# annegnx/PnP-Flow

Measured on AMD Instinct MI355X. Metric: restored images/sec, higher is better.
Workload: dtype f32-equivalent (f16 hi+lo split operands, 3 x f16 MFMA per product, f32 accumulate); 1 GPU; CelebA-shaped 256x256 box-inpainting (half-size 40, sigma 0.05) pnp_flow B=32/GPU 100x5 (the configuration BASELINE.json's metric is quoted on; main.py:132-136 at 256^2); image=256x256x3, batch_per_gpu=32, global_batch=32, steps_pnp=100, num_samples=5, weights=synthetic seed 0 (no checkpoint offline), hipgraph=True, unet_batch=160, parallelism=dp1 (contiguous shards of the global batch, no data-path collective)

## Files before the change

pnpflow_amd/csrc/conv_route.h:

```cpp
#pragma once
#include <cstddef>

namespace pf {

constexpr int ROUTE_LDS_MAX = 160 * 1024;

constexpr int PP_MAXCH = 32;
constexpr int PP_PW = 18;
constexpr int pp_w9(int TERMS) { return TERMS == 3 ? 36864 : 18432; }
constexpr int pp_w1(int TERMS) { return TERMS == 3 ? 4096 : 2048; }
constexpr int pp_npix(int MT) { return (8 * MT + 2) * PP_PW; }
constexpr int pp_patch_bytes(int MT) { return pp_npix(MT) * 128; }
constexpr int PP_MT = 1;
constexpr size_t pp_weight_bytes(int n9, int n1, int TERMS) { return (size_t)n9 * pp_w9(TERMS) + (size_t)n1 * pp_w1(TERMS); }
constexpr int pp_teams(int n9, int n1, int TERMS) { return 2 * (pp_weight_bytes(n9, n1, TERMS) + pp_patch_bytes(PP_MT)) <= (size_t)ROUTE_LDS_MAX ? 1 : 2; }
constexpr size_t pp_lds(int n9, int n1, int TEAMS, int TERMS) { return pp_weight_bytes(n9, n1, TERMS) + (size_t)TEAMS * pp_patch_bytes(PP_MT); }
constexpr bool pp_structure(int n9, int n1, bool res) {
    if (res) return n9 == 1 && n1 == 0;
    return (n1 == 0 && n9 >= 1 && n9 <= 3) || (n9 == 1 && (n1 == 2 || n1 == 3));
}

constexpr int SP_PITCH = 20, SP_PW = 18;
constexpr int sp_rows(int MT) { return 8 * MT; }
constexpr int sp_npix(int MT) { return (sp_rows(MT) + 2) * SP_PW; }
constexpr int sp_patch(int MT) { return (sp_rows(MT) + 2) * SP_PITCH * 64; }
constexpr int sp_tap(int NT, int TERMS = 3) { return (TERMS == 3 ? 2 : 1) * NT * 1024; }
constexpr int sp_x(int NT, int TERMS = 3) { return (5 * sp_tap(NT, TERMS) + 4095) / 4096 * 4096; }
constexpr int sp_y(int NT, int TERMS = 3) { return 4 * sp_tap(NT, TERMS); }
constexpr int SP_TAB = PP_MAXCH * 32;
constexpr int sp_lds(int MT, int NT, int TERMS = 3) { return sp_x(NT, TERMS) + sp_y(NT, TERMS) + 2 * sp_patch(MT) + SP_TAB; }

constexpr int DMA_TH = 8, DMA_BN = 128;
constexpr size_t dma_lds() {
    constexpr int PH = DMA_TH + 2, PW = 18, NINST = (PH * PW * 8 + 63) / 64, IPW = (NINST + 3) / 4, BUF = IPW * 4 * 1024;
    return 2 * (size_t)BUF;
}

struct RouteSeg {
    int C = 0, cstride = 0, taps = 0, xform = 0, w_mode = 0;
    bool has_w16 = false;
    bool has_w16_src = false;
    int src_lo = 0, src_hi = 0, src_O = 0, src_kk = 0;
};
struct RouteShape {
    RouteSeg seg[3];
    int nseg = 0, B = 0, H = 0, W = 0, Hs = 0, Ws = 0, Cout = 0, out_cstride = 0, res_cstride = 0, gn_C = 0;
    bool residual = false, addvec = false, coef = false, scale = false, gnb = false;
};
struct RouteEnv {
    int cu_grid = 0;
    int pp = 1;
    int sp = 1;
    int dma = 1;
    int upphase = 1;
};
inline RouteEnv mfma_only(RouteEnv env) { env.pp = env.sp = env.dma = 0; return env; }

enum class ConvFamily { MFMA32, MFMA16, DMA, PP, SP };
struct ConvRoute {
    ConvFamily family = ConvFamily::MFMA32;
    int terms = 0;
    int MT = 0, NT = 0, WM = 0, WN = 0, S = 1, UP = 0, BM = 0, KC = 0;
    int n9 = 0, n1 = 0, teams = 0, nsplit = 0; bool res = false, gnb = false;
    int grid_x = 0, grid_y = 1, xcd_map = 0; size_t lds_bytes = 0;
    int csv_code = 0;
    const char* refused = nullptr;
};

inline int ilog2_exact(int v) { int l = 0; while (l < 30 && (1 << l) < v) ++l; return (1 << l) == v ? l : -1; }

namespace route_detail {

inline bool packed16(const RouteShape& p) {
    for (int i = 0; i < p.nseg; ++i) if (p.seg[i].w_mode != 0 || !p.seg[i].has_w16) return false;
    return true;
}
inline bool chunk_sources(const RouteShape& p, bool nine_taps) {
    for (int i = 0; i < p.nseg; ++i) {
        const RouteSeg& s = p.seg[i];
        if (!s.has_w16_src || s.src_O != p.Cout || (nine_taps && s.src_kk != 9)) return false;
    }
    return true;
}

inline bool pp_ok(const RouteShape& p, int stride, int up, int terms, const RouteEnv& env, int& n9, int& n1) {
    constexpr int TH = 8 * PP_MT;
    if (env.pp == 0 || (terms != 3 && !(terms == 1 && env.pp != 3)) || stride != 1 || up != 0 || p.gnb) return false;
    if (p.Cout != 32 || p.out_cstride != 32 || (p.residual && p.res_cstride != 32)) return false;
    if (p.H % TH || p.W % 16 || p.Hs != p.H || p.Ws != p.W) return false;
    if (ilog2_exact(p.H / TH) < 0 || ilog2_exact(p.W / 16) < 0) return false;
    if (env.cu_grid < 8 || (long long)p.B * (p.H / TH) * (p.W / 16) < 32LL * 2 * env.cu_grid) return false;
    if (p.W > 2048) return false;
    n9 = 0; n1 = 0;
    for (int i = 0; i < p.nseg; ++i) {
        const RouteSeg& s = p.seg[i];
        if (s.w_mode != 0 || !s.has_w16 || s.C % 32) return false;
        if (s.taps == 9) { if (n1 > 0 || s.xform == 0) return false; n9 += s.C / 32; }
        else if (s.taps == 1) { if (s.xform != 0) return false; n1 += s.C / 32; }
        else return false;
    }
    if (!pp_structure(n9, n1, p.residual)) return false;
    if (p.gn_C > 0 && !p.coef) return false;
    if (pp_weight_bytes(n9, n1, terms) + 2 * (size_t)pp_patch_bytes(PP_MT) > (size_t)ROUTE_LDS_MAX) return false;
    return chunk_sources(p, false);
}

inline bool sp_ok(const RouteShape& p, int stride, int up, int terms, const RouteEnv& env) {
    const int mode = env.sp;
    if (mode == 0 || (terms != 3 && !(terms == 1 && mode != 3)) || stride != 1 || up != 0 || p.gnb) return false;
    const int nsplit = p.Cout == 256 ? 2 : 1;
    if (p.Cout != 128 && !(p.Cout == 64 && (mode == 1 || mode == 4)) && !(p.Cout == 256 && mode == 1 && terms == 3)) return false;
    if (p.out_cstride != p.Cout || (p.residual && p.res_cstride != p.Cout)) return false;
    if (!p.addvec) return false;
    const int TH = p.Cout == 64 ? sp_rows(4) : sp_rows(2);
    if (p.H % TH || p.W % 16 || p.Hs != p.H || p.Ws != p.W) return false;
    if ((long long)(TH + 1) * p.W + SP_PW - 1 > 65535) return false;
    if (ilog2_exact(p.H / TH) < 0 || ilog2_exact(p.W / 16) < 0) return false;
    const int grid = env.cu_grid;
    if (grid < 8 || (long long)nsplit * p.B * (p.H / TH) * (p.W / 16) < 4LL * grid || (nsplit == 2 && grid % 16 != 0)) return false;
    int nch = 0;
    for (int i = 0; i < p.nseg; ++i) {
        const RouteSeg& s = p.seg[i];
        if ((double)p.B * p.H * p.W * s.cstride >= 2147483648.0) return false;
        if (s.w_mode != 0 || !s.has_w16 || s.C % 32 || s.taps != 9 || s.xform != 2) return false;
        nch += s.C / 16;
    }
    if (nch < 2 || nch > PP_MAXCH || (nch & 1)) return false;
    if (!(p.gn_C > 0 && p.coef && p.scale)) return false;
    return chunk_sources(p, true);
}

inline bool dma_phase_shape_ok(const RouteShape& p, int terms, const RouteEnv& env) {
    if (env.upphase == 0 || env.dma == 0 || (terms != 3 && terms != 1) || p.nseg != 1 || p.residual || p.gnb) return false;
    if (p.H != 2 * p.Hs || p.W != 2 * p.Ws || p.Hs % DMA_TH != 0 || p.Ws % 16 != 0 || p.Cout % 32 != 0 || (4 * p.Cout) % DMA_BN != 0) return false;
    if (p.seg[0].w_mode != 0 || p.seg[0].C % (terms == 3 ? 32 : 64) != 0) return false;
    if ((size_t)(p.Hs + 2) * (p.Ws + 2) * 128 >= (1ull << 31)) return false;
    if (env.dma >= 2) return true;
    return (long long)p.B * (p.Hs / DMA_TH) * (p.Ws / 16) * (4 * p.Cout / DMA_BN) >= 512;
}

inline bool dma_ok(const RouteShape& p, int stride, int up, int terms, const RouteEnv& env) {
    if (terms != 3 && terms != 1) return false;
    if (terms == 1)
        for (int i = 0; i < p.nseg; ++i)
            if (p.seg[i].w_mode != 0 || !p.seg[i].has_w16_src || (p.seg[i].src_hi - p.seg[i].src_lo) % 64 != 0) return false;
    if (env.dma == 0 || stride != 1 || (up != 0 && up != 1 && up != 2)) return false;
    if (p.gnb) return false;
    if (up == 2) return dma_phase_shape_ok(p, terms, env) && p.seg[0].taps == 4 && p.seg[0].has_w16;
    if (p.Cout % DMA_BN != 0 || p.H % DMA_TH != 0 || p.W % 16 != 0) return false;
    if (up == 1 && (p.H != 2 * p.Hs || p.W != 2 * p.Ws)) return false;
    if (up == 0 && (p.H != p.Hs || p.W != p.Ws)) return false;
    const int kc = terms == 3 ? 32 : 64;
    for (int i = 1; i < p.nseg; ++i) if (p.seg[i].taps == 9 && p.seg[i - 1].taps == 1) return false;
    for (int i = 0; i < p.nseg; ++i) {
        const RouteSeg& s = p.seg[i];
        if (s.w_mode != 0 || !s.has_w16) return false;
        if (s.C % kc != 0 || (s.taps != 9 && s.taps != 1)) return false;
    }
    if ((size_t)(p.Hs + 2) * (p.Ws + 2) * 128 >= (1ull << 31)) return false;
    if (env.dma >= 2) return true;
    const long long wgs = (long long)p.B * (p.H / DMA_TH) * (p.W / 16) * (p.Cout / DMA_BN);
    if (wgs < 512) return false;
    constexpr double min_ratio = 2000.0;
    double macs = 0.0, elts = 0.0; bool all1 = true;
    for (int i = 0; i < p.nseg; ++i) { macs += (double)p.seg[i].taps * p.seg[i].C * p.Cout; elts += p.seg[i].C; all1 &= p.seg[i].taps == 1; }
    if (up) elts *= 0.25;
    if (all1) return p.Cout >= 3 * (int)elts;
    return macs / elts >= min_ratio;
}

struct Tile { int MT, NT, WM, WN; };
constexpr int tile_th(const Tile& t) { return 2 * t.MT * t.WM; }
constexpr int tile_bn(const Tile& t) { return t.WN * t.NT * 32; }
inline long long tile_wgs(const RouteShape& p, const Tile& t) {
    return (long long)p.B * ((p.H + tile_th(t) - 1) / tile_th(t)) * ((p.W + 15) / 16) * ((p.Cout + tile_bn(t) - 1) / tile_bn(t));
}
inline Tile ladder(const RouteShape& p, const Tile* t, int n, long long min_wgs) {
    for (int i = 0; i + 1 < n; ++i) if (tile_wgs(p, t[i]) >= min_wgs) return t[i];
    return t[n - 1];
}
inline void set_tile(ConvRoute& r, const RouteShape& p, const Tile& t, bool xcd_fold) {
    r.MT = t.MT; r.NT = t.NT; r.WM = t.WM; r.WN = t.WN;
    const long long tiles = (long long)p.B * ((p.H + tile_th(t) - 1) / tile_th(t)) * ((p.W + 15) / 16), nblk = (p.Cout + tile_bn(t) - 1) / tile_bn(t);
    r.grid_x = (int)tiles; r.grid_y = (int)nblk; r.xcd_map = 0;
    if (xcd_fold && (tiles * nblk) % 8 == 0) { r.xcd_map = 1; r.grid_x = (int)(tiles * nblk); r.grid_y = 1; }
}
inline size_t mfma_epilogue_floats(const Tile& t) { return 4 * 32 * 36 + (size_t)t.WM * tile_bn(t) * 2; }

inline ConvRoute mfma16(const RouteShape& p, int stride, int up, int terms) {
    ConvRoute r; r.family = ConvFamily::MFMA16; r.terms = terms == 1 ? 1 : 3; r.gnb = p.gnb; r.csv_code = 0;
    if (p.gn_C > 1024 || (p.gn_C > 0 && !p.coef)) { r.refused = "conv_mfma16 parks at most 4 x 256 GroupNorm channels and needs their coefficients"; return r; }
    bool all_1tap = true, all32 = true;
    for (int i = 0; i < p.nseg; ++i) {
        all_1tap &= p.seg[i].taps == 1 && p.seg[i].C % 64 == 0;
        all32 &= p.seg[i].C % 32 == 0;
    }
    if (all_1tap && stride == 1 && !up) { r.S = 1; r.UP = 0; r.KC = 64; }
    else if (stride == 2) { r.S = 2; r.UP = 0; r.KC = 16; }
    else if (up == 2) { r.S = 1; r.UP = 2; r.KC = 16; }
    else { r.S = 1; r.UP = up ? 1 : 0; r.KC = all32 ? 32 : 16; }
    if (p.gnb && !(r.S == 1 && r.UP == 0)) { r.refused = "the GroupNorm-backward epilogue exists at stride 1 without upsampling only"; return r; }
    const long long MIN_WGS = r.KC == 64 ? 1024 : 512;
    static constexpr Tile s1_32 = {2, 1, 4, 1};
    static constexpr Tile s1_64[] = {{4, 1, 2, 2}, {2, 1, 2, 2}, {1, 1, 2, 2}};
    static constexpr Tile s1_128[] = {{4, 1, 1, 4}, {2, 1, 1, 4}, {1, 1, 2, 2}};
    static constexpr Tile s2_32 = {1, 1, 4, 1}, s2_64 = {2, 1, 2, 2}, s2_128 = {1, 1, 2, 2};
    const Tile t = r.S == 1 ? (p.Cout <= 32 ? s1_32 : p.Cout <= 64 ? ladder(p, s1_64, 3, MIN_WGS) : ladder(p, s1_128, 3, MIN_WGS))
                            : (p.Cout <= 32 ? s2_32 : p.Cout <= 64 ? s2_64 : s2_128);
    set_tile(r, p, t, true);
    const int ROW = (r.terms == 3 ? r.KC : r.KC / 2) + 4, HALO = r.KC == 64 ? 0 : 1;
    const int PH = (tile_th(t) - 1) * r.S + 1 + 2 * HALO, PW = 15 * r.S + 1 + 2 * HALO, RS = ((PW * ROW + 63) / 64) * 64;
    const size_t patch = (size_t)PH * RS, epi = mfma_epilogue_floats(t);
    r.lds_bytes = ((patch > epi ? patch : epi) + 2 * (size_t)((p.gn_C + 3) & ~3)) * 4;
    return r;
}

inline ConvRoute mfma32(const RouteShape& p, int stride, int up, int terms) {
    ConvRoute r; r.family = ConvFamily::MFMA32; r.terms = terms; r.csv_code = 0;
    if (p.gnb) { r.refused = "the GroupNorm-backward epilogue exists on conv_mfma16 only"; return r; }
    bool generic = false;
    for (int i = 0; i < p.nseg; ++i) generic |= p.seg[i].w_mode != 0;
    if (generic) {
        for (int i = 0; i < p.nseg; ++i) if (p.seg[i].w_mode == 0) { r.refused = "packed and generic weight operands in one launch"; return r; }
        if (stride != 1 || up) { r.refused = "generic weight operands at stride 1 without upsampling only"; return r; }
    }
    bool all_1tap = true;
    for (int i = 0; i < p.nseg; ++i) all_1tap &= p.seg[i].taps == 1 && (generic ? p.seg[i].C >= 64 : p.seg[i].C % 64 == 0);
    r.BM = generic ? 1 : 0;
    if (all_1tap && stride == 1 && !up) { r.S = 1; r.UP = 0; r.KC = 64; }
    else if (generic) { r.S = 1; r.UP = 0; r.KC = 16; }
    else if (stride == 2) { r.S = 2; r.UP = 0; r.KC = 16; }
    else { r.S = 1; r.UP = up == 2 ? 2 : up ? 1 : 0; r.KC = 16; }
    constexpr long long MIN_WGS = 512;
    static constexpr Tile s1_32 = {2, 1, 4, 1};
    static constexpr Tile s1_64[] = {{2, 2, 4, 1}, {1, 2, 4, 1}, {1, 1, 2, 2}};
    static constexpr Tile s1_128[] = {{2, 2, 2, 2}, {1, 2, 2, 2}, {1, 2, 4, 1}, {1, 1, 2, 2}};
    static constexpr Tile s2_32 = {1, 1, 4, 1}, s2_64 = {1, 2, 4, 1}, s2_128 = {1, 1, 2, 2};
    const Tile t = r.S == 1 ? (p.Cout <= 32 ? s1_32 : p.Cout <= 64 ? ladder(p, s1_64, 3, MIN_WGS) : ladder(p, s1_128, 4, MIN_WGS))
                            : (p.Cout <= 32 ? s2_32 : p.Cout <= 64 ? s2_64 : s2_128);
    set_tile(r, p, t, false);
    const size_t patch = (size_t)((tile_th(t) - 1) * r.S + 3) * (15 * r.S + 3) * (r.KC + 4), epi = mfma_epilogue_floats(t);
    r.lds_bytes = ((patch > epi ? patch : epi) + 2 * (size_t)((p.gn_C + 3) & ~3)) * sizeof(float);
    return r;
}

}

inline bool conv_route_phase_ok(const RouteShape& p, int terms, const RouteEnv& env) { return route_detail::dma_phase_shape_ok(p, terms, env); }

inline ConvRoute conv_route(const RouteShape& p, int stride, int up, int terms, const RouteEnv& env) {
    namespace d = route_detail;
    if (terms != 1 && terms != 3) return d::mfma32(p, stride, up, 0);
    ConvRoute r; r.terms = terms;
    if (d::sp_ok(p, stride, up, terms, env)) {
        r.family = ConvFamily::SP; r.csv_code = 5;
        r.MT = p.Cout == 64 ? 4 : 2; r.NT = p.Cout == 64 ? 2 : 4; r.nsplit = p.Cout == 256 ? 2 : 1; r.res = p.residual;
        for (int i = 0; i < p.nseg; ++i) r.n9 += p.seg[i].C / 16;
        r.grid_x = env.cu_grid; r.lds_bytes = (size_t)sp_lds(r.MT, r.NT, terms);
        return r;
    }
    if (d::pp_ok(p, stride, up, terms, env, r.n9, r.n1)) {
        r.family = ConvFamily::PP; r.csv_code = 2;
        r.MT = PP_MT; r.res = p.residual; r.teams = pp_teams(r.n9, r.n1, terms);
        r.grid_x = env.cu_grid * (r.teams == 1 ? 2 : 1); r.lds_bytes = pp_lds(r.n9, r.n1, r.teams, terms);
        return r;
    }
    r.n9 = r.n1 = 0;
    if (d::dma_ok(p, stride, up, terms, env)) {
        r.family = ConvFamily::DMA; r.csv_code = 1;
        r.MT = 4; r.NT = 1; r.WM = 1; r.WN = 4; r.UP = up; r.KC = terms == 3 ? 32 : 64;
        const long long tiles = up == 2 ? (long long)p.B * (p.Hs / DMA_TH) * (p.Ws / 16) : (long long)p.B * (p.H / DMA_TH) * (p.W / 16);
        const long long nblk = (up == 2 ? 4 * p.Cout : p.Cout) / DMA_BN;
        r.grid_x = (int)tiles; r.grid_y = (int)nblk;
        if ((tiles * nblk) % 8 == 0) { r.xcd_map = 1; r.grid_x = (int)(tiles * nblk); r.grid_y = 1; }
        r.lds_bytes = dma_lds();
        return r;
    }
    return d::packed16(p) ? d::mfma16(p, stride, up, terms) : d::mfma32(p, stride, up, terms);
}

}
```

pnpflow_amd/csrc/conv_sp.hip:

```cpp
#include "pp_common.h"

namespace pf {

constexpr int sp_a9(int MT) { return (sp_npix(MT) * 4 + 255) / 256; }
constexpr int sp_stage_n(int A9, int tap) {
    const int slot = tap < 4 ? tap : tap < 8 ? tap - 1 : 7;
    if (tap == 4 || tap == 8) return 0;
    return A9 / 7 + (slot < A9 % 7 ? 1 : 0);
}
constexpr int sp_stage_0(int A9, int tap) { int n = 0; for (int t = 0; t < tap; ++t) n += sp_stage_n(A9, t); return n; }

__device__ __forceinline__ void glds16_sp(unsigned voff, const char* sbase, unsigned lds_dst) {
    unsigned keep;
    asm volatile("s_mov_b32 %0, m0\n\ts_mov_b32 m0, %3\n\ts_nop 0\n\tglobal_load_lds_dwordx4 %1, %2\n\ts_mov_b32 m0, %0"
                 : "=&s"(keep) : "v"(voff), "s"(sbase), "s"(lds_dst) : "memory");
}

#ifdef PP_PROBE_BUILD
__device__ unsigned long long* g_sp_dbg = nullptr;
#define SP_STAMP(k) do { if (stamp_buf != nullptr && blockIdx.x == 0 && tid == 0 && stamp_n < 64) stamp_buf[stamp_n * 16 + (k)] = __builtin_readcyclecounter(); } while (0)
#else
#define SP_STAMP(k) do { } while (0)
#endif

template <int MT, int NT, bool RES, int TERMS = 3, int NSPLIT = 1>
__global__ __launch_bounds__(256, 1) void conv_sp_kernel(const PPParams p) {
    constexpr int TH = sp_rows(MT), NPIX = sp_npix(MT), A9 = sp_a9(MT), PATCH = sp_patch(MT);
    constexpr int TAPB = sp_tap(NT, TERMS), XB = sp_x(NT, TERMS), COUT = 32 * NT, CTOT = COUT * NSPLIT, OB = CTOT * 4;
    constexpr int NFRAG = (TERMS == 3 ? 2 : 1) * (MT + NT), NMMA = TERMS * MT * NT;
    static_assert(TERMS == 3 || TERMS == 1, "split terms");
    static_assert(NSPLIT == 1 || NSPLIT == 2, "N-halves");
    static_assert(sp_y(NT, TERMS) % 4096 == 0 && 9 * TAPB >= XB, "refill rounds of 4 KiB; slot X's over-fetch stays inside the chunk image");
    constexpr int REQ1 = sp_stage_0(A9, 4), REQ2 = A9 - REQ1 + 3;
    static_assert(sp_stage_0(A9, 9) == A9 && REQ1 + NT + 4 * MT * NT < 64, "staging distribution / vmcnt range");
    extern __shared__ __attribute__((aligned(16))) char smem[];
    const int tid = threadIdx.x;
    const int lane = tid & 63, wq = __builtin_amdgcn_readfirstlane(tid >> 6);
    const int l31 = lane & 31, hi = lane >> 5;
    constexpr unsigned PATCH0 = (unsigned)(XB + sp_y(NT, TERMS)), TAB = PATCH0 + 2u * (unsigned)PATCH;
    const pp_float_cptr scale_c = (pp_float_cptr)(uintptr_t)p.scale;
    const int nch = p.n9;

    const int qi = tid & 3, p0 = tid >> 2;
    unsigned pk[A9], ldsw[A9];
#pragma unroll
    for (int i = 0; i < A9; ++i) {
        const int pp = min(p0 + 64 * i, NPIX - 1);
        const int py = pp / SP_PW, px = pp - py * SP_PW;
        pk[i] = (unsigned)(py * p.W + px) | ((py == 0 ? 1u : 0u) << 20) | ((py == TH + 1 ? 1u : 0u) << 21) | ((px == 0 ? 1u : 0u) << 22) |
                ((px == SP_PW - 1 ? 1u : 0u) << 23);
        ldsw[i] = PATCH0 + (unsigned)((py * SP_PITCH + px) * 64) + (unsigned)((((qi >> 1) ^ ((px >> 2) & 3)) << 4) + (qi & 1) * 8);
    }
    const int pix_safe = p.W + 1;

    const int prow = l31 >> 4, pcol = l31 & 15;
    unsigned a_addr[3][2];
#pragma unroll
    for (int kx = 0; kx < 3; ++kx) {
        const unsigned base = PATCH0 + (unsigned)(((wq * 2 * MT + prow) * SP_PITCH + pcol + kx) * 64);
        const unsigned s = (unsigned)(((pcol + kx) >> 2) & 3);
#pragma unroll
        for (int tm = 0; tm < 2; ++tm) a_addr[kx][tm] = base + ((((unsigned)(hi + 2 * tm)) ^ s) << 4);
    }
    const unsigned b_lane = (unsigned)lane * 16u;
    const unsigned dma_lane = (unsigned)(wq * 1024 + lane * 16);

    const bool bit3 = (lane & 8) != 0;
    const int em = lane & 7;
    const int ch_of_col = 4 * (l31 & 7) + (l31 >> 3);
    const unsigned e_lane = (unsigned)((4 * hi + ((lane >> 3) & 3)) * OB + em * 16);

    const int G = (int)gridDim.x / NSPLIT;
    const int rg0 = (blockIdx.x & 7) * ((int)gridDim.x >> 3) + (blockIdx.x >> 3);
    const int rg = NSPLIT == 2 ? rg0 >> 1 : rg0, half = NSPLIT == 2 ? rg0 & 1 : 0;
    const int hoff = NSPLIT == 2 ? half * COUT : 0;
    const int T = p.B << (p.lx + p.ly);
    const int t_begin = (int)((long)rg * T / G), t_end = (int)((long)(rg + 1) * T / G);
    const int ntl = t_end - t_begin;
    const int rot = ntl > 0 ? (int)(((long)rg * p.rot) % ntl) : 0;
    auto tile_of = [&](int it) __attribute__((always_inline)) -> PPTile {
        const int idx = min(it, ntl - 1);
        const int wrapped = idx + rot >= ntl ? idx + rot - ntl : idx + rot;
        const int tl = t_begin + wrapped;
        PPTile r;
        const int tx = tl & ((1 << p.lx) - 1), ty = (tl >> p.lx) & ((1 << p.ly) - 1);
        r.b = tl >> (p.lx + p.ly); r.oy0 = ty * TH; r.ox0 = tx * 16;
        r.edge = (ty == 0 ? 1 : 0) | (ty == (1 << p.ly) - 1 ? 2 : 0) | (tx == 0 ? 4 : 0) | (tx == (1 << p.lx) - 1 ? 8 : 0);
        return r;
    };

    float4 ra[A9];
    unsigned zero_v;
    asm volatile("v_mov_b32 %0, 0" : "=v"(zero_v));
    struct Coef { float4 csc, csh; float ascale; unsigned inval; };
    Coef cf0, cf1;
    typedef const __attribute__((address_space(1))) char* gptr;
    struct Src { gptr base; unsigned cs4; };
    const unsigned q16 = (unsigned)qi * 16u;
    struct Desc { gptr base; const char* cb; unsigned cs4; int edge; unsigned sofs; };
    struct Ent { uint4 a, b; };
    auto fetch = [&](int c) __attribute__((always_inline)) -> Ent {
        Ent e;
        e.a = *reinterpret_cast<const uint4*>(smem + TAB + (unsigned)c * 32u); e.b = *reinterpret_cast<const uint4*>(smem + TAB + (unsigned)c * 32u + 16u);
        return e;
    };
    auto sptr = [&](unsigned lo, unsigned hi) __attribute__((always_inline)) -> gptr {
        return (gptr)(((unsigned long long)(unsigned)__builtin_amdgcn_readfirstlane((int)hi) << 32) | (unsigned)__builtin_amdgcn_readfirstlane((int)lo));
    };
    auto describe = [&](const PPTile& tl, const Ent& e) __attribute__((always_inline)) -> Desc {
        const int pix = (tl.b * p.H + tl.oy0) * p.W + tl.ox0 - p.W - 1;
        const int cstride = __builtin_amdgcn_readfirstlane((int)e.b.x), coff = __builtin_amdgcn_readfirstlane((int)e.b.y);
        const int gn_c0 = __builtin_amdgcn_readfirstlane((int)e.b.z), seg = __builtin_amdgcn_readfirstlane((int)e.b.w);
        Desc d;
        d.sofs = (unsigned)(8 * tl.b + seg) * 4u;
        d.edge = tl.edge;
        d.cb = reinterpret_cast<const char*>(p.coef + (tl.b * 2 * p.coef_stride + gn_c0));
        d.base = sptr(e.a.x, e.a.y) + (long)(pix * cstride + coff) * 4;
        d.cs4 = (unsigned)cstride * 4u;
        return d;
    };
    auto prep = [&](Coef& N, const Desc& d) __attribute__((always_inline)) -> Src {
        N.ascale = *reinterpret_cast<const float*>(reinterpret_cast<const char*>(p.scale) + d.sofs + zero_v);
        unsigned inval = 0;
#pragma unroll
        for (int i = 0; i < A9; ++i) inval |= (((pk[i] >> 20) & (unsigned)d.edge) != 0u ? 1u : 0u) << i;
        N.inval = inval;
        N.csc = *reinterpret_cast<const float4*>(d.cb + q16); N.csh = *reinterpret_cast<const float4*>(d.cb + (unsigned)(p.coef_stride * 4) + q16);
        Src r; r.base = d.base; r.cs4 = d.cs4;
        return r;
    };
    auto issue_one = [&](const Coef& N, const Src& sr, int i) __attribute__((always_inline)) {
        const unsigned px = ((N.inval >> i) & 1u) ? (unsigned)pix_safe : (pk[i] & 0xffffu);
        const pp_f4v t_ = *reinterpret_cast<const __attribute__((address_space(1))) pp_f4v*>(sr.base + (__umul24(px, sr.cs4) + q16));
        ra[i] = make_float4(t_.x, t_.y, t_.z, t_.w);
    };
    auto transform_one = [&](const Coef& S, int i, unsigned pofs) __attribute__((always_inline)) {
        float4 v = ra[i];
        v.x = silu_pp(v.x * S.csc.x + S.csh.x); v.y = silu_pp(v.y * S.csc.y + S.csh.y);
        v.z = silu_pp(v.z * S.csc.z + S.csh.z); v.w = silu_pp(v.w * S.csc.w + S.csh.w);
        const float f = ((S.inval >> i) & 1u) ? 0.0f : S.ascale;
        v.x *= f; v.y *= f; v.z *= f; v.w *= f;
        f16x4 h = {(_Float16)v.x, (_Float16)v.y, (_Float16)v.z, (_Float16)v.w};
        if constexpr (TERMS == 3) {
            f16x4 l = {(_Float16)(v.x - (float)h[0]), (_Float16)(v.y - (float)h[1]), (_Float16)(v.z - (float)h[2]), (_Float16)(v.w - (float)h[3])};
            const unsigned addr = ldsw[i] + pofs;
            *reinterpret_cast<f16x4*>(smem + addr) = h;
            *reinterpret_cast<f16x4*>(smem + (addr ^ 32u)) = l;
        } else {
            *reinterpret_cast<f16x4*>(smem + ldsw[i] + pofs) = h;
        }
    };

    f32x16 acc[MT][NT];
#pragma unroll
    for (int mt = 0; mt < MT; ++mt)
#pragma unroll
        for (int nt = 0; nt < NT; ++nt)
#pragma unroll
            for (int r = 0; r < 16; ++r) acc[mt][nt][r] = 0.f;
    float run1[4 * NT], run2[4 * NT];
#pragma unroll
    for (int j = 0; j < 4 * NT; ++j) { run1[j] = 0.f; run2[j] = 0.f; }
    int run_b = -1, run_n = 0;

    auto flush_stats = [&]() __attribute__((always_inline)) {
        if (p.stats_out == nullptr || run_b < 0) return;
#pragma unroll
        for (int j = 0; j < 4 * NT; ++j) {
            double a = (double)run1[j], q = (double)run2[j];
            a += __shfl_xor(a, 8); q += __shfl_xor(q, 8);
            a += __shfl_xor(a, 16); q += __shfl_xor(q, 16);
            a += __shfl_xor(a, 32); q += __shfl_xor(q, 32);
            if (lane < 8) {
                double* dst = p.stats_out + ((size_t)run_b * CTOT + hoff + (j >> 2) * 32 + em * 4 + (j & 3)) * 2;
                unsafeAtomicAdd(dst, a); unsafeAtomicAdd(dst + 1, q);
            }
            run1[j] = 0.f; run2[j] = 0.f;
        }
        run_n = 0;
    };

    auto tile_offs = [&](int mt, int nt, int g) __attribute__((always_inline)) -> size_t {
        return (size_t)((mt * 2 + (g >> 1)) * p.W) * OB + (size_t)((g & 1) * 8 * OB + nt * 128) + e_lane;
    };
    int seg_c1 = -1, seg_c2 = -1;
    for (int c = 1; c < nch; ++c)
        if (p.ch[c].seg != p.ch[c - 1].seg) { if (seg_c1 < 0) seg_c1 = c; else seg_c2 = c; }
    const int seg_id[4] = {p.ch[0].seg, p.ch[seg_c1 > 0 ? seg_c1 : 0].seg, p.ch[seg_c2 > 0 ? seg_c2 : 0].seg, p.ch[nch - 1].seg};
    float addv[NT]; float oscale = 0.f;
    auto tile_inputs = [&](const PPTile& tl) __attribute__((always_inline)) {
#pragma unroll
        for (int nt = 0; nt < NT; ++nt) addv[nt] = p.addvec[(size_t)tl.b * p.addvec_bs + hoff + nt * 32 + ch_of_col];
        const float inv_last = scale_c[8 * tl.b + 4 + seg_id[3]];
        oscale = p.out_scale * (1.0f / 256.0f) * inv_last;
        asm volatile("" : "+v"(oscale));
    };
    auto epilogue = [&](const PPTile& tl) __attribute__((always_inline)) {
        if (tl.b != run_b || run_n >= 32) { flush_stats(); run_b = tl.b; }
        ++run_n;
        const size_t pix0 = ((size_t)tl.b * p.H + tl.oy0 + wq * 2 * MT) * p.W + tl.ox0;
        char* obase = reinterpret_cast<char*>(p.out + pix0 * CTOT + hoff);
        const char* rbase = RES ? reinterpret_cast<const char*>(p.residual + pix0 * CTOT + hoff) : nullptr;
        float4 rv[3][4];
        if constexpr (RES) {
#pragma unroll
            for (int g = 0; g < 4; ++g) rv[0][g] = nt_load4(rbase + tile_offs(0, 0, g));
            if (MT * NT > 1) {
#pragma unroll
                for (int g = 0; g < 4; ++g) rv[1][g] = nt_load4(rbase + tile_offs(1 / NT, 1 % NT, g));
            }
        }
#pragma unroll
        for (int mt = 0; mt < MT; ++mt)
#pragma unroll
            for (int nt = 0; nt < NT; ++nt) {
                const int k = mt * NT + nt;
                if constexpr (RES) {
                    if (k + 2 < MT * NT) {
#pragma unroll
                        for (int g = 0; g < 4; ++g) rv[(k + 2) % 3][g] = nt_load4(rbase + tile_offs((k + 2) / NT, (k + 2) % NT, g));
                    }
                }
                float e[16];
#pragma unroll
                for (int r = 0; r < 16; ++r) e[r] = acc[mt][nt][r] * oscale + addv[nt];
#pragma unroll
                for (int g = 0; g < 4; ++g) {
                    oct_transpose(e[4 * g], e[4 * g + 1], e[4 * g + 2], e[4 * g + 3], bit3);
                    float4 v = make_float4(e[4 * g], e[4 * g + 1], e[4 * g + 2], e[4 * g + 3]);
                    if constexpr (RES) {
                        const float rsc = p.res_scale; const float4 r4 = rv[k % 3][g];
                        v.x = fmaf(r4.x, rsc, v.x); v.y = fmaf(r4.y, rsc, v.y); v.z = fmaf(r4.z, rsc, v.z); v.w = fmaf(r4.w, rsc, v.w);
                    }
                    *reinterpret_cast<float4*>(obase + tile_offs(mt, nt, g)) = v;
                    run1[nt * 4 + 0] += v.x; run1[nt * 4 + 1] += v.y; run1[nt * 4 + 2] += v.z; run1[nt * 4 + 3] += v.w;
                    run2[nt * 4 + 0] += v.x * v.x; run2[nt * 4 + 1] += v.y * v.y; run2[nt * 4 + 2] += v.z * v.z; run2[nt * 4 + 3] += v.w * v.w;
                }
            }
#pragma unroll
        for (int mt = 0; mt < MT; ++mt)
#pragma unroll
            for (int nt = 0; nt < NT; ++nt)
#pragma unroll
                for (int r = 0; r < 16; ++r) acc[mt][nt][r] = 0.f;
    };

    f16x8 fa[2][MT][2], fb[2][NT][2];
    auto load_tap = [&](int set, int tap, unsigned pofs) __attribute__((always_inline)) {
        const int ky = tap / 3, kx = tap % 3;
        const unsigned wb = (unsigned)(tap < 5 ? tap * TAPB : XB + (tap - 5) * TAPB) + b_lane;
        if constexpr (TERMS == 3) {
#pragma unroll
            for (int mt = 0; mt < MT; ++mt) fa[set][mt][1] = *reinterpret_cast<const f16x8*>(smem + a_addr[kx][1] + (unsigned)((mt * 2 + ky) * SP_PITCH * 64) + pofs);
        }
#pragma unroll
        for (int nt = 0; nt < NT; ++nt) fb[set][nt][0] = *reinterpret_cast<const f16x8*>(smem + wb + (unsigned)(nt * 1024));
#pragma unroll
        for (int mt = 0; mt < MT; ++mt) fa[set][mt][0] = *reinterpret_cast<const f16x8*>(smem + a_addr[kx][0] + (unsigned)((mt * 2 + ky) * SP_PITCH * 64) + pofs);
        if constexpr (TERMS == 3) {
#pragma unroll
            for (int nt = 0; nt < NT; ++nt) fb[set][nt][1] = *reinterpret_cast<const f16x8*>(smem + wb + (unsigned)(NT * 1024 + nt * 1024));
        }
    };
    auto load_frag = [&](int set, int tap, unsigned pofs, int idx) __attribute__((always_inline)) {
        const int ky = tap / 3, kx = tap % 3;
        const unsigned wb = (unsigned)(tap < 5 ? tap * TAPB : XB + (tap - 5) * TAPB) + b_lane;
        if constexpr (TERMS == 3) {
            if (idx < MT) fa[set][idx][1] = *reinterpret_cast<const f16x8*>(smem + a_addr[kx][1] + (unsigned)((idx * 2 + ky) * SP_PITCH * 64) + pofs);
            else if (idx < MT + NT) fb[set][idx - MT][0] = *reinterpret_cast<const f16x8*>(smem + wb + (unsigned)((idx - MT) * 1024));
            else if (idx < 2 * MT + NT) fa[set][idx - MT - NT][0] = *reinterpret_cast<const f16x8*>(smem + a_addr[kx][0] + (unsigned)(((idx - MT - NT) * 2 + ky) * SP_PITCH * 64) + pofs);
            else fb[set][idx - 2 * MT - NT][1] = *reinterpret_cast<const f16x8*>(smem + wb + (unsigned)(NT * 1024 + (idx - 2 * MT - NT) * 1024));
        } else {
            if (idx < NT) fb[set][idx][0] = *reinterpret_cast<const f16x8*>(smem + wb + (unsigned)(idx * 1024));
            else fa[set][idx - NT][0] = *reinterpret_cast<const f16x8*>(smem + a_addr[kx][0] + (unsigned)(((idx - NT) * 2 + ky) * SP_PITCH * 64) + pofs);
        }
    };
    auto mma_group = [&](int set, int g) __attribute__((always_inline)) {
        const int term = TERMS == 3 ? g / MT : 2, mt = g % MT;
#pragma unroll
        for (int nt = 0; nt < NT; ++nt)
            acc[mt][nt] = __builtin_amdgcn_mfma_f32_32x32x16_f16(fa[set][mt][term == 0 ? 1 : 0], fb[set][nt][term == 1 ? 1 : 0], acc[mt][nt], 0, 0, 0);
    };
    auto mma_tap = [&](int set) __attribute__((always_inline)) {
#pragma unroll
        for (int g = 0; g < TERMS * MT; ++g) mma_group(set, g);
    };
    auto tap_pattern = [&]() __attribute__((always_inline)) {
        if constexpr (TERMS == 3) {
#pragma unroll
        for (int k = 0; k < 3 * MT * NT; ++k) {
            __builtin_amdgcn_sched_group_barrier(0x008, 1, 0);
            if (k < 2 * (MT + NT)) __builtin_amdgcn_sched_group_barrier(0x100, 1, 0);
            if (k < 2 * (MT + NT)) __builtin_amdgcn_sched_group_barrier(0x002, A9 > 7 ? 2 : 1, 0);
            else __builtin_amdgcn_sched_group_barrier(0x002, A9 > 7 ? 5 : 3, 0);
            __builtin_amdgcn_sched_group_barrier(0x400, 1, 0);
            __builtin_amdgcn_sched_group_barrier(0x004, 2, 0);
            if (k >= 3 * MT * NT - 4) __builtin_amdgcn_sched_group_barrier(0x200, 1, 0);
            if (k == 3 * MT * NT - 2) __builtin_amdgcn_sched_group_barrier(0x020, 1, 0);
        }
        } else {
#pragma unroll
        for (int k = 0; k < MT * NT; ++k) {
            __builtin_amdgcn_sched_group_barrier(0x008, 1, 0);
            if (k < NFRAG) __builtin_amdgcn_sched_group_barrier(0x100, 1, 0);
            __builtin_amdgcn_sched_group_barrier(0x002, A9 > 7 ? 10 : 6, 0);
            __builtin_amdgcn_sched_group_barrier(0x400, A9 > 7 ? 2 : 1, 0);
            __builtin_amdgcn_sched_group_barrier(0x004, 4, 0);
            if (k >= MT * NT - 4) __builtin_amdgcn_sched_group_barrier(0x200, 1, 0);
            if (k >= MT * NT - 2) __builtin_amdgcn_sched_group_barrier(0x020, 1, 0);
        }
        }
    };
    auto mma_tap_refill = [&](int set, const __attribute__((address_space(1))) char* src, int t0, int nrounds, int nset, int ntap, unsigned npofs) __attribute__((always_inline)) {
        const unsigned dst0 = (unsigned)(t0 < 5 ? t0 * TAPB : XB + (t0 - 5) * TAPB) + (unsigned)(wq * nrounds * 1024);
        const __attribute__((address_space(1))) char* sb = src + t0 * TAPB + wq * nrounds * 1024;
        unsigned keep;
        asm volatile("s_mov_b32 %0, m0" : "=s"(keep));
#pragma unroll
        for (int g = 0; g < TERMS * MT; ++g) {
            const int term = TERMS == 3 ? g / MT : 2, mt = g % MT;
#pragma unroll
            for (int nt = 0; nt < NT; ++nt) {
                acc[mt][nt] = __builtin_amdgcn_mfma_f32_32x32x16_f16(fa[set][mt][term == 0 ? 1 : 0], fb[set][nt][term == 1 ? 1 : 0], acc[mt][nt], 0, 0, 0);
                __builtin_amdgcn_sched_barrier(0);
                const int j = g * NT + nt;
                if (j < nrounds) {
                    if ((j & 3) == 0) asm volatile("s_mov_b32 m0, %0\n\ts_nop 0" :: "s"(dst0 + (unsigned)(j * 1024)) : "memory");
                    if ((j & 3) == 0) asm volatile("global_load_lds_dwordx4 %0, %1" :: "v"(b_lane), "s"(sb + j * 1024) : "memory");
                    if ((j & 3) == 1) asm volatile("global_load_lds_dwordx4 %0, %1 offset:1024" :: "v"(b_lane), "s"(sb + (j - 1) * 1024) : "memory");
                    if ((j & 3) == 2) asm volatile("global_load_lds_dwordx4 %0, %1 offset:2048" :: "v"(b_lane), "s"(sb + (j - 2) * 1024) : "memory");
                    if ((j & 3) == 3) asm volatile("global_load_lds_dwordx4 %0, %1 offset:3072" :: "v"(b_lane), "s"(sb + (j - 3) * 1024) : "memory");
                }
                if (j < NFRAG) load_frag(nset, ntap, npofs, j);
                __builtin_amdgcn_sched_barrier(0);
            }
        }
        asm volatile("s_mov_b32 m0, %0" :: "s"(keep));
    };

    int stamp_n = 0; (void)stamp_n;
#ifdef PP_PROBE_BUILD
    unsigned long long* const stamp_buf = g_sp_dbg;
#endif
    gptr wimg_next = (gptr)(uintptr_t)(half ? p.wimg_h1[1] : p.ch[1].wimg);
    Desc dn;
    Src sr;
    auto chunk = [&](int it, int c, auto SI_, bool last_chunk) __attribute__((always_inline)) {
        constexpr int SI = decltype(SI_)::value;
        constexpr unsigned PCUR = SI ? PATCH : 0, PNXT = SI ? 0 : PATCH;
        Coef& C = SI == 0 ? cf1 : cf0;
        Coef& N = SI == 0 ? cf0 : cf1;
        const gptr wnext = wimg_next;
        (void)last_chunk;
        SP_STAMP(0);
#pragma unroll
        for (int tap = 0; tap < 4; ++tap) {
            __builtin_amdgcn_sched_barrier(0);
            load_tap((tap + 1 + SI) & 1, tap + 1, PCUR);
#pragma unroll
            for (int i = sp_stage_0(A9, tap); i < sp_stage_0(A9, tap) + sp_stage_n(A9, tap); ++i) { transform_one(C, i, PNXT); issue_one(N, sr, i); }
            mma_tap((tap + SI) & 1);
            tap_pattern();
            __builtin_amdgcn_sched_barrier(0);
            SP_STAMP(1 + tap);
        }
        __builtin_amdgcn_sched_barrier(0);
        if (c == 0) asm volatile("s_waitcnt vmcnt(%0) lgkmcnt(0)" :: "n"(REQ1 + NT + 4 * MT * NT) : "memory");
        else asm volatile("s_waitcnt vmcnt(%0) lgkmcnt(0)" :: "n"(REQ1) : "memory");
#pragma unroll
        for (int i = REQ1; i < A9; ++i) asm volatile("" :: "v"(ra[i].x));
        SP_STAMP(13);
        __builtin_amdgcn_s_barrier();
        __builtin_amdgcn_sched_barrier(0);
        SP_STAMP(5);
        mma_tap_refill((4 + SI) & 1, wnext, 0, XB / 4096, (5 + SI) & 1, 5, PCUR);
        SP_STAMP(6);
#pragma unroll
        for (int tap = 5; tap < 8; ++tap) {
            __builtin_amdgcn_sched_barrier(0);
            int q = c + 3, wrap = 0;
            if (q >= nch) { q -= nch; wrap = 1; }
            if (q >= nch) { q -= nch; wrap = 2; }
            const int c2 = c + 2 >= nch ? c + 2 - nch : c + 2;
            Ent eq, e2;
            if (tap == 6) { eq = fetch(q); e2 = fetch(c2); }
            load_tap((tap + 1 + SI) & 1, tap + 1, PCUR);
#pragma unroll
            for (int i = sp_stage_0(A9, tap); i < sp_stage_0(A9, tap) + sp_stage_n(A9, tap); ++i) { transform_one(C, i, PNXT); issue_one(N, sr, i); }
            if (tap == 6) {
                dn = describe(tile_of(it + wrap), eq);
                wimg_next = sptr(e2.a.z, e2.a.w);
            }
            if (tap == 7) sr = prep(C, dn);
            mma_tap((tap + SI) & 1);
            tap_pattern();
            __builtin_amdgcn_sched_barrier(0);
            SP_STAMP(2 + tap);
        }
        __builtin_amdgcn_sched_barrier(0);
        asm volatile("s_waitcnt vmcnt(%0) lgkmcnt(0)" :: "n"(REQ2) : "memory");
#pragma unroll
        for (int i = 0; i < REQ1; ++i) asm volatile("" :: "v"(ra[i].x));
        SP_STAMP(14);
        __builtin_amdgcn_s_barrier();
        __builtin_amdgcn_sched_barrier(0);
        SP_STAMP(10);
        mma_tap_refill((8 + SI) & 1, wnext, 5, 4 * TAPB / 4096, (9 + SI) & 1, 0, PNXT);
        SP_STAMP(11);
        SP_STAMP(12);
        ++stamp_n;
    };

    if (ntl <= 0) return;
    for (int c = 0; c < nch; ++c) {
        if (tid == 0) {
            const unsigned long long sp_ = (unsigned long long)(uintptr_t)p.ch[c].src, wp_ = (unsigned long long)(uintptr_t)(half ? p.wimg_h1[c] : p.ch[c].wimg);
            *reinterpret_cast<uint4*>(smem + TAB + (unsigned)c * 32u) = make_uint4((unsigned)sp_, (unsigned)(sp_ >> 32), (unsigned)wp_, (unsigned)(wp_ >> 32));
            *reinterpret_cast<uint4*>(smem + TAB + (unsigned)c * 32u + 16u) = make_uint4((unsigned)p.ch[c].cstride, (unsigned)p.ch[c].coff, (unsigned)p.ch[c].gn_c0, (unsigned)p.ch[c].seg);
        }
    }
    __syncthreads();
    {
        const Src s0 = prep(cf0, describe(tile_of(0), fetch(0)));
#pragma unroll
        for (int i = 0; i < A9; ++i) issue_one(cf0, s0, i);
        {
            const char* w0 = reinterpret_cast<const char*>(half ? p.wimg_h1[0] : p.ch[0].wimg);
#pragma unroll
            for (int j = 0; j < (TERMS == 3 ? 9 * TAPB : XB) / 4096; ++j) glds16_sp(dma_lane, w0 + j * 4096, (unsigned)(j * 4096) + (unsigned)(wq * 1024));
            if constexpr (TERMS != 3) {
#pragma unroll
                for (int j = 0; j < 4 * TAPB / 4096; ++j) glds16_sp(dma_lane, w0 + 5 * TAPB + j * 4096, (unsigned)(XB + j * 4096) + (unsigned)(wq * 1024));
            }
        }
#pragma unroll
        for (int i = 0; i < A9; ++i) transform_one(cf0, i, 0);
        const Src s1 = prep(cf1, describe(tile_of(0), fetch(1)));
#pragma unroll
        for (int i = 0; i < A9; ++i) issue_one(cf1, s1, i);
        sr = prep(cf0, describe(tile_of(2 >= nch ? 1 : 0), fetch(2 >= nch ? 2 - nch : 2)));
        asm volatile("s_waitcnt vmcnt(0) lgkmcnt(0)" ::: "memory");
        __builtin_amdgcn_s_barrier();
        __builtin_amdgcn_sched_barrier(0);
        load_tap(0, 0, 0);
    }
    const int seg_lo[4] = {0, seg_c1 > 0 ? seg_c1 : nch, seg_c2 > 0 ? seg_c2 : nch, nch};
#pragma unroll 1
    for (int it = 0; it < ntl; ++it) {
        tile_inputs(tile_of(it));
#pragma unroll 1
        for (int sg = 0; sg < 3; ++sg) {
            const int lo = seg_lo[sg], hi = seg_lo[sg + 1];
            if (lo >= hi) continue;
            if (sg > 0) {
                const PPTile tl = tile_of(it);
                const float ratio = scale_c[8 * tl.b + seg_id[sg]] * scale_c[8 * tl.b + 4 + seg_id[sg - 1]];
                if (ratio != 1.0f) {
#pragma unroll
                    for (int mt = 0; mt < MT; ++mt)
#pragma unroll
                        for (int nt = 0; nt < NT; ++nt)
#pragma unroll
                            for (int r = 0; r < 16; ++r) acc[mt][nt][r] *= ratio;
                }
            }
#pragma unroll 1
            for (int c = lo; c < hi; c += 2) {
                chunk(it, c, ic<0>{}, false);
                chunk(it, c + 1, ic<1>{}, false);
            }
        }
        epilogue(tile_of(it));
    }
    flush_stats();
    asm volatile("s_waitcnt vmcnt(0)" ::: "memory");
}


template <int MT, int NT, int TERMS, int NSPLIT = 1>
static hipError_t launch_sp_t(const PPParams& p0, const ConvRoute& r, hipStream_t s) {
    static unsigned long long attr_set[2] = {0ull, 0ull};
    const void* kern = r.res ? reinterpret_cast<const void*>(conv_sp_kernel<MT, NT, true, TERMS, NSPLIT>) : reinterpret_cast<const void*>(conv_sp_kernel<MT, NT, false, TERMS, NSPLIT>);
    { hipError_t e = set_max_dynamic_lds_once(kern, attr_set[r.res ? 1 : 0], ROUTE_LDS_MAX); if (e != hipSuccess) return e; }
    if (r.grid_x <= 0 || (NSPLIT == 2 && r.grid_x % 16 != 0)) return hipErrorInvalidConfiguration;
    PPParams p = p0;
    p.lx = ilog2_exact(p.W / 16); p.ly = ilog2_exact(p.H / sp_rows(MT));
    p.rot = 5;
    if (r.res) hipLaunchKernelGGL((conv_sp_kernel<MT, NT, true, TERMS, NSPLIT>), dim3(r.grid_x), dim3(256), r.lds_bytes, s, p);
    else hipLaunchKernelGGL((conv_sp_kernel<MT, NT, false, TERMS, NSPLIT>), dim3(r.grid_x), dim3(256), r.lds_bytes, s, p);
    return hipGetLastError();
}

hipError_t launch_conv_sp(const PPParams& p, const ConvRoute& r, hipStream_t s) {
    if (r.family != ConvFamily::SP || r.n9 != p.n9 || p.n1 != 0 || r.res != (p.residual != nullptr)) return hipErrorInvalidValue;
    switch (r.MT * 1000 + r.NT * 100 + r.nsplit * 10 + r.terms) {
        case 2423: return launch_sp_t<2, 4, 3, 2>(p, r, s);
        case 2413: return launch_sp_t<2, 4, 3>(p, r, s);
        case 2411: return launch_sp_t<2, 4, 1>(p, r, s);
        case 4213: return launch_sp_t<4, 2, 3>(p, r, s);
        case 4211: return launch_sp_t<4, 2, 1>(p, r, s);
        default: return hipErrorInvalidValue;
    }
}

}
```

pnpflow_amd/csrc/engine.hip:

```cpp
#include <algorithm>
#include <cmath>
#include <cstdio>
#include <cstring>
#include <cstdlib>
#include <functional>
#include <map>
#include <memory>
#include <string>
#include <vector>

#include "../../include/pnpflow_hip.h"
#include "pf_common.h"
#include "weight_pack.h"
#include "rk45_control.h"
#include "adam_step.h"

using namespace pf;

namespace {

struct HostTensor { std::vector<int64_t> shape; std::vector<float> data; bool loaded = false; };

struct ResDesc {
    std::string prefix;
// ... 73 lines not shown
    int in_ch = 0, out_ch = 0;
    bool up = false, down = false;
};

struct CachedGraph;
struct SolverBufs;
struct OdeBufs;
struct DFlowState;
struct DopriState;
struct PnpGsState;
struct FlowPriorsState;
struct PriorEvalState;

struct pf_engine {
    int device = 0;
    pf_unet_cfg cfg{};
    int arch = 0;
    pf_ncsnpp_cfg ncfg{};
    std::vector<NxMod> nx_mods;
    float solver_time_scale = 1.0f;
    std::string err;
    std::vector<std::pair<std::string, std::vector<int64_t>>> expected;
    std::map<std::string, HostTensor> host;
    bool finalized = false;
    std::vector<LevelDesc> down, up;
    ResDesc mid0, mid2; std::string mid_attn;
    int mid_ch = 0;
    std::vector<std::pair<std::string, int>> res_order;
    std::map<std::string, float*> dev;
    struct W16Src { std::string name; int lo, hi; };
    std::map<const void*, W16Src> w16_src;
    std::vector<void*> weight_allocs;
    int temb_total = 0;
    std::map<std::string, int> temb_off;
    std::map<int, std::unique_ptr<Plan>> plans;
    Plan* last_plan = nullptr;
    Plan* retained_plan = nullptr;
    int retained_B = 0;
    uint64_t plan_clock = 0;
    int64_t bytes = 0;
    int precision = 1;
    SolverBufs* sb = nullptr;
    OdeBufs* ob = nullptr;
    int64_t ode_krylov_iters = 0;
    hipStream_t work_stream = nullptr;
    DFlowState* dflow = nullptr;
    DopriState* dopri = nullptr;
    PnpGsState* pnpgs = nullptr;
    PriorEvalState* prior = nullptr;
    FlowPriorsState* fprior = nullptr;
    std::vector<CachedGraph*> graphs;
    bool profile = false;
    std::vector<std::pair<hipEvent_t, hipEvent_t>> ev_pool;
    std::vector<const Op*> ev_ops;
    size_t ev_used = 0;
    int64_t prof_launches = 0; double prof_ms = 0.0, prof_flops = 0.0;
};

static thread_local std::string g_create_err;

static int poison_mask() { static const int m = getenv("PNPFLOW_HIP_POISON") ? atoi(getenv("PNPFLOW_HIP_POISON")) : 0; return m == 1 ? 7 : m; }
static bool poison_enabled() { return poison_mask() != 0; }
static void poison(void* p, size_t bytes, int group = 1) {
    if ((poison_mask() & group) && p) { hipDeviceSynchronize(); hipMemset(p, 0xFF, bytes); hipDeviceSynchronize(); }
}

struct DeviceGuard {
    int prev = -1; hipError_t err = hipSuccess;
    explicit DeviceGuard(int dev) { if (hipGetDevice(&prev) != hipSuccess) prev = -1; err = hipSetDevice(dev); }
    ~DeviceGuard() { if (prev >= 0) hipSetDevice(prev); }
};
#define USE_DEVICE(e) DeviceGuard _dg((e)->device); HIPCHK(e, _dg.err)

#define LAUNCHCHK(call)                                                        \
    do { hipError_t _r = (call); if (_r != hipSuccess) return _r == hipErrorInvalidValue ? PF_ERR_INVALID : PF_ERR_HIP; } while (0)


#define HIPCHK(e, call)                                                                        \
    do {                                                                                       \
        hipError_t _r = (call);                                                                \
        if (_r != hipSuccess) {                                                                \
            (e)->err = std::string(#call) + ": " + hipGetErrorString(_r);                      \
            return PF_ERR_HIP;                                                                 \
        }                                                                                      \
    } while (0)

#include "solver_rt.inc"

static bool in_attn_res(const pf_unet_cfg& c, int h) {
    for (int i = 0; i < c.num_attn_resolutions; ++i) if (c.attn_resolutions[i] == h) return true;
    return false;
}

static void expect(pf_engine* e, const std::string& n, std::vector<int64_t> s) { e->expected.emplace_back(n, std::move(s)); }
static void expect_lin(pf_engine* e, const std::string& p, int i, int o) { expect(e, p + "weight", {o, i}); expect(e, p + "bias", {o}); }
static void expect_conv(pf_engine* e, const std::string& p, int i, int o, int k) { expect(e, p + "weight", {o, i, k, k}); expect(e, p + "bias", {o}); }
static void expect_gn(pf_engine* e, const std::string& p, int c) { expect(e, p + "weight", {c}); expect(e, p + "bias", {c}); }
static void expect_res(pf_engine* e, const std::string& p, int i, int o, int tch) {
    expect_lin(e, p + "temb_proj.", tch, o); expect_gn(e, p + "norm1.", i); expect_conv(e, p + "conv1.", i, o, 3);
    expect_gn(e, p + "norm2.", o); expect_conv(e, p + "conv2.", o, o, 3);
    if (i != o) expect_conv(e, p + "shortcut.", i, o, 1);
}
static void expect_attn(pf_engine* e, const std::string& p, int c) {
    expect_conv(e, p + "attn_q.", c, c, 1); expect_conv(e, p + "attn_k.", c, c, 1);
    expect_conv(e, p + "attn_v.", c, c, 1); expect_conv(e, p + "proj_out.", c, c, 1);
    expect_gn(e, p + "norm.", c);
}

static int build_arch(pf_engine* e) {
    const pf_unet_cfg& c = e->cfg;
    const int ch = c.ch, nlev = c.num_levels, nres = c.num_res_blocks, tch = 4 * ch;
    char buf[128];
    expect_lin(e, "temb_net.main.0.", ch, tch); expect_lin(e, "temb_net.main.2.", tch, tch);
    expect_conv(e, "begin_conv.", c.input_channels, ch, 3);
    std::vector<int> chans{ch};
    int cur = ch, h = c.input_height;
    for (int lvl = 0; lvl < nlev; ++lvl) {
        LevelDesc L;
        const int o = ch * c.ch_mult[lvl];
        for (int blk = 0; blk < nres; ++blk) {
            ResDesc r;
            snprintf(buf, sizeof buf, "down_modules.%d.%da_%da_block.", lvl, lvl, blk); r.prefix = buf;
            r.cin0 = cur; r.cout = o;
            expect_res(e, r.prefix, cur, o, tch);
            if (in_attn_res(c, h)) {
                r.attn = true;
                snprintf(buf, sizeof buf, "down_modules.%d.%da_%db_attn.", lvl, lvl, blk); r.attn_prefix = buf;
                expect_attn(e, r.attn_prefix, o);
            }
            L.blocks.push_back(r); chans.push_back(o); cur = o;
        }
        if (lvl != nlev - 1) {
            snprintf(buf, sizeof buf, "down_modules.%d.%db_downsample.", lvl, lvl); L.resample = buf; L.res_ch = o;
            expect_conv(e, L.resample, o, o, 3);
            h /= 2; chans.push_back(o);
        }
        e->down.push_back(L);
    }
    e->mid_ch = cur;
    e->mid0.prefix = "mid_modules.0."; e->mid0.cin0 = cur; e->mid0.cout = cur;
    e->mid2.prefix = "mid_modules.2."; e->mid2.cin0 = cur; e->mid2.cout = cur;
    e->mid_attn = "mid_modules.1.";
    expect_res(e, e->mid0.prefix, cur, cur, tch); expect_attn(e, e->mid_attn, cur); expect_res(e, e->mid2.prefix, cur, cur, tch);
    for (int idx = 0; idx < nlev; ++idx) {
        const int lvl = nlev - 1 - idx;
        LevelDesc L;
        const int o = ch * c.ch_mult[lvl];
        for (int blk = 0; blk < nres + 1; ++blk) {
            ResDesc r;
            snprintf(buf, sizeof buf, "up_modules.%d.%da_%da_block.", idx, lvl, blk); r.prefix = buf;
            r.cin0 = cur; r.cin1 = chans.back(); chans.pop_back(); r.cout = o;
            expect_res(e, r.prefix, r.cin0 + r.cin1, o, tch);
            if (in_attn_res(c, h)) {
                r.attn = true;
                snprintf(buf, sizeof buf, "up_modules.%d.%da_%db_attn.", idx, lvl, blk); r.attn_prefix = buf;
                expect_attn(e, r.attn_prefix, o);
            }
            L.blocks.push_back(r); cur = o;
        }
        if (lvl != 0) {
            snprintf(buf, sizeof buf, "up_modules.%d.%db_upsample.up_conv.", idx, lvl); L.resample = buf; L.res_ch = o;
            expect_conv(e, L.resample, o, o, 3);
            h *= 2;
        }
        e->up.push_back(L);
    }
    if (!chans.empty()) { e->err = "internal: skip stack not empty"; return PF_ERR_INVALID; }
    expect_gn(e, "end_conv.0.", cur); expect_conv(e, "end_conv.2.", cur, c.output_channels, 3);
    if (cur != ch) { e->err = "internal: final width != ch"; return PF_ERR_INVALID; }
    for (auto& L : e->down) for (auto& r : L.blocks) e->res_order.emplace_back(r.prefix, r.cout);
    e->res_order.emplace_back(e->mid0.prefix, e->mid0.cout); e->res_order.emplace_back(e->mid2.prefix, e->mid2.cout);
    for (auto& L : e->up) for (auto& r : L.blocks) e->res_order.emplace_back(r.prefix, r.cout);
    int off = 0;
    for (auto& pr : e->res_order) { e->temb_off[pr.first] = off; off += pr.second; }
    e->temb_total = off;
    return PF_OK;
}

static const HostTensor& W(pf_engine* e, const std::string& n) { return e->host.at(n); }

static float* upload_new(pf_engine* e, const std::string& key, const void* src, size_t bytes) {
    float* d = nullptr;
    if (hipMalloc(&d, std::max<size_t>(bytes, 16)) != hipSuccess) return nullptr;
    e->bytes += (int64_t)std::max<size_t>(bytes, 16);
    hipMemcpy(d, src, bytes, hipMemcpyHostToDevice);
    e->weight_allocs.push_back(d);
    e->dev[key] = d;
    return d;
}
static float* upload(pf_engine* e, const std::string& key, const std::vector<float>& v) {
    auto it = e->dev.find(key);
    return it != e->dev.end() ? it->second : upload_new(e, key, v.data(), v.size() * sizeof(float));
}

static wpack::Oihw oihw(pf_engine* e, const std::string& wname) {
    const HostTensor& t = W(e, wname);
    return {t.data.data(), (int)t.shape[0], (int)t.shape[1], (int)(t.shape[2] * t.shape[3])};
}
static std::string range_key(int lo, int hi) { return std::to_string(lo) + ":" + std::to_string(hi); }

template <class Pack>
static float* weight_image(pf_engine* e, const std::string& key, Pack pack, const pf_engine::W16Src* src = nullptr) {
    auto it = e->dev.find(key);
    if (it != e->dev.end()) return it->second;
    const auto img = pack();
    float* d = upload_new(e, key, img.data(), img.size() * sizeof(img[0]));
    if (d && src) e->w16_src[d] = *src;
    return d;
}

static float* packed_conv(pf_engine* e, const std::string& wname, int lo, int hi) {
    return weight_image(e, wname + "#" + range_key(lo, hi), [&] { return wpack::frag32(oihw(e, wname), lo, hi); });
}
static const void* packed_conv16(pf_engine* e, const std::string& wname, int lo, int hi, int terms = 3) {
    const pf_engine::W16Src src{wname, lo, hi};
    return weight_image(e, wname + (terms == 1 ? "#h1_" : "#h") + range_key(lo, hi), [&] { return wpack::slice16(oihw(e, wname), lo, hi, terms); }, terms == 1 ? nullptr : &src);
}

static int conv_terms(const pf_engine* e) { return e->precision == 0 ? 0 : e->precision == 2 ? 1 : 3; }

struct Builder {
    pf_engine* e; Plan* plan; int B; bool ok = true;
    std::multimap<size_t, void*> free_list;
    std::map<void*, size_t> sizes;
    size_t stats_bytes = 0;
    std::vector<std::pair<double**, size_t>> stats_fix;

    float* acquire(size_t nfloats) {
        const size_t bytes = ((nfloats * sizeof(float) + 255) / 256) * 256;
        auto it = free_list.find(bytes);
        if (it != free_list.end()) { void* p = it->second; free_list.erase(it); return (float*)p; }
        void* p = nullptr;
        if (hipMalloc(&p, bytes) != hipSuccess) { ok = false; e->err = "hipMalloc failed (activations)"; return nullptr; }
        poison(p, bytes);
        plan->allocs.push_back(p); sizes[p] = bytes; plan->bytes += (int64_t)bytes; e->bytes += (int64_t)bytes;
        return (float*)p;
    }
    bool keep = getenv("PNPFLOW_HIP_KEEP_ACTIVATIONS") != nullptr;
    void release(float* p) { if (p && !keep) free_list.emplace(sizes[p], p); }
    void recycle(float* p) { if (p) free_list.emplace(sizes[p], p); }
    Tensor make(int C, int H, int W, bool stats) {
        Tensor t; t.C = C; t.H = H; t.W = W; t.p = acquire((size_t)B * H * W * C);
        if (stats) { t.stats = (double*)(uintptr_t)(stats_bytes + 1); stats_bytes += (size_t)B * C * 2 * sizeof(double); }
        return t;
    }
};

static ConvParams base_params(int B, int H, int W, int Hs, int Ws, const Tensor& out) {
    ConvParams p{};
    p.B = B; p.H = H; p.W = W; p.Hs = Hs; p.Ws = Ws; p.Cout = out.C; p.out = out.p; p.out_cstride = out.C;
    p.out_scale = 1.0f; p.res_scale = 1.0f; p.stats_out = out.stats; p.gn_eps = 1e-6f;
    return p;
}

static void add_seg(ConvParams& p, const Tensor& t, int xform, int taps, int gn_off) {
    ConvSeg& s = p.seg[p.nseg++];
    s.src = t.p; s.C = t.C; s.cstride = t.C; s.coff = 0; s.xform = xform; s.taps = taps; s.gn_off = gn_off; s.stats = t.stats;
}
static void packed_seg(pf_engine* e, ConvParams& p, const Tensor& t, int xform, int taps, int gn_off, const std::string& wname, int lo, int hi) {
    add_seg(p, t, xform, taps, gn_off);
    ConvSeg& s = p.seg[p.nseg - 1];
    s.w = packed_conv(e, wname, lo, hi); s.w_mode = 0; s.w16 = packed_conv16(e, wname, lo, hi);
}

static void ensure_coef(Builder& bd) {
    Plan* plan = bd.plan;
    if (plan->coef) return;
    plan->coef = bd.acquire((size_t)bd.B * 2 * Plan::COEF_STRIDE);
    plan->scale = bd.acquire((size_t)bd.B * 8);
    plan->flags = reinterpret_cast<unsigned int*>(bd.acquire(64));
    if (plan->flags) { hipMemset(plan->flags, 0, 64); hipDeviceSynchronize(); }
}

static ConvParams with_coef(Builder& bd, ConvParams p, std::vector<Op>& ops) {
    Plan* plan = bd.plan;
    ensure_coef(bd);
    bool raw_stats = false, packed16 = true;
    for (int i = 0; i < p.nseg; ++i) {
        raw_stats |= p.seg[i].xform == 0 && p.seg[i].stats != nullptr;
        packed16 &= p.seg[i].w_mode == 0 && p.seg[i].w16 != nullptr;
    }
    const bool want_scale = bd.e->precision != 0 && packed16 && (raw_stats || p.gn_C > 0);
    if (p.gn_C == 0 && !want_scale) return p;
    Op op{}; op.kind = OP_GN_COEF;
    GnCoefParams& g = op.gp;
    g.nseg = p.nseg;
    for (int i = 0; i < p.nseg; ++i) { g.st[i] = p.seg[i].stats; g.C[i] = p.seg[i].C; g.xform[i] = p.seg[i].xform; g.gn_off[i] = p.seg[i].gn_off; }
    g.gn_C = p.gn_C; g.gn_cpg = p.gn_cpg; g.HW = p.Hs * p.Ws; g.eps = p.gn_eps; g.gamma = p.gamma; g.beta = p.beta;
    g.coef = plan->coef; g.coef_stride = Plan::COEF_STRIDE; g.scale = want_scale ? plan->scale : nullptr; g.flags = plan->flags; g.id = (int)ops.size();
    static const bool ret_env = !(getenv("PNPFLOW_HIP_GN_RETAIN") && atoi(getenv("PNPFLOW_HIP_GN_RETAIN")) == 0);
    if (plan->retain && ret_env && p.gn_C > 0 && &ops == &plan->ops && !plan->gn_ret.count(p.gamma)) {
        float* mu = bd.acquire((size_t)bd.B * p.gn_C); float* rs = bd.acquire((size_t)bd.B * p.gn_C);
        if (mu && rs) { g.mu_out = mu; g.rs_out = rs; plan->gn_ret[p.gamma] = {mu, rs}; }
    }
    ops.push_back(op);
    p.coef = plan->coef; p.coef_stride = Plan::COEF_STRIDE; p.scale = want_scale ? plan->scale : nullptr;
    return p;
}

static RouteEnv route_env() {
    static const RouteEnv switches = [] {
        auto rd = [](const char* name) { const char* v = getenv(name); return v ? atoi(v) : 1; };
        RouteEnv v; v.pp = rd("PNPFLOW_HIP_PP"); v.sp = rd("PNPFLOW_HIP_SP"); v.dma = rd("PNPFLOW_HIP_DMA"); v.upphase = rd("PNPFLOW_HIP_UPPHASE");
        return v;
    }();
    RouteEnv v = switches; v.cu_grid = persistent_grid();
    return v;
}
static RouteShape routed_shape(pf_engine* e, const ConvParams& p) {
    RouteShape s = route_shape(p);
    for (int i = 0; i < p.nseg; ++i) {
        auto it = e->w16_src.find(p.seg[i].w16);
        if (it == e->w16_src.end()) continue;
        const wpack::Oihw w = oihw(e, it->second.name);
        RouteSeg& q = s.seg[i];
        q.has_w16_src = true; q.src_lo = it->second.lo; q.src_hi = it->second.hi; q.src_O = w.O; q.src_kk = w.kk;
    }
    return s;
}

static bool attach_dma(Builder& bd, ConvParams& p, const ConvRoute& r, std::vector<Op>& ops) {
    pf_engine* e = bd.e;
    if (r.terms == 1)
        for (int i = 0; i < p.nseg; ++i) {
            const pf_engine::W16Src& src = e->w16_src.at(p.seg[i].w16);
            p.seg[i].w16h = packed_conv16(e, src.name, src.lo, src.hi, 1);
            if (!p.seg[i].w16h) return false;
        }
    Op op{}; op.kind = OP_PREP;
    PrepParams& q = op.pp;
    q.nseg = p.nseg; q.B = p.B; q.Hs = p.Hs; q.Ws = p.Ws; q.terms = r.terms;
    q.coef = p.coef; q.coef_stride = p.coef_stride; q.scale = p.scale;
    std::vector<float*> tmp;
    for (int i = 0; i < p.nseg; ++i) {
        ConvSeg& sg = p.seg[i];
        float* a = bd.acquire(conv_dma_a16_bytes(p.B, sg.C, p.Hs, p.Ws, r.terms) / sizeof(float));
        if (!a) return false;
        tmp.push_back(a);
        sg.a16 = a;
        q.src[i] = sg.src; q.dst[i] = a; q.C[i] = sg.C; q.cstride[i] = sg.cstride; q.coff[i] = sg.coff; q.xform[i] = sg.xform; q.gn_off[i] = sg.gn_off;
    }
    ops.push_back(op);
    for (float* a : tmp) bd.recycle(a);
    return true;
}

static bool attach_pp(Builder& bd, const ConvParams& p, const ConvRoute& r, PPParams& q) {
    pf_engine* e = bd.e;
    const bool sp = r.family == ConvFamily::SP;
    const int terms = r.terms;
    q = PPParams{};
    q.cout = p.Cout;
    const int kc = sp ? 16 : 32;
    int n = 0;
    for (int i = 0; i < p.nseg; ++i) {
        const ConvSeg& sg = p.seg[i];
        const pf_engine::W16Src& src = e->w16_src.at(sg.w16);
        const wpack::Oihw w = oihw(e, src.name);
        for (int cc = 0; cc < sg.C / kc; ++cc) {
            PPChunk& k = q.ch[n++];
            k.src = sg.src; k.cstride = sg.cstride; k.coff = sg.coff + cc * kc; k.xform = sg.xform;
            k.gn_c0 = sg.gn_off + cc * kc; k.seg = i;
            const std::string& wn = src.name; const int lo = src.lo + cc * kc;
            const std::string sp_key = wn + (terms == 1 ? "#sph" : "#sp") + std::to_string(p.Cout) + "_" + std::to_string(lo);
            k.wimg = !sp ? weight_image(e, wn + "#pp" + std::to_string(lo), [&] { return wpack::chunk_pp(w, lo); })
                         : weight_image(e, r.nsplit == 2 ? sp_key + "_h0" : sp_key, [&] { return wpack::chunk_sp(w, lo, r.NT, terms, 0); });
            if (!k.wimg) return false;
            if (r.nsplit == 2) {
                q.wimg_h1[n - 1] = weight_image(e, sp_key + "_h1", [&] { return wpack::chunk_sp(w, lo, r.NT, terms, 128); });
                if (!q.wimg_h1[n - 1]) return false;
            }
            (sg.taps == 9 ? q.n9 : q.n1) += 1;
        }
    }
    q.B = p.B; q.H = p.H; q.W = p.W;
    q.out = p.out; q.addvec = p.addvec; q.addvec_bs = p.addvec_bs; q.residual = p.residual; q.res_scale = p.res_scale;
    q.stats_out = p.stats_out; q.out_scale = p.out_scale; q.coef = p.coef; q.coef_stride = p.coef_stride; q.scale = p.scale;
    return true;
}

static ConvFamily push_conv(Builder& bd, const ConvParams& p0, int stride = 1, int up = 0) {
    pf_engine* e = bd.e;
    ConvParams p = with_coef(bd, p0, bd.plan->ops);
    Op op{}; op.kind = OP_CONV;
    op.route = conv_route(routed_shape(e, p), stride, up, conv_terms(e), route_env());
    const ConvFamily f = op.route.family;
    bool built = true;
    if (op.route.refused) { built = false; e->err = std::string("conv launch refused: ") + op.route.refused; }
    else if (f == ConvFamily::PP || f == ConvFamily::SP) built = attach_pp(bd, p, op.route, op.ppp);
    else if (f == ConvFamily::DMA) built = attach_dma(bd, p, op.route, bd.plan->ops);
    if (!built) {
        if (bd.ok) { bd.ok = false; if (!op.route.refused) e->err = "conv launch: a weight image or operand buffer could not be allocated"; }
        return f;
    }
    op.cp = p; op.stride = stride; op.up = up; op.flops = conv_flops(p);
    bd.plan->gemm_flops += op.flops;
    bd.plan->ops.push_back(op);
    return f;
}


static Tensor res_block(Builder& bd, const ResDesc& r, const Tensor& in0, const Tensor* in1, float* temb_vec) {
    pf_engine* e = bd.e; const int B = bd.B, H = in0.H, Wd = in0.W;
    const int cin = in0.C + (in1 ? in1->C : 0);
    Tensor h1 = bd.make(r.cout, H, Wd, true);
    {
        ConvParams p = base_params(B, H, Wd, H, Wd, h1);
        packed_seg(e, p, in0, 2, 9, 0, r.prefix + "conv1.weight", 0, in0.C);
        if (in1) packed_seg(e, p, *in1, 2, 9, in0.C, r.prefix + "conv1.weight", in0.C, cin);
        p.gn_C = cin; p.gn_cpg = cin / 32;
        p.gamma = upload(e, r.prefix + "norm1.weight", W(e, r.prefix + "norm1.weight").data);
        p.beta = upload(e, r.prefix + "norm1.bias", W(e, r.prefix + "norm1.bias").data);
        p.addvec = temb_vec + e->temb_off.at(r.prefix); p.addvec_bs = e->temb_total;
        push_conv(bd, p);
    }
    Tensor out = bd.make(r.cout, H, Wd, true);
    {
        ConvParams p = base_params(B, H, Wd, H, Wd, out);
        packed_seg(e, p, h1, 2, 9, 0, r.prefix + "conv2.weight", 0, r.cout);
        p.gn_C = r.cout; p.gn_cpg = r.cout / 32;
        p.gamma = upload(e, r.prefix + "norm2.weight", W(e, r.prefix + "norm2.weight").data);
        p.beta = upload(e, r.prefix + "norm2.bias", W(e, r.prefix + "norm2.bias").data);
        std::vector<float> bias = W(e, r.prefix + "conv2.bias").data;
        if (cin != r.cout) {
            const std::string sw = r.prefix + "shortcut.weight";
            packed_seg(e, p, in0, 0, 1, 0, sw, 0, in0.C);
            if (in1) packed_seg(e, p, *in1, 0, 1, 0, sw, in0.C, cin);
            const auto& sb = W(e, r.prefix + "shortcut.bias").data;
            for (size_t i = 0; i < bias.size(); ++i) bias[i] += sb[i];
        } else {
            p.residual = in0.p; p.res_cstride = in0.C;
        }
        p.addvec = upload(e, r.prefix + "conv2.bias+sc", bias); p.addvec_bs = 0;
        push_conv(bd, p);
    }
    bd.release(h1.p);
    if (bd.plan->retain) {
        TapeRec tr; tr.kind = TP_RES; tr.r = &r; tr.in0 = in0; tr.has_in1 = in1 != nullptr; if (in1) tr.in1 = *in1; tr.h1 = h1; tr.out = out;
        bd.plan->tape.push_back(tr);
    }
    return out;
}

static Tensor attn_block(Builder& bd, const std::string& pfx, const Tensor& x, int groups = 32, float s_out = 1.0f) {
    pf_engine* e = bd.e; const int B = bd.B, H = x.H, Wd = x.W, C = x.C, HW = H * Wd;
    std::string key = pfx + "qkv";
    if (!e->dev.count(key + ".w")) {
        HostTensor cat; cat.shape = {3 * C, C, 1, 1}; cat.data.reserve((size_t)3 * C * C);
        std::vector<float> bias;
        for (const char* nm : {"attn_q.", "attn_k.", "attn_v."}) {
            const auto& w = W(e, pfx + nm + "weight").data; cat.data.insert(cat.data.end(), w.begin(), w.end());
            const auto& bb = W(e, pfx + nm + "bias").data; bias.insert(bias.end(), bb.begin(), bb.end());
        }
        e->host[key + ".w"] = cat; e->host[key + ".w"].loaded = true;
        upload(e, key + ".b", bias);
        e->dev[key + ".w"] = packed_conv(e, key + ".w", 0, C);
    }
    static const bool fuse_env = !(getenv("PNPFLOW_HIP_FUSED_ATTN") && atoi(getenv("PNPFLOW_HIP_FUSED_ATTN")) == 0);
    static const bool fold_env = !(getenv("PNPFLOW_HIP_ATTN_FOLD") && atoi(getenv("PNPFLOW_HIP_ATTN_FOLD")) == 0);
    const bool fused = fuse_env && e->precision != 0 && !bd.plan->retain && attn_fused_supported(HW, C);
    const bool fold = fused && fold_env && s_out == 1.0f;
    static const bool pack_env = !(getenv("PNPFLOW_HIP_ATTN_PACK") && atoi(getenv("PNPFLOW_HIP_ATTN_PACK")) == 0);
    const bool kv_packed = fused && pack_env;
    if (fold) {
        key = pfx + "qkvf";
        if (!e->dev.count(key + ".w")) {
            const auto& wv = W(e, pfx + "attn_v.weight").data; const auto& bv = W(e, pfx + "attn_v.bias").data;
            const auto& wp = W(e, pfx + "proj_out.weight").data;
            HostTensor cat; cat.shape = {3 * C, C, 1, 1}; cat.data.reserve((size_t)3 * C * C);
            std::vector<float> bias;
            for (const char* nm : {"attn_q.", "attn_k."}) {
                const auto& w = W(e, pfx + nm + "weight").data; cat.data.insert(cat.data.end(), w.begin(), w.end());
                const auto& bb = W(e, pfx + nm + "bias").data; bias.insert(bias.end(), bb.begin(), bb.end());
            }
            std::vector<double> row((size_t)C);
            for (int o = 0; o < C; ++o) {
                std::fill(row.begin(), row.end(), 0.0);
                double bsum = 0.0;
                for (int m = 0; m < C; ++m) {
                    const double a = (double)wp[(size_t)o * C + m];
                    const float* wr = wv.data() + (size_t)m * C;
                    for (int i = 0; i < C; ++i) row[i] += a * (double)wr[i];
                    bsum += a * (double)bv[m];
                }
                for (int i = 0; i < C; ++i) cat.data.push_back((float)row[i]);
                bias.push_back((float)bsum);
            }
            e->host[key + ".w"] = cat; e->host[key + ".w"].loaded = true;
            upload(e, key + ".b", bias);
            e->dev[key + ".w"] = packed_conv(e, key + ".w", 0, C);
        }
    }
    Tensor qkv = bd.make(3 * C, H, Wd, false);
    {
        ConvParams p = base_params(B, H, Wd, H, Wd, qkv);
        packed_seg(e, p, x, 1, 1, 0, key + ".w", 0, C);
        p.gn_C = C; p.gn_cpg = C / groups;
        p.gamma = upload(e, pfx + "norm.weight", W(e, pfx + "norm.weight").data);
        p.beta = upload(e, pfx + "norm.bias", W(e, pfx + "norm.bias").data);
        p.addvec = e->dev.at(key + ".b"); p.addvec_bs = 0;
        p.pack_from_p1 = kv_packed ? C + 1 : 0;
        push_conv(bd, p);
    }
    if (fold) {
        Tensor out = bd.make(C, H, Wd, true);
        Op op{}; op.kind = OP_ATTN;
        op.ap.qkv = qkv.p; op.ap.out = out.p; op.ap.B = B; op.ap.T = HW; op.ap.C = C; op.ap.scale = 1.0f / sqrtf((float)C); op.ap.kv_packed = kv_packed ? 1 : 0;
        op.ap.bias = upload(e, pfx + "proj_out.bias", W(e, pfx + "proj_out.bias").data); op.ap.residual = x.p;
        float* part = bd.acquire((size_t)B * (HW / 32) * C * 2);
        op.ap.stats_part = part;
        op.flops = (size_t)4 * B * HW * HW * C;
        bd.plan->ops.push_back(op);
        { Op st{}; st.kind = OP_STATS; st.P[0] = part; st.O = out.stats; st.I[0] = HW / 32; st.I[1] = C; bd.plan->ops.push_back(st); }
        bd.recycle(part);
        bd.release(qkv.p);
        return out;
    }
    Tensor S{}, o = bd.make(C, H, Wd, false);
    if (fused) {
        Op op{}; op.kind = OP_ATTN;
        op.ap.qkv = qkv.p; op.ap.out = o.p; op.ap.B = B; op.ap.T = HW; op.ap.C = C; op.ap.scale = 1.0f / sqrtf((float)C); op.ap.kv_packed = kv_packed ? 1 : 0;
        op.flops = (size_t)4 * B * HW * HW * C;
        bd.plan->ops.push_back(op);
    } else {
    S = bd.make(HW, H, Wd, false);
    {
        ConvParams p = base_params(B, H, Wd, H, Wd, S);
        ConvSeg& s = p.seg[p.nseg++];
        s.src = qkv.p; s.C = C; s.cstride = 3 * C; s.coff = 0; s.xform = 0; s.taps = 1; s.stats = nullptr;
        s.w = qkv.p + C; s.w_mode = 1; s.w_bs = (int64_t)HW * 3 * C; s.w_cs = 0; s.w_ts = 0; s.w_ns = 3 * C; s.w_ks = 1;
        p.out_scale = 1.0f / sqrtf((float)C);
        push_conv(bd, p);
    }
    { Op op{}; op.kind = OP_SOFTMAX; op.sm = S.p; op.sm_rows = (int64_t)B * HW; op.sm_cols = HW; bd.plan->ops.push_back(op); }
    {
        ConvParams p = base_params(B, H, Wd, H, Wd, o);
        ConvSeg& s = p.seg[p.nseg++];
        s.src = S.p; s.C = HW; s.cstride = HW; s.coff = 0; s.xform = 0; s.taps = 1; s.stats = nullptr;
        s.w = qkv.p + 2 * C; s.w_mode = 1; s.w_bs = (int64_t)HW * 3 * C; s.w_ks = 3 * C; s.w_cs = 0; s.w_ts = 0; s.w_ns = 1;
        push_conv(bd, p);
    }
    }
    Tensor out = bd.make(C, H, Wd, true);
    {
        ConvParams p = base_params(B, H, Wd, H, Wd, out);
        packed_seg(e, p, o, 0, 1, 0, pfx + "proj_out.weight", 0, C);
        if (s_out == 1.0f) {
            p.addvec = upload(e, pfx + "proj_out.bias", W(e, pfx + "proj_out.bias").data);
        } else {
            std::vector<float> bs = W(e, pfx + "proj_out.bias").data;
            for (auto& v : bs) v *= s_out;
            p.addvec = upload(e, pfx + "proj_out.bias*s", bs);
            p.out_scale = s_out; p.res_scale = s_out;
        }
        p.addvec_bs = 0;
        p.residual = x.p; p.res_cstride = C;
        push_conv(bd, p);
    }
    bd.release(qkv.p); if (S.p) bd.release(S.p); bd.release(o.p);
    if (bd.plan->retain) {
        TapeRec tr; tr.kind = TP_ATTN; tr.pfx = pfx; tr.in0 = x; tr.qkv = qkv; tr.S = S; tr.o = o; tr.out = out; tr.groups = groups; tr.s = s_out;
        bd.plan->tape.push_back(tr);
    }
    return out;
}

static std::string phase_weight(pf_engine* e, const std::string& wname) {
    const std::string key = wname + "#phase";
    if (e->host.count(key)) return key;
    const wpack::Oihw w = oihw(e, wname);
    HostTensor ph; ph.shape = {4 * w.O, w.I, 2, 2}; ph.data = wpack::phase_sums(w); ph.loaded = true;
    e->host[key] = std::move(ph);
    return key;
}

static bool push_conv_up_phase(Builder& bd, const ConvParams& p0, const Tensor& x, const std::string& wname) {
    pf_engine* e = bd.e;
    const int terms = conv_terms(e);
    if (terms == 0) return false;
    ConvParams q = p0;
    add_seg(q, x, 0, 4, 0);
    ConvSeg& sg = q.seg[0];
    if (!conv_route_phase_ok(route_shape(q), terms, route_env())) return false;
    sg.w16 = packed_conv16(e, phase_weight(e, wname), 0, sg.C);
    if (!sg.w16) { bd.ok = false; e->err = "phase upsampling conv: the phase weight image could not be allocated"; return true; }
    if (push_conv(bd, q, 1, 2) != ConvFamily::DMA && bd.ok) { bd.ok = false; e->err = "phase upsampling conv: conv_dma refused a launch it had accepted"; }
    return true;
}

static Tensor resample_conv(Builder& bd, const std::string& pfx, const Tensor& x, bool down) {
    pf_engine* e = bd.e; const int B = bd.B;
    const int H = down ? x.H / 2 : x.H * 2, Wd = down ? x.W / 2 : x.W * 2;
    Tensor out = bd.make(x.C, H, Wd, true);
    ConvParams p = base_params(B, H, Wd, x.H, x.W, out);
    p.addvec = upload(e, pfx + "bias", W(e, pfx + "bias").data); p.addvec_bs = 0;
    if (down || !push_conv_up_phase(bd, p, x, pfx + "weight")) {
        packed_seg(e, p, x, 0, 9, 0, pfx + "weight", 0, x.C);
        push_conv(bd, p, down ? 2 : 1, down ? 0 : 1);
    }
    if (bd.plan->retain) {
        TapeRec tr; tr.kind = down ? TP_DOWN : TP_UP; tr.pfx = pfx; tr.in0 = x; tr.out = out;
        bd.plan->tape.push_back(tr);
    }
    return out;
}

static void fix_stats(Op& op, double* slab) {
    auto fx = [&](const double*& p) { if (p) p = (const double*)((char*)slab + ((uintptr_t)p - 1)); };
    auto fxm = [&](double*& p) { if (p) p = (double*)((char*)slab + ((uintptr_t)p - 1)); };
    if (op.kind == OP_CONV) { for (int i = 0; i < op.cp.nseg; ++i) fx(op.cp.seg[i].stats); fxm(op.cp.stats_out); fxm(op.cp.gnb_sum); if (op.route.family == ConvFamily::PP || op.route.family == ConvFamily::SP) op.ppp.stats_out = op.cp.stats_out; }
    if (op.kind == OP_GN_COEF) for (int i = 0; i < op.gp.nseg; ++i) fx(op.gp.st[i]);
    if (op.kind == OP_STATS) { double* d = (double*)op.O; fxm(d); op.O = d; }
    if (op.kind == OP_NX_FIR) fxm(op.fp.stats_raw);
    if (op.kind == OP_END) fx(op.ep.stats);
    if (op.kind == OP_BEGIN) fxm(op.ep.stats_out);
    if (op.kind == OP_GN_FWD_COEF) { const double* a = (const double*)op.P[0]; const double* b2 = (const double*)op.P[1]; fx(a); fx(b2); op.P[0] = a; op.P[1] = b2; }
    if (op.kind == OP_GN_BWD_PRE || op.kind == OP_GN_BWD_COEF) { const double* a = (const double*)op.P[6]; fx(a); op.P[6] = a; }
}

static int build_backward(pf_engine* e, Plan* plan, struct Builder& bd);
static int nx_build_backward(pf_engine* e, Plan* plan, struct Builder& bd);

static int unet_walk(pf_engine* e, Builder& bd, Plan* plan) {
    const int B = bd.B;
    const pf_unet_cfg& c = e->cfg;
    const int H0 = c.input_height, ch = c.ch, tch = 4 * ch;
    float* temb_vec = bd.acquire((size_t)B * e->temb_total);
    {
        if (!e->dev.count("temb.wp")) {
            std::vector<float> wp, bp;
            for (auto& pr : e->res_order) {
                const auto& w = W(e, pr.first + "temb_proj.weight").data; wp.insert(wp.end(), w.begin(), w.end());
                const auto& b1 = W(e, pr.first + "temb_proj.bias").data; const auto& b2 = W(e, pr.first + "conv1.bias").data;
                for (size_t i = 0; i < b1.size(); ++i) bp.push_back(b1[i] + b2[i]);
            }
            upload(e, "temb.wp", wp); upload(e, "temb.bp", bp);
        }
        Op op{}; op.kind = OP_TEMB;
        op.tp.w0 = upload(e, "temb_net.main.0.weight", W(e, "temb_net.main.0.weight").data);
        op.tp.b0 = upload(e, "temb_net.main.0.bias", W(e, "temb_net.main.0.bias").data);
        op.tp.w1 = upload(e, "temb_net.main.2.weight", W(e, "temb_net.main.2.weight").data);
        op.tp.b1 = upload(e, "temb_net.main.2.bias", W(e, "temb_net.main.2.bias").data);
        op.tp.wp = e->dev.at("temb.wp"); op.tp.bp = e->dev.at("temb.bp");
        op.tp.out = temb_vec; op.tp.B = B; op.tp.ch = ch; op.tp.total_out = e->temb_total;
        (void)tch;
        plan->ops.push_back(op);
    }
    std::vector<Tensor> hs;
    {
        Tensor t0 = bd.make(ch, H0, H0, true);
        const HostTensor& w = W(e, "begin_conv.weight");
        const int ci_n = c.input_channels;
        std::vector<float> wp((size_t)9 * ci_n * ch);
        for (int n = 0; n < ch; ++n) for (int ci = 0; ci < ci_n; ++ci) for (int tap = 0; tap < 9; ++tap)
            wp[((size_t)tap * ci_n + ci) * ch + n] = w.data[((size_t)n * ci_n + ci) * 9 + tap];
        Op op{}; op.kind = OP_BEGIN;
        op.ep.out = t0.p; op.ep.w = upload(e, "begin_conv.packed", wp);
        op.ep.bias = upload(e, "begin_conv.bias", W(e, "begin_conv.bias").data);
        op.ep.B = B; op.ep.H = H0; op.ep.W = H0; op.ep.Cimg = ci_n; op.ep.C = ch;
        op.ep.stats_out = t0.stats;
        if (ch == 32 && e->precision != 0 && (ci_n == 1 || ci_n == 3))
            op.ep.w16 = weight_image(e, "begin_conv.mfma16", [&] { return wpack::edge_frag(oihw(e, "begin_conv.weight"), true); });
        plan->ops.push_back(op);
        hs.push_back(t0);
        plan->t_begin = t0;
        plan->taps.push_back({"begin_conv", t0});
    }
    char nm[64];
    for (size_t lvl = 0; lvl < e->down.size(); ++lvl) {
        const LevelDesc& L = e->down[lvl];
        for (size_t blk = 0; blk < L.blocks.size(); ++blk) {
            Tensor h = res_block(bd, L.blocks[blk], hs.back(), nullptr, temb_vec);
            if (L.blocks[blk].attn) { Tensor a = attn_block(bd, L.blocks[blk].attn_prefix, h); bd.release(h.p); h = a; }
            hs.push_back(h);
            snprintf(nm, sizeof nm, "down%zu_%zu", lvl, blk); plan->taps.push_back({nm, h});
        }
        if (!L.resample.empty()) {
            hs.push_back(resample_conv(bd, L.resample, hs.back(), true));
            snprintf(nm, sizeof nm, "downsample%zu", lvl); plan->taps.push_back({nm, hs.back()});
        }
    }
    Tensor h = hs.back();
    bool h_owned = false;
    {
        Tensor a = res_block(bd, e->mid0, h, nullptr, temb_vec);
        Tensor b2 = attn_block(bd, e->mid_attn, a); bd.release(a.p);
        Tensor c2 = res_block(bd, e->mid2, b2, nullptr, temb_vec); bd.release(b2.p);
        h = c2; h_owned = true;
        plan->taps.push_back({"mid", h});
    }
    for (size_t idx = 0; idx < e->up.size(); ++idx) {
        const LevelDesc& L = e->up[idx];
        const int lvl = (int)e->up.size() - 1 - (int)idx;
        for (size_t blk = 0; blk < L.blocks.size(); ++blk) {
            Tensor skip = hs.back(); hs.pop_back();
            Tensor o = res_block(bd, L.blocks[blk], h, &skip, temb_vec);
            if (h_owned) bd.release(h.p);
            bd.release(skip.p);
            if (L.blocks[blk].attn) { Tensor a = attn_block(bd, L.blocks[blk].attn_prefix, o); bd.release(o.p); o = a; }
            h = o; h_owned = true;
            snprintf(nm, sizeof nm, "up%d_%zu", lvl, blk); plan->taps.push_back({nm, h});
        }
        if (!L.resample.empty()) {
            Tensor o = resample_conv(bd, L.resample, h, false);
            bd.release(h.p); h = o;
            snprintf(nm, sizeof nm, "upsample%d", lvl); plan->taps.push_back({nm, h});
        }
    }
    {
        const HostTensor& w = W(e, "end_conv.2.weight");
        const int co_n = c.output_channels;
        std::vector<float> wp((size_t)9 * co_n * ch);
        for (int co = 0; co < co_n; ++co) for (int ci = 0; ci < ch; ++ci) for (int tap = 0; tap < 9; ++tap)
            wp[((size_t)tap * co_n + co) * ch + ci] = w.data[((size_t)co * ch + ci) * 9 + tap];
        Op op{}; op.kind = OP_END;
        op.ep.in = h.p; op.ep.w = upload(e, "end_conv.packed", wp);
        op.ep.bias = upload(e, "end_conv.2.bias", W(e, "end_conv.2.bias").data);
        op.ep.B = B; op.ep.H = H0; op.ep.W = H0; op.ep.Cimg = co_n; op.ep.C = ch;
        op.ep.stats = h.stats; op.ep.gamma = upload(e, "end_conv.0.weight", W(e, "end_conv.0.weight").data);
        op.ep.beta = upload(e, "end_conv.0.bias", W(e, "end_conv.0.bias").data);
        op.ep.gn_cpg = ch / 32; op.ep.gn_eps = 1e-6f;
        if (ch == 32 && e->precision != 0)
            op.ep.w16 = weight_image(e, "end_conv.mfma16", [&] { return wpack::edge_frag(oihw(e, "end_conv.2.weight"), false); });
        plan->ops.push_back(op);
        plan->t_last = h;
    }
    return PF_OK;
}

#include "engine_ncsnpp.inc"

static int build_plan(pf_engine* e, int B, bool retain, Plan** out_plan) {
    const int key = (B * 2 + (retain ? 1 : 0)) * 3 + e->precision;
    auto it = e->plans.find(key);
    if (it != e->plans.end()) { *out_plan = e->last_plan = it->second.get(); it->second->last_used = ++e->plan_clock; return PF_OK; }
    while (e->plans.size() >= 8) {
        auto victim = e->plans.end();
        for (auto jt = e->plans.begin(); jt != e->plans.end(); ++jt) {
            if (jt->second.get() == e->retained_plan || plan_is_held(e, jt->second.get())) continue;
            if (victim == e->plans.end() || jt->second->last_used < victim->second->last_used) victim = jt;
        }
        if (victim == e->plans.end()) break;
        hipDeviceSynchronize();
        for (void* p : victim->second->allocs) hipFree(p);
        e->bytes -= victim->second->bytes;
        if (e->last_plan == victim->second.get()) e->last_plan = nullptr;
        e->plans.erase(victim);
    }
    auto plan = std::make_unique<Plan>(); plan->B = B; plan->retain = retain; plan->last_used = ++e->plan_clock;
    Builder bd{e, plan.get(), B};
    if (retain) bd.keep = true;
    { Op op{}; op.kind = OP_MEMSET; plan->ops.push_back(op); }
    auto fail = [&](int rc) { for (void* q : plan->allocs) hipFree(q); e->bytes -= plan->bytes; plan->allocs.clear(); plan->bytes = 0; return rc; };
    if (e->arch == 1) {
        int rc = nx_walk(e, bd, plan.get());
        if (rc != PF_OK) return fail(rc);
    } else {
        int rc = unet_walk(e, bd, plan.get());
        if (rc != PF_OK) return fail(rc);
    }
    if (retain) { int rc = e->arch == 1 ? nx_build_backward(e, plan.get(), bd) : build_backward(e, plan.get(), bd); if (rc != PF_OK) return fail(rc); }
    if (!bd.ok) return fail(PF_ERR_HIP);
    for (auto& kv : e->dev) if (kv.second == nullptr) { e->err = "weight upload failed: " + kv.first; return fail(PF_ERR_HIP); }
    void* slab = nullptr;
    if (hipMalloc(&slab, std::max<size_t>(bd.stats_bytes, 256)) != hipSuccess) { e->err = "hipMalloc failed (stats)"; return fail(PF_ERR_HIP); }
    poison(slab, std::max<size_t>(bd.stats_bytes, 256));
    plan->allocs.push_back(slab); plan->bytes += (int64_t)std::max<size_t>(bd.stats_bytes, 256); e->bytes += (int64_t)std::max<size_t>(bd.stats_bytes, 256);
    for (auto& op : plan->ops) fix_stats(op, (double*)slab);
    for (auto& op : plan->bops) fix_stats(op, (double*)slab);
    for (auto& tp : plan->taps) if (tp.t.stats) tp.t.stats = (double*)((char*)slab + ((uintptr_t)tp.t.stats - 1));
    plan->ops[0].ptr = slab; plan->ops[0].bytes = bd.stats_bytes;
    if (!plan->bops.empty()) plan->bops[0].ptr = (char*)slab + ((uintptr_t)plan->bops[0].ptr - 1);
    *out_plan = plan.get();
    e->last_plan = plan.get();
    e->plans[key] = std::move(plan);
    return PF_OK;
}

static std::string adjoint_weight(pf_engine* e, const std::string& wname, int lo, int hi) {
    const std::string key = wname + "#T" + range_key(lo, hi);
    if (!e->host.count(key)) {
        const wpack::Oihw w = oihw(e, wname); const int64_t K = W(e, wname).shape[2];
        HostTensor tt; tt.shape = {hi - lo, w.O, K, K}; tt.data = wpack::adjoint(w, lo, hi); tt.loaded = true;
        e->host[key] = std::move(tt);
    }
    return key;
}

struct GradEntry { Tensor t; bool has = false; };

struct BwdCtx {
    pf_engine* e; Plan* plan; Builder* bd; int B;
    std::map<float*, GradEntry> grads;
    GradEntry& G(const Tensor& fwd) {
        auto it = grads.find(fwd.p);
        if (it == grads.end()) {
            GradEntry g; g.t.C = fwd.C; g.t.H = fwd.H; g.t.W = fwd.W; g.t.p = bd->acquire((size_t)B * fwd.H * fwd.W * fwd.C);
            it = grads.emplace(fwd.p, g).first;
        }
        return it->second;
    }
    Tensor tmp(int C, int H, int W) { Tensor t; t.C = C; t.H = H; t.W = W; t.p = bd->acquire((size_t)B * H * W * C); return t; }
    float* fvec(size_t n) { return bd->acquire(n); }
    double* dsum(size_t n_doubles) { double* p = (double*)(uintptr_t)(bd->stats_bytes + 1); bd->stats_bytes += n_doubles * sizeof(double); return p; }
    void push(const Op& op) { plan->bops.push_back(op); }
    void conv_to(ConvParams p, GradEntry& dst, int stride = 1, int up = 0) {
        p.out = dst.t.p; p.out_cstride = dst.t.C;
        if (dst.has) { p.residual = dst.t.p; p.res_cstride = dst.t.C; }
        dst.has = true;
        conv_plain(p, stride, up);
    }
    void conv_plain(const ConvParams& p, int stride = 1, int up = 0) {
        Op op{}; op.kind = OP_CONV; op.cp = p; op.stride = stride; op.up = up; op.flops = conv_flops(p);
        op.route = conv_route(route_shape(p), stride, up, conv_terms(e), mfma_only(route_env()));
        if (op.route.refused && bd->ok) { bd->ok = false; e->err = std::string("backward conv launch refused: ") + op.route.refused; }
        plan->bwd_flops += op.flops;
        push(op);
    }
};

static ConvParams bwd_params(int B, int H, int W, int Hs, int Ws, int Cout) {
    ConvParams p{};
    p.B = B; p.H = H; p.W = W; p.Hs = Hs; p.Ws = Ws; p.Cout = Cout; p.out_scale = 1.0f; p.res_scale = 1.0f; p.gn_eps = 1e-6f;
    return p;
}
static void raw_seg(ConvParams& p, const float* src, int C, int cstride, int taps, const float* w, const void* w16 = nullptr) {
    ConvSeg& s = p.seg[p.nseg++];
    s.src = src; s.C = C; s.cstride = cstride; s.coff = 0; s.xform = 0; s.taps = taps; s.gn_off = 0; s.stats = nullptr;
    s.w = w; s.w_mode = 0; s.w_bs = 0; s.w_cs = 0; s.w_ts = 0; s.w_ns = 0; s.w_ks = 0; s.w16 = w16;
}
static void adj_seg(pf_engine* e, ConvParams& p, const float* src, int C, int cstride, int taps, const std::string& wname, int lo, int hi) {
    const std::string key = adjoint_weight(e, wname, lo, hi);
    const int cin = (int)W(e, key).shape[1];
    raw_seg(p, src, C, cstride, taps, packed_conv(e, key, 0, cin), packed_conv16(e, key, 0, cin));
}
static void gen_seg(ConvParams& p, const float* src, int C, int cstride, const float* w, int64_t w_bs, int64_t w_ns, int64_t w_ks) {
    ConvSeg& s = p.seg[p.nseg++];
    s.src = src; s.C = C; s.cstride = cstride; s.coff = 0; s.xform = 0; s.taps = 1; s.gn_off = 0; s.stats = nullptr;
    s.w = w; s.w_mode = 1; s.w_bs = w_bs; s.w_cs = 0; s.w_ts = 0; s.w_ns = w_ns; s.w_ks = w_ks;
}

struct GnBwd {
    std::vector<Tensor> srcs; int Ct = 0, cpg = 0, HW = 0; bool silu = false;
    bool retained = false;
    float *mu = nullptr, *rs = nullptr, *m1 = nullptr, *m2 = nullptr; double* bsum = nullptr;
    const float *gamma = nullptr, *beta = nullptr;
    std::vector<bool> fused;
};

static GnBwd gn_bwd_begin(BwdCtx& c, const std::vector<Tensor>& srcs, const std::string& norm_prefix, bool silu, int groups = 32) {
    pf_engine* e = c.e; const int B = c.B;
    GnBwd g; g.srcs = srcs; g.silu = silu; g.HW = srcs[0].H * srcs[0].W;
    for (auto& t : srcs) g.Ct += t.C;
    g.cpg = g.Ct / groups; g.fused.assign(srcs.size(), false);
    g.m1 = c.fvec((size_t)B * g.Ct); g.m2 = c.fvec((size_t)B * g.Ct);
    g.bsum = c.dsum((size_t)B * g.Ct * 2);
    g.gamma = upload(e, norm_prefix + "weight", W(e, norm_prefix + "weight").data);
    g.beta = upload(e, norm_prefix + "bias", W(e, norm_prefix + "bias").data);
    auto rt = c.plan->gn_ret.find(g.gamma);
    if (rt != c.plan->gn_ret.end()) {
        g.mu = rt->second.first; g.rs = rt->second.second; g.retained = true;
        return g;
    }
    g.mu = c.fvec((size_t)B * g.Ct); g.rs = c.fvec((size_t)B * g.Ct);
    Op op{}; op.kind = OP_GN_FWD_COEF; op.P[0] = srcs[0].stats; op.P[1] = srcs.size() > 1 ? srcs[1].stats : nullptr; op.P[2] = g.mu; op.P[3] = g.rs;
    op.I[0] = srcs[0].C; op.I[1] = srcs.size() > 1 ? srcs[1].C : 0; op.I[2] = g.cpg; op.I[3] = g.HW; c.push(op);
    return g;
}

static bool gn_bwd_fuse(BwdCtx& c, GnBwd& g, size_t j, ConvParams& p, int stride = 1, int up = 0) {
    static const bool enabled = !(getenv("PNPFLOW_HIP_GNB_FUSE") && atoi(getenv("PNPFLOW_HIP_GNB_FUSE")) == 0);
    bool ok16 = c.e->precision != 0 && enabled && stride == 1 && up == 0 && p.residual == nullptr && p.stats_out == nullptr && p.Cout % 4 == 0;
    for (int i = 0; i < p.nseg; ++i) ok16 &= p.seg[i].w_mode == 0 && p.seg[i].w16 != nullptr;
    if (!ok16) return false;
    int coff = 0; for (size_t k = 0; k < j; ++k) coff += g.srcs[k].C;
    p.gnb_x = g.srcs[j].p; p.gnb_xstride = g.srcs[j].C; p.gnb_mu = g.mu; p.gnb_rs = g.rs; p.gnb_gamma = g.gamma; p.gnb_beta = g.beta;
    p.gnb_Ct = g.Ct; p.gnb_coff = coff; p.gnb_silu = g.silu ? 1 : 0; p.gnb_sum = g.bsum;
    g.fused[j] = true;
    return true;
}

static void gn_bwd_finish(BwdCtx& c, GnBwd& g, const std::vector<Tensor>& gtmp, const std::vector<GradEntry*>& dst,
                          const std::vector<const float*>& add, float add_scale = 1.0f) {
    int coff = 0;
    for (size_t j = 0; j < g.srcs.size(); ++j) {
        if (!g.fused[j]) {
            Op op{}; op.kind = OP_GN_BWD_PRE; op.O = gtmp[j].p; op.P[0] = g.srcs[j].p; op.P[1] = g.mu; op.P[2] = g.rs; op.P[3] = g.gamma; op.P[4] = g.beta;
            op.P[6] = g.bsum; op.I[0] = g.HW; op.I[1] = g.srcs[j].C; op.I[2] = coff; op.I[3] = g.Ct; op.I[4] = g.silu ? 1 : 0; c.push(op);
        }
        coff += g.srcs[j].C;
    }
    { Op op{}; op.kind = OP_GN_BWD_COEF; op.P[6] = g.bsum; op.P[1] = g.m1; op.P[2] = g.m2; op.I[0] = g.Ct; op.I[1] = g.cpg; op.I[2] = g.HW; c.push(op); }
    coff = 0;
    for (size_t j = 0; j < g.srcs.size(); ++j) {
        Op op{}; op.kind = OP_GN_BWD_POST; op.P[0] = gtmp[j].p; op.P[1] = g.srcs[j].p; op.P[2] = g.mu; op.P[3] = g.rs; op.P[4] = g.m1; op.P[5] = g.m2;
        op.P[7] = add[j]; op.F = add_scale; op.O = dst[j]->t.p; op.I[0] = g.HW; op.I[1] = g.srcs[j].C; op.I[2] = coff; op.I[3] = g.Ct; op.I[4] = dst[j]->has ? 1 : 0;
        dst[j]->has = true; c.push(op);
        coff += g.srcs[j].C;
    }
    if (!g.retained) { c.bd->recycle(g.mu); c.bd->recycle(g.rs); }
    c.bd->recycle(g.m1); c.bd->recycle(g.m2);
}

static void gn_backward(BwdCtx& c, const std::vector<Tensor>& srcs, const std::vector<Tensor>& gtmp, const std::vector<GradEntry*>& dst,
                        const std::vector<const float*>& add, const std::string& norm_prefix, bool silu) {
    GnBwd g = gn_bwd_begin(c, srcs, norm_prefix, silu);
    gn_bwd_finish(c, g, gtmp, dst, add);
}

static void bwd_attn(BwdCtx& c, const TapeRec& tr, GradEntry& gout) {
    pf_engine* e = c.e; Builder& bd = *c.bd; const int B = c.B;
    const int H = tr.out.H, Wd = tr.out.W;
    const Tensor& x = tr.in0; const int C = x.C, HW = H * Wd;
    const float scale = 1.0f / sqrtf((float)C);
    Tensor d_o = c.tmp(C, H, Wd);
    { ConvParams p = bwd_params(B, H, Wd, H, Wd, C);
      adj_seg(e, p, gout.t.p, C, C, 1, tr.pfx + "proj_out.weight", 0, C); p.out = d_o.p; p.out_cstride = C;
      p.out_scale = tr.s; c.conv_plain(p); }
    Tensor dA = c.tmp(HW, H, Wd);
    { ConvParams p = bwd_params(B, H, Wd, H, Wd, HW);
      gen_seg(p, d_o.p, C, C, tr.qkv.p + 2 * C, (int64_t)HW * 3 * C, 3 * C, 1); p.out = dA.p; p.out_cstride = HW; c.conv_plain(p); }
    Tensor dqkv = c.tmp(3 * C, H, Wd);
    Tensor AT = c.tmp(HW, H, Wd);
    { Op op{}; op.kind = OP_TRANSPOSE; op.P[0] = tr.S.p; op.O = AT.p; op.I[0] = HW; op.I[1] = HW; c.push(op); }
    { ConvParams p = bwd_params(B, H, Wd, H, Wd, C);
      gen_seg(p, AT.p, HW, HW, d_o.p, (int64_t)HW * C, 1, C); p.out = dqkv.p + 2 * C; p.out_cstride = 3 * C; c.conv_plain(p); }
    { Op op{}; op.kind = OP_SOFTMAX_BWD; op.P[0] = tr.S.p; op.O = dA.p; op.sm_rows = (int64_t)B * HW; op.sm_cols = HW; op.F = scale; c.push(op); }
    { ConvParams p = bwd_params(B, H, Wd, H, Wd, C);
      gen_seg(p, dA.p, HW, HW, tr.qkv.p + C, (int64_t)HW * 3 * C, 1, 3 * C); p.out = dqkv.p; p.out_cstride = 3 * C; c.conv_plain(p); }
    { Op op{}; op.kind = OP_TRANSPOSE; op.P[0] = dA.p; op.O = AT.p; op.I[0] = HW; op.I[1] = HW; c.push(op); }
    { ConvParams p = bwd_params(B, H, Wd, H, Wd, C);
      gen_seg(p, AT.p, HW, HW, tr.qkv.p, (int64_t)HW * 3 * C, 1, 3 * C); p.out = dqkv.p + C; p.out_cstride = 3 * C; c.conv_plain(p); }
    Tensor dhn = c.tmp(C, H, Wd);
    GnBwd gna = gn_bwd_begin(c, {x}, tr.pfx + "norm.", false, tr.groups);
    { ConvParams p = bwd_params(B, H, Wd, H, Wd, C);
      adj_seg(e, p, dqkv.p, 3 * C, 3 * C, 1, tr.pfx + "qkv.w", 0, C); p.out = dhn.p; p.out_cstride = C;
      gn_bwd_fuse(c, gna, 0, p);
      c.conv_plain(p); }
    gn_bwd_finish(c, gna, {dhn}, {&c.G(x)}, {gout.t.p}, tr.s);
    for (float* q : {d_o.p, dA.p, dqkv.p, AT.p, dhn.p}) bd.recycle(q);
}

static int build_backward(pf_engine* e, Plan* plan, Builder& bd) {
    const int B = plan->B;
    const pf_unet_cfg& cf = e->cfg;
    const int ch = cf.ch, H0 = cf.input_height;
    BwdCtx c{e, plan, &bd, B};
    { Op op{}; op.kind = OP_MEMSET; plan->bops.push_back(op); }
    plan->vec_scaled = bd.acquire((size_t)B * cf.input_channels * cf.input_height * cf.input_height);
    plan->vjp_scale = bd.acquire(64); plan->vjp_amax = reinterpret_cast<unsigned int*>(bd.acquire(64));
    const size_t bwd_lo = bd.stats_bytes;
    {
        const HostTensor& w = W(e, "end_conv.2.weight");
        const int co_n = cf.output_channels;
        std::vector<float> wp((size_t)9 * co_n * ch), zero(ch, 0.f);
        for (int co = 0; co < co_n; ++co) for (int ci = 0; ci < ch; ++ci) for (int tap = 0; tap < 9; ++tap)
            wp[((size_t)tap * co_n + co) * ch + ci] = w.data[((size_t)co * ch + ci) * 9 + (8 - tap)];
        Tensor da = c.tmp(ch, H0, H0);
        Op op{}; op.kind = OP_BEGIN; op.ep.out = da.p; op.ep.w = upload(e, "end_conv.adj", wp); op.ep.bias = upload(e, "zero.ch", zero);
        op.ep.B = B; op.ep.H = H0; op.ep.W = H0; op.ep.Cimg = co_n; op.ep.C = ch; c.push(op);
        gn_backward(c, {plan->t_last}, {da}, {&c.G(plan->t_last)}, {nullptr}, "end_conv.0.", true);
        bd.recycle(da.p);
    }
    for (auto it = plan->tape.rbegin(); it != plan->tape.rend(); ++it) {
        const TapeRec& tr = *it;
        GradEntry& gout = c.G(tr.out);
        if (!gout.has) { e->err = "internal: backward reached a tensor without gradient"; return PF_ERR_INVALID; }
        const int H = tr.out.H, Wd = tr.out.W;
        static const bool upadj_env = !(getenv("PNPFLOW_HIP_UPPHASE_BWD") && atoi(getenv("PNPFLOW_HIP_UPPHASE_BWD")) == 0);
        if (tr.kind == TP_UP && e->precision != 0 && upadj_env && tr.out.C % 16 == 0 && tr.in0.C % 4 == 0) {
            const int Cy = tr.out.C, Cx = tr.in0.C, Hs = tr.in0.H, Ws = tr.in0.W;
            const std::string pk = phase_weight(e, tr.pfx + "weight");
            const HostTensor& ph = W(e, pk);
            GradEntry& gx = c.G(tr.in0);
            for (int dy = 0; dy < 2; ++dy) {
                ConvParams p = bwd_params(B, Hs, Ws, Hs, Ws, Cx);
                p.src_row_pitch = 2 * Ws;
                for (int dxp = 0; dxp < 2; ++dxp) {
                    const std::string key = pk + "T" + std::to_string(dy) + std::to_string(dxp);
                    if (!e->host.count(key)) {
                        HostTensor tt; tt.shape = {Cx, Cy, 2, 2}; tt.data.resize((size_t)Cx * Cy * 4); tt.loaded = true;
                        for (int ci = 0; ci < Cx; ++ci) for (int co = 0; co < Cy; ++co) for (int u = 0; u < 2; ++u) for (int v = 0; v < 2; ++v)
                            tt.data[((size_t)ci * Cy + co) * 4 + u * 2 + v] = ph.data[(((size_t)(dy * 2 + dxp) * Cy + co) * Cx + ci) * 4 + (1 - u) * 2 + (1 - v)];
                        e->host[key] = std::move(tt);
                    }
                    raw_seg(p, gout.t.p + ((size_t)dy * Wd + dxp) * Cy, Cy, 2 * Cy, 4, nullptr, packed_conv16(e, key, 0, Cy));
                    p.seg[p.nseg - 1].oy = 1 - dy; p.seg[p.nseg - 1].ox = 1 - dxp;
                }
                c.conv_to(p, gx);
            }
        } else if (tr.kind == TP_UP) {
            Tensor dU = c.tmp(tr.in0.C, H, Wd);
            ConvParams p = bwd_params(B, H, Wd, H, Wd, tr.in0.C);
            adj_seg(e, p, gout.t.p, tr.out.C, tr.out.C, 9, tr.pfx + "weight", 0, tr.in0.C);
            p.out = dU.p; p.out_cstride = dU.C; c.conv_plain(p);
            GradEntry& gx = c.G(tr.in0);
            Op op{}; op.kind = OP_SUMPOOL; op.P[0] = dU.p; op.O = gx.t.p; op.I[0] = tr.in0.H; op.I[1] = tr.in0.W; op.I[2] = tr.in0.C; op.I[3] = gx.has ? 1 : 0;
            gx.has = true; c.push(op);
            bd.recycle(dU.p);
        } else if (tr.kind == TP_DOWN && e->precision != 0 && upadj_env && tr.out.C % 16 == 0 && tr.in0.C % 4 == 0) {
            const int Cy = tr.out.C, Cx = tr.in0.C, Hc = tr.out.H, Wc = tr.out.W;
            const HostTensor& w = W(e, tr.pfx + "weight");
            GradEntry& gx = c.G(tr.in0);
            static const int KOF[2][2] = {{1, -1}, {2, 0}};
            for (int py = 0; py < 2; ++py) for (int px = 0; px < 2; ++px) {
                const bool one = py == 0 && px == 0;
                const std::string key = tr.pfx + "weight#dT" + std::to_string(py) + std::to_string(px);
                if (!e->host.count(key)) {
                    const int kk = one ? 1 : 4;
                    HostTensor tt; tt.shape = {Cx, Cy, one ? 1 : 2, one ? 1 : 2}; tt.data.assign((size_t)Cx * Cy * kk, 0.f); tt.loaded = true;
                    for (int ci = 0; ci < Cx; ++ci) for (int co = 0; co < Cy; ++co) for (int u = 0; u < (one ? 1 : 2); ++u) for (int v = 0; v < (one ? 1 : 2); ++v) {
                        const int ky = KOF[py][u], kx = KOF[px][v];
                        if (ky >= 0 && kx >= 0) tt.data[((size_t)ci * Cy + co) * kk + u * 2 * (one ? 0 : 1) + v] = w.data[((size_t)co * Cx + ci) * 9 + ky * 3 + kx];
                    }
                    e->host[key] = std::move(tt);
                }
                ConvParams p = bwd_params(B, Hc, Wc, Hc, Wc, Cx);
                raw_seg(p, gout.t.p, Cy, Cy, one ? 1 : 4, nullptr, packed_conv16(e, key, 0, Cy));
                p.seg[0].oy = 1; p.seg[0].ox = 1;
                p.out = gx.t.p + ((size_t)py * tr.in0.W + px) * Cx; p.out_cstride = 2 * Cx; p.dst_row_pitch = 2 * Wc;
                if (gx.has) { p.residual = p.out; p.res_cstride = 2 * Cx; }
                c.conv_plain(p);
            }
            gx.has = true;
        } else if (tr.kind == TP_DOWN) {
            ConvParams p = bwd_params(B, tr.in0.H, tr.in0.W, H, Wd, tr.in0.C);
            adj_seg(e, p, gout.t.p, tr.out.C, tr.out.C, 9, tr.pfx + "weight", 0, tr.in0.C);
            c.conv_to(p, c.G(tr.in0), 1, 2);
        } else if (tr.kind == TP_RES) {
            const ResDesc& r = *tr.r;
            const int cin = tr.in0.C + (tr.has_in1 ? tr.in1.C : 0);
            Tensor t1 = c.tmp(r.cout, H, Wd);
            GnBwd gn2 = gn_bwd_begin(c, {tr.h1}, r.prefix + "norm2.", true);
            {
                ConvParams p = bwd_params(B, H, Wd, H, Wd, r.cout);
                adj_seg(e, p, gout.t.p, r.cout, r.cout, 9, r.prefix + "conv2.weight", 0, r.cout);
                p.out = t1.p; p.out_cstride = r.cout;
                gn_bwd_fuse(c, gn2, 0, p);
                c.conv_plain(p);
            }
            GradEntry gh1; gh1.t = c.tmp(r.cout, H, Wd);
            gn_bwd_finish(c, gn2, {t1}, {&gh1}, {nullptr});
            bd.recycle(t1.p);
            std::vector<Tensor> srcs{tr.in0}; if (tr.has_in1) srcs.push_back(tr.in1);
            std::vector<Tensor> us; std::vector<GradEntry*> dsts; std::vector<const float*> adds;
            GnBwd gn1 = gn_bwd_begin(c, srcs, r.prefix + "norm1.", true);
            int lo = 0;
            for (size_t sj = 0; sj < srcs.size(); ++sj) {
                const Tensor& sT = srcs[sj];
                Tensor u = c.tmp(sT.C, H, Wd);
                ConvParams p = bwd_params(B, H, Wd, H, Wd, sT.C);
                adj_seg(e, p, gh1.t.p, r.cout, r.cout, 9, r.prefix + "conv1.weight", lo, lo + sT.C);
                p.out = u.p; p.out_cstride = sT.C;
                gn_bwd_fuse(c, gn1, sj, p);
                c.conv_plain(p);
                us.push_back(u);
                GradEntry& gd = c.G(sT);
                if (cin != r.cout) {
                    ConvParams q = bwd_params(B, H, Wd, H, Wd, sT.C);
                    adj_seg(e, q, gout.t.p, r.cout, r.cout, 1, r.prefix + "shortcut.weight", lo, lo + sT.C);
                    c.conv_to(q, gd);
                    adds.push_back(nullptr);
                } else {
                    adds.push_back(gout.t.p);
                }
                dsts.push_back(&gd);
                lo += sT.C;
            }
            gn_bwd_finish(c, gn1, us, dsts, adds);
            for (auto& u : us) bd.recycle(u.p);
            bd.recycle(gh1.t.p);
        } else {
            bwd_attn(c, tr, gout);
        }
    }
    {
        GradEntry& g0 = c.G(plan->t_begin);
        if (!g0.has) { e->err = "internal: no gradient at begin_conv output"; return PF_ERR_INVALID; }
        const HostTensor& w = W(e, "begin_conv.weight");
        const int ci_n = cf.input_channels;
        std::vector<float> wp((size_t)9 * ci_n * ch), zero3(4, 0.f);
        for (int n = 0; n < ch; ++n) for (int ci = 0; ci < ci_n; ++ci) for (int tap = 0; tap < 9; ++tap)
            wp[((size_t)tap * ci_n + ci) * ch + n] = w.data[((size_t)n * ci_n + ci) * 9 + (8 - tap)];
        Op op{}; op.kind = OP_END; op.ep.in = g0.t.p; op.ep.w = upload(e, "begin_conv.adj", wp); op.ep.bias = upload(e, "zero.img", zero3);
        op.ep.B = B; op.ep.H = H0; op.ep.W = H0; op.ep.Cimg = ci_n; op.ep.C = ch; op.ep.stats = nullptr; op.ep.gn_cpg = 1; op.ep.gn_eps = 1e-6f;
        c.push(op);
    }
    plan->bops[0].ptr = (void*)(uintptr_t)(bwd_lo + 1);
    plan->bops[0].bytes = bd.stats_bytes - bwd_lo;
    return PF_OK;
}

__global__ __launch_bounds__(256) void zero_fill_kernel(uint4* p, size_t n16, unsigned char* tail, size_t ntail) {
    const uint4 z = make_uint4(0u, 0u, 0u, 0u);
    for (size_t i = (size_t)blockIdx.x * 256 + threadIdx.x; i < n16; i += (size_t)gridDim.x * 256) p[i] = z;
    if (blockIdx.x == 0) for (size_t i = threadIdx.x; i < ntail; i += 256) tail[i] = 0;
}
static hipError_t zero_fill(void* ptr, size_t bytes, hipStream_t s) {
    if (bytes == 0) return hipSuccess;
    if (((uintptr_t)ptr & 15) != 0) return hipMemsetAsync(ptr, 0, bytes, s);
    const size_t n16 = bytes / 16, ntail = bytes % 16;
    const unsigned g = (unsigned)std::min<size_t>((n16 + 255) / 256 + 1, 2048);
    hipLaunchKernelGGL(zero_fill_kernel, dim3(g), dim3(256), 0, s, (uint4*)ptr, n16, (unsigned char*)ptr + n16 * 16, ntail);
    return hipGetLastError();
}

#include "engine_ncsnpp_bwd.inc"

static hipError_t dispatch_conv(const Op& op, hipStream_t s);
static int run_backward(pf_engine* e, Plan* plan, const float* vec, float* g, hipStream_t s) {
    const int B = plan->B;
    const int64_t nimg = (int64_t)B * e->cfg.input_channels * e->cfg.input_height * e->cfg.input_height;
    { hipError_t r = launch_vjp_normalise(vec, plan->vec_scaled, nimg, plan->vjp_amax, plan->vjp_scale, s);
      if (r != hipSuccess) { e->err = std::string("vjp normalise: ") + hipGetErrorString(r); return PF_ERR_HIP; } }
    vec = plan->vec_scaled;
    for (auto& op : plan->bops) {
        hipError_t r = hipSuccess;
        switch (op.kind) {
            case OP_MEMSET: if (op.bytes) r = zero_fill(op.ptr, op.bytes, s); break;
            case OP_BEGIN: { EdgeConvParams ep = op.ep; ep.in = vec; r = launch_begin_conv(ep, s); break; }
            case OP_END: { EdgeConvParams ep = op.ep; ep.out = g; r = launch_end_conv(ep, s); break; }
            case OP_CONV: r = dispatch_conv(op, s); break;
            case OP_PREP: r = launch_prep_split(op.pp, s); break;
            case OP_GN_FWD_COEF:
                r = launch_gn_fwd_coeffs((const double*)op.P[0], op.I[0], (const double*)op.P[1], op.I[1], op.I[2], op.I[3], 1e-6f, (float*)op.P[2],
                                         (float*)op.P[3], B, s); break;
            case OP_GN_BWD_PRE:
                r = launch_gn_bwd_pre((float*)op.O, (const float*)op.P[0], (const float*)op.P[1], (const float*)op.P[2], (const float*)op.P[3],
                                      (const float*)op.P[4], (double*)op.P[6], B, op.I[0], op.I[1], op.I[2], op.I[3], op.I[4], s); break;
            case OP_GN_BWD_COEF:
                r = launch_gn_bwd_coeffs((const double*)op.P[6], op.I[0], op.I[1], op.I[2], (float*)op.P[1], (float*)op.P[2], B, s); break;
            case OP_GN_BWD_POST:
                r = launch_gn_bwd_post((const float*)op.P[0], (const float*)op.P[1], (const float*)op.P[2], (const float*)op.P[3], (const float*)op.P[4],
                                       (const float*)op.P[5], (const float*)op.P[7], (float*)op.O, B, op.I[0], op.I[1], op.I[2], op.I[3], op.I[4], s, op.F); break;
            case OP_TRANSPOSE: r = launch_transpose((const float*)op.P[0], (float*)op.O, B, op.I[0], op.I[1], s); break;
            case OP_SOFTMAX_BWD: r = launch_softmax_bwd((const float*)op.P[0], (float*)op.O, op.sm_rows, op.sm_cols, op.F, s); break;
            case OP_SUMPOOL: r = launch_sumpool2((const float*)op.P[0], (float*)op.O, B, op.I[0], op.I[1], op.I[2], op.I[3], s); break;
            case OP_NX_IMG_IN: r = launch_img_to_nhwc32(vec, (float*)op.O, B, op.I[0], op.I[1], op.I[2], s, (const float*)op.P[0]); break;
            case OP_NX_FIR: r = launch_fir_nhwc(op.fp, s); break;
            case OP_NX_IMG_OUT: r = launch_nhwc32_to_img((const float*)op.P[0], g, (const float*)op.P[1], 1.0f, op.P[1] != nullptr ? 1 : 0, B, op.I[0], op.I[1], op.I[2], s); break;
            default: break;
        }
        if (r != hipSuccess) { e->err = std::string("backward launch failed: ") + hipGetErrorString(r); return PF_ERR_HIP; }
    }
    { hipError_t r = launch_scale_inplace(g, nimg, plan->vjp_scale + 1, s);
      if (r != hipSuccess) { e->err = std::string("vjp rescale: ") + hipGetErrorString(r); return PF_ERR_HIP; } }
    return PF_OK;
}

static hipError_t dispatch_conv(const Op& op, hipStream_t s) {
    switch (op.route.family) {
        case ConvFamily::SP: return launch_conv_sp(op.ppp, op.route, s);
        case ConvFamily::PP: return launch_conv_pp(op.ppp, op.route, s);
        case ConvFamily::DMA: return launch_conv_dma(op.cp, op.route, s);
        case ConvFamily::MFMA16: return launch_conv16(op.cp, op.route, s);
        case ConvFamily::MFMA32: return launch_conv(op.cp, op.route, s);
    }
    return hipErrorInvalidValue;
}

static int run_plan(pf_engine* e, Plan* plan, const float* x, const float* t, float* v, hipStream_t s, float t_scale = 1.0f) {
    bool prep_open = false;
    for (auto& op : plan->ops) {
        hipError_t r = hipSuccess;
        switch (op.kind) {
            case OP_MEMSET: r = zero_fill(op.ptr, op.bytes, s); break;
            case OP_TEMB: { TembParams tp = op.tp; tp.t = t; r = launch_temb(tp, s); break; }
            case OP_BEGIN: { EdgeConvParams ep = op.ep; ep.in = x; r = launch_begin_conv(ep, s); break; }
            case OP_PREP:
                if (e->profile) {
                    if (e->ev_used == e->ev_pool.size()) {
                        hipEvent_t a, b; hipEventCreate(&a); hipEventCreate(&b); e->ev_pool.emplace_back(a, b);
                    }
                    hipEventRecord(e->ev_pool[e->ev_used].first, s);
                    prep_open = true;
                }
                r = launch_prep_split(op.pp, s);
                break;
            case OP_CONV:
                if (e->profile) {
                    if (e->ev_used == e->ev_pool.size()) {
                        hipEvent_t a, b; hipEventCreate(&a); hipEventCreate(&b); e->ev_pool.emplace_back(a, b);
                    }
                    auto& ev = e->ev_pool[e->ev_used++];
                    if (e->ev_ops.size() < e->ev_used) e->ev_ops.resize(e->ev_used);
                    e->ev_ops[e->ev_used - 1] = &op;
                    if (!prep_open) hipEventRecord(ev.first, s);
                    prep_open = false;
                    r = dispatch_conv(op, s);
                    hipEventRecord(ev.second, s);
                    e->prof_flops += (double)op.flops;
                } else {
                    r = dispatch_conv(op, s);
                }
                break;
            case OP_SOFTMAX: r = launch_softmax_rows(op.sm, op.sm_rows, op.sm_cols, s); break;
            case OP_ATTN: r = launch_attn_fused(op.ap, s); break;
            case OP_STATS: r = launch_partial_stats((const float*)op.P[0], (double*)op.O, plan->B, op.I[0], op.I[1], s); break;
            case OP_END: { EdgeConvParams ep = op.ep; ep.out = v; r = launch_end_conv(ep, s); break; }
            case OP_GN_COEF: r = launch_gn_coef(op.gp, plan->B, s); break;
            case OP_NX_TEMB: { NxTembParams tp = op.ntp; tp.t = t; tp.t_scale = t_scale; r = launch_nx_temb(tp, s); break; }
            case OP_NX_IMG_IN: r = launch_img_to_nhwc32(x, (float*)op.O, plan->B, op.I[0], op.I[1], op.I[2], s); break;
            case OP_NX_FIR: r = launch_fir_nhwc(op.fp, s); break;
            case OP_NX_IMG_OUT: r = launch_nhwc32_to_img((const float*)op.P[0], v, t, t_scale, op.I[3], plan->B, op.I[0], op.I[1], op.I[2], s, (float*)op.O); break;
            default: break;
        }
        if (r != hipSuccess) { e->err = std::string("kernel launch failed: ") + hipGetErrorString(r); return PF_ERR_HIP; }
    }
    return PF_OK;
}

__global__ void prep_iter_kernel(const int* iter, const float* t_all, const float* coef_all, float* t_cur, float* coef_cur, int B) {
    const int it = *iter;
    for (int b = threadIdx.x; b < B; b += blockDim.x) { t_cur[b] = t_all[it]; coef_cur[b] = coef_all[it]; }
}
__global__ void bump_iter_kernel(int* iter) { if (threadIdx.x == 0) *iter += 1; }



extern "C" {

int pf_abi_version(void) { return PF_ABI_VERSION; }

const char* pf_last_error(const pf_engine* e) { return e ? e->err.c_str() : g_create_err.c_str(); }

int pf_engine_create(int device_id, const pf_unet_cfg* cfg, pf_engine** out) {
    if (!cfg || !out) { g_create_err = "null argument"; return PF_ERR_INVALID; }
    if (cfg->num_levels < 1 || cfg->num_levels > 8 || cfg->num_attn_resolutions < 0 || cfg->num_attn_resolutions > 8 ||
        cfg->ch != 32 || cfg->input_channels < 1 || cfg->input_channels > 3 || cfg->output_channels < 1 || cfg->output_channels > 3 ||
        cfg->num_res_blocks < 1 || cfg->input_height % (1 << (cfg->num_levels - 1)) != 0) {
        g_create_err = "unsupported UNet configuration (need ch=32, 1..3 image channels, height divisible by 2^(levels-1))";
        return PF_ERR_INVALID;
    }
    int ndev = 0;
    hipError_t r = hipGetDeviceCount(&ndev);
    if (r != hipSuccess || ndev <= 0) { g_create_err = std::string("no HIP device: ") + hipGetErrorString(r); return PF_ERR_HIP; }
    if (device_id < 0 || device_id >= ndev) { g_create_err = "bad device id"; return PF_ERR_INVALID; }
    if ((r = hipSetDevice(device_id)) != hipSuccess) { g_create_err = hipGetErrorString(r); return PF_ERR_HIP; }
    auto* e = new pf_engine();
    e->device = device_id; e->cfg = *cfg;
    int rc = build_arch(e);
    if (rc != PF_OK) { g_create_err = e->err; delete e; return rc; }
    *out = e;
    return PF_OK;
}

int pf_ncsnpp_create(int device_id, const pf_ncsnpp_cfg* cfg, pf_engine** out) {
    if (!cfg || !out) { g_create_err = "null argument"; return PF_ERR_INVALID; }
    bool ok = cfg->num_levels >= 1 && cfg->num_levels <= 8 && cfg->num_attn_resolutions >= 0 && cfg->num_attn_resolutions <= 8 &&
              cfg->nf >= 32 && cfg->nf <= 128 && cfg->nf % 32 == 0 && cfg->num_channels >= 1 && cfg->num_channels <= 3 && cfg->num_res_blocks >= 1 &&
              cfg->fir_taps >= 2 && cfg->fir_taps <= 8 && cfg->fir_taps % 2 == 0 && cfg->centered == 1 && cfg->image_size > 0 &&
              cfg->image_size % (1 << (cfg->num_levels - 1)) == 0;
    for (int i = 0; ok && i < cfg->num_levels; ++i) ok = cfg->ch_mult[i] >= 1 && cfg->nf * cfg->ch_mult[i] <= 256;
    if (!ok) {
        g_create_err = "unsupported NCSN++ configuration (need nf in {32,64,96,128}, nf*ch_mult <= 256, 1..3 image channels, centered data, "
                       "an even-length FIR kernel, image_size divisible by 2^(levels-1))";
        return PF_ERR_INVALID;
    }
    int ndev = 0;
    hipError_t r = hipGetDeviceCount(&ndev);
    if (r != hipSuccess || ndev <= 0) { g_create_err = std::string("no HIP device: ") + hipGetErrorString(r); return PF_ERR_HIP; }
    if (device_id < 0 || device_id >= ndev) { g_create_err = "bad device id"; return PF_ERR_INVALID; }
    if ((r = hipSetDevice(device_id)) != hipSuccess) { g_create_err = hipGetErrorString(r); return PF_ERR_HIP; }
    auto* e = new pf_engine();
    e->device = device_id; e->arch = 1; e->ncfg = *cfg;
    e->cfg.input_channels = e->cfg.output_channels = cfg->num_channels; e->cfg.input_height = cfg->image_size;
    int rc = nx_build_arch(e);
    if (rc != PF_OK) { g_create_err = e->err; delete e; return rc; }
    *out = e;
    return PF_OK;
}

int pf_engine_set_solver_time_scale(pf_engine* e, float scale) {
    if (!e || !(scale > 0.f)) return PF_ERR_INVALID;
    if (scale != e->solver_time_scale) { drop_all_graphs(e); e->solver_time_scale = scale; }
    return PF_OK;
}

static int check_flags(pf_engine* e) {
    bool bad = false; std::string where;
    for (auto& kv : e->plans) {
        Plan* pl = kv.second.get();
        if (!pl->flags) continue;
        unsigned int f[2] = {0, 0};
        HIPCHK(e, hipMemcpy(f, pl->flags, sizeof f, hipMemcpyDeviceToHost));
        if (f[0]) {
            bad = true; HIPCHK(e, hipMemset(pl->flags, 0, sizeof f)); HIPCHK(e, hipDeviceSynchronize());
            char buf[160] = "";
            const int id = (int)f[1];
            if (id >= 1 && id < (int)pl->ops.size() && pl->ops[id].kind == OP_CONV)
                snprintf(buf, sizeof buf, " (first seen by launch #%d of the B=%d plan: %dx%d, K segments %d, Cout %d)", id, pl->B, pl->ops[id].cp.H,
                         pl->ops[id].cp.W, pl->ops[id].cp.nseg, pl->ops[id].cp.Cout);
            where = buf;
        }
    }
    if (bad) {
        e->err = "non-finite activation statistics: an activation overflowed or was NaN inside the U-Net (inputs / weights out of range)" + where;
        return PF_ERR_NUMERIC;
    }
    return PF_OK;
}

static void free_solver_states(pf_engine* e);

void pf_engine_destroy(pf_engine* e) {
    if (!e) return;
    hipSetDevice(e->device);
    free_solver_states(e);
    for (auto& kv : e->plans) for (void* p : kv.second->allocs) hipFree(p);
    for (void* p : e->weight_allocs) hipFree(p);
    for (auto& ev : e->ev_pool) { hipEventDestroy(ev.first); hipEventDestroy(ev.second); }
    if (e->work_stream) hipStreamDestroy(e->work_stream);
    delete e;
}

int pf_engine_num_weights(const pf_engine* e) { return e ? (int)e->expected.size() : 0; }
const char* pf_engine_weight_name(const pf_engine* e, int i) {
    if (!e || i < 0 || i >= (int)e->expected.size()) return nullptr;
    return e->expected[i].first.c_str();
}

int pf_engine_weight_shape(const pf_engine* e, int i, int64_t shape[4]) {
    if (!e || !shape || i < 0 || i >= (int)e->expected.size()) return PF_ERR_INVALID;
    const auto& s = e->expected[i].second;
    for (size_t k = 0; k < s.size() && k < 4; ++k) shape[k] = s[k];
    return (int)s.size();
}

int pf_engine_load_weight(pf_engine* e, const char* name, const float* host_data, const int64_t* shape, int ndim) {
    if (!e || !name || !host_data || !shape) return PF_ERR_INVALID;
    if (e->finalized) { e->err = "weights already finalized"; return PF_ERR_STATE; }
    for (auto& ex : e->expected) {
        if (ex.first != name) continue;
        if ((int)ex.second.size() != ndim) { e->err = std::string("rank mismatch for ") + name; return PF_ERR_WEIGHTS; }
        size_t n = 1;
        for (int i = 0; i < ndim; ++i) {
            if (ex.second[i] != shape[i]) { e->err = std::string("shape mismatch for ") + name; return PF_ERR_WEIGHTS; }
            n *= (size_t)shape[i];
        }
        HostTensor& t = e->host[name];
        t.shape.assign(shape, shape + ndim); t.data.assign(host_data, host_data + n); t.loaded = true;
        return PF_OK;
    }
    e->err = std::string("unexpected weight: ") + name;
    return PF_ERR_WEIGHTS;
}

int pf_engine_finalize_weights(pf_engine* e) {
    if (!e) return PF_ERR_INVALID;
    for (auto& ex : e->expected) {
        auto it = e->host.find(ex.first);
        if (it == e->host.end() || !it->second.loaded) { e->err = "missing weight: " + ex.first; return PF_ERR_WEIGHTS; }
    }
    USE_DEVICE(e);
    e->finalized = true;
    return PF_OK;
}

int pf_engine_set_precision(pf_engine* e, int mode) {
    if (!e) return PF_ERR_INVALID;
    if (mode < 0 || mode > 2) { e->err = "precision mode must be 0 (fp32 MFMA), 1 (split-fp16 MFMA, fp32-equivalent) or 2 (single fp16 MFMA)"; return PF_ERR_INVALID; }
    if (mode != e->precision) drop_all_graphs(e);
    e->precision = mode;
    return PF_OK;
}

int pf_unet_forward(pf_engine* e, const float* x, const float* t, float* v, int B, void* stream) {
    if (!e || !x || !t || !v || B <= 0) return PF_ERR_INVALID;
    if (!e->finalized) { e->err = "weights not finalized"; return PF_ERR_STATE; }
    USE_DEVICE(e);
    Plan* plan = nullptr;
    int rc = build_plan(e, B, false, &plan);
    if (rc != PF_OK) return rc;
    return run_plan(e, plan, x, t, v, (hipStream_t)stream);
}

int pf_unet_forward_retain(pf_engine* e, const float* x, const float* t, float* v, int B, void* stream) {
    if (!e || !x || !t || !v || B <= 0) return PF_ERR_INVALID;
    if (!e->finalized) { e->err = "weights not finalized"; return PF_ERR_STATE; }
    USE_DEVICE(e);
    Plan* plan = nullptr;
    int rc = build_plan(e, B, true, &plan);
    if (rc != PF_OK) return rc;
    e->retained_B = B; e->retained_plan = plan;
    return run_plan(e, plan, x, t, v, (hipStream_t)stream);
}

int pf_unet_backward(pf_engine* e, const float* vec, float* g, int B, void* stream) {
    if (!e || !vec || !g || B <= 0) return PF_ERR_INVALID;
    if (e->retained_B != B || !e->retained_plan) { e->err = "pf_unet_backward: no retained forward with this batch size"; return PF_ERR_STATE; }
    USE_DEVICE(e);
    Plan* plan = nullptr;
    int rc = build_plan(e, B, true, &plan);
    if (rc != PF_OK) return rc;
    if (plan != e->retained_plan) {
        e->err = "pf_unet_backward: the retained forward ran under a different precision mode / plan";
        return PF_ERR_STATE;
    }
    return run_backward(e, plan, vec, g, (hipStream_t)stream);
}

int pf_unet_vjp(pf_engine* e, const float* x, const float* t, const float* vec, float* v, float* g, int B, void* stream) {
    int rc = pf_unet_forward_retain(e, x, t, v, B, stream);
    if (rc != PF_OK) return rc;
    return pf_unet_backward(e, vec, g, B, stream);
}

int pf_ot_ode_vec(const pf_degradation* d, const float* x, const float* vt, const float* y, const float* one_minus_t, const float* rt2,
                  float sigma2, float* vec, int B, int C, int H, int W, float* scratch, void* stream) {
    if (!d || !x || !vt || !y || !one_minus_t || !rt2 || !vec) return PF_ERR_INVALID;
    switch (deg_solve(d->kind)) {
        case DegSolve::FourierSeparable: case DegSolve::FourierPsf: case DegSolve::FourierLowRes:
            LAUNCHCHK(launch_ot_ode_vec_blur(to_view(d), x, vt, y, one_minus_t, rt2, sigma2, vec, B, C, H, W, scratch, (hipStream_t)stream));
            return PF_OK;
        case DegSolve::ClosedForm: case DegSolve::Krylov: break;
    }
    LAUNCHCHK(launch_ot_ode_vec(to_view(d), x, vt, y, one_minus_t, rt2, sigma2, vec, B, C, H, W, (hipStream_t)stream));
    return PF_OK;
}

int pf_psf_power_spectrum(const pf_degradation* d, int H, int W, float* pw2, void* stream) {
    if (!d || !pw2) return PF_ERR_INVALID;
    LAUNCHCHK(launch_psf_power_spectrum(to_view(d), H, W, pw2, (hipStream_t)stream));
    return PF_OK;
}

int pf_sr_aliased_spectrum(const pf_degradation* d, int H, int W, float* lam, float* tmp, void* stream) {
    if (!d || !lam || !tmp) return PF_ERR_INVALID;
    LAUNCHCHK(launch_sr_aliased_spectrum(to_view(d), H, W, lam, tmp, (hipStream_t)stream));
    return PF_OK;
}

int64_t pf_sr_solve_scratch_floats(int B, int C, int H, int W, int sf) {
    if (B <= 0 || C <= 0 || H <= 0 || W <= 0 || sf <= 0) return 0;
    return (int64_t)sr_solve_scratch_floats(B, C, H, W, sf);
}

int pf_sr_prox(const pf_degradation* d, const float* in, const double* alpha_dev, const float* lam, float* out, int B, int C, int H, int W, float* scratch,
               void* stream) {
    if (!d || !in || !alpha_dev || !lam || !out || !scratch || B <= 0 || C <= 0) return PF_ERR_INVALID;
    LAUNCHCHK(launch_fft_prox_sr(to_view(d), in, alpha_dev, lam, out, B, C, H, W, scratch, (hipStream_t)stream));
    return PF_OK;
}

int pf_ot_ode_update(float* x, const float* vt, const float* vec, const float* g, const float* one_minus_t, const float* coef, float delta,
                     int B, int n_per_image, void* stream) {
    if (!x || !vt || !vec || !g || !one_minus_t || !coef) return PF_ERR_INVALID;
    LAUNCHCHK(launch_ot_ode_update(x, vt, vec, g, one_minus_t, coef, delta, B, n_per_image, (hipStream_t)stream));
    return PF_OK;
}

int pf_engine_num_taps(const pf_engine* e) {
    if (!e || !e->last_plan) return 0;
    return (int)e->last_plan->taps.size();
}
// ... 484 lines not shown
```

pnpflow_amd/csrc/pf_common.h:

```cpp
#pragma once
#include <hip/hip_runtime.h>
#include <stdint.h>
#include <atomic>

#include "conv_route.h"
#include "deg_rules.h"

namespace pf {

inline hipError_t set_max_dynamic_lds_once(const void* kernel, unsigned long long& done, int bytes = 160 * 1024) {
    int dev = 0;
    hipError_t e = hipGetDevice(&dev);
    if (e != hipSuccess) return e;
    if (dev >= 0 && dev < 64 && ((done >> dev) & 1ull)) return hipSuccess;
    e = hipFuncSetAttribute(kernel, hipFuncAttributeMaxDynamicSharedMemorySize, bytes);
    if (e == hipSuccess && dev >= 0 && dev < 64) done |= 1ull << dev;
    return e;
}

inline int device_cu_count() {
    static std::atomic<int> cache[64] = {};
    int dev = 0;
    if (hipGetDevice(&dev) != hipSuccess) return 0;
    if (dev >= 0 && dev < 64) { const int c = cache[dev].load(std::memory_order_relaxed); if (c > 0) return c; }
    int v = 0;
    if (hipDeviceGetAttribute(&v, hipDeviceAttributeMultiprocessorCount, dev) != hipSuccess || v < 0) v = 0;
    if (dev >= 0 && dev < 64) cache[dev].store(v, std::memory_order_relaxed);
    return v;
}
inline int persistent_grid() { return (device_cu_count() / 8) * 8; }

struct ConvSeg {
    const float* src;
    int C;
    int cstride;
    int coff;
    int xform;
    int taps;
    int gn_off;
    const double* stats;
    const float* w;
    int w_mode;
    int64_t w_bs, w_cs, w_ts, w_ns, w_ks;
    const void* w16;
    const void* w16h;
    const void* a16;
    int oy, ox;
};

struct ConvParams {
    ConvSeg seg[3];
    int nseg;
    int B, H, W;
    int Hs, Ws;
    int Cout;
    float* out;
    int out_cstride;
    const float* addvec;
    int addvec_bs;
    const float* residual;
    int res_cstride;
    float res_scale;
    double* stats_out;
    float out_scale;
    int gn_C;
    int gn_cpg;
    float gn_eps;
    const float* gamma;
    const float* beta;
    const float* coef;
    int coef_stride;
    const float* scale;
    const float* gnb_x;
    int gnb_xstride;
    const float* gnb_mu; const float* gnb_rs;
    const float* gnb_gamma; const float* gnb_beta;
    int gnb_Ct, gnb_coff, gnb_silu;
    double* gnb_sum;
    int xcd_map;
    int pack_from_p1;
    int src_row_pitch;
    int dst_row_pitch;
};

inline RouteShape route_shape(const ConvParams& p) {
    RouteShape r;
    r.nseg = p.nseg; r.B = p.B; r.H = p.H; r.W = p.W; r.Hs = p.Hs; r.Ws = p.Ws; r.Cout = p.Cout;
    r.out_cstride = p.out_cstride; r.res_cstride = p.res_cstride; r.gn_C = p.gn_C;
    r.residual = p.residual != nullptr; r.addvec = p.addvec != nullptr; r.coef = p.coef != nullptr; r.scale = p.scale != nullptr; r.gnb = p.gnb_x != nullptr;
    for (int i = 0; i < p.nseg && i < 3; ++i) {
        const ConvSeg& s = p.seg[i]; RouteSeg& q = r.seg[i];
        q.C = s.C; q.cstride = s.cstride; q.taps = s.taps; q.xform = s.xform; q.w_mode = s.w_mode; q.has_w16 = s.w16 != nullptr;
    }
    return r;
}

#if defined(__HIPCC__)
__device__ __forceinline__ unsigned int pack_hilo(float v) {
    asm volatile("" : "+v"(v));
    const _Float16 h = (_Float16)v;
    const _Float16 l = (_Float16)(v - (float)h);
    return (unsigned int)__builtin_bit_cast(unsigned short, h) | ((unsigned int)__builtin_bit_cast(unsigned short, l) << 16);
}
__device__ __forceinline__ float4 pack_hilo4(float4 v) {
    return make_float4(__uint_as_float(pack_hilo(v.x)), __uint_as_float(pack_hilo(v.y)), __uint_as_float(pack_hilo(v.z)), __uint_as_float(pack_hilo(v.w)));
}
#endif

constexpr int CONV_KC = 16;

struct EdgeConvParams {
    const float* in;
    float* out;
    const float* w;
    const float* bias;
    int B, H, W, Cimg, C;
    const double* stats; const float* gamma; const float* beta; int gn_cpg; float gn_eps;
    double* stats_out;
    const void* w16;
};

struct AttnParams { const float* qkv; float* out; int B, T, C; float scale; const float* bias; const float* residual; float* stats_part; int kv_packed; };
hipError_t launch_partial_stats(const float* part, double* stats, int B, int nparts, int C, hipStream_t s);
bool attn_fused_supported(int T, int C);
hipError_t launch_attn_fused(const AttnParams& p, hipStream_t s);

struct TembParams {
    const float* t;
    const float* w0; const float* b0;
    const float* w1; const float* b1;
    const float* wp;
    const float* bp;
    float* out;
    int B, ch, total_out;
};

struct GnCoefParams {
    const double* st[3];
    int C[3], xform[3], gn_off[3];
    int nseg, gn_C, gn_cpg, HW;
    float eps;
    const float* gamma; const float* beta;
    float* coef; int coef_stride;
    float* scale;
    unsigned int* flags;
    int id;
    float* mu_out; float* rs_out;
};
hipError_t launch_gn_coef(const GnCoefParams& p, int B, hipStream_t s);

struct PrepParams {
    const float* src[3]; void* dst[3];
    int C[3], cstride[3], coff[3], xform[3], gn_off[3];
    int nseg, B, Hs, Ws, terms;
    const float* coef; int coef_stride;
    const float* scale;
};
hipError_t launch_prep_split(const PrepParams& p, hipStream_t s);
hipError_t launch_conv_dma(const ConvParams& p, const ConvRoute& r, hipStream_t s);
size_t conv_dma_a16_bytes(int B, int C, int Hs, int Ws, int terms);

struct PPChunk {
    const float* src;
    const void* wimg;
    int cstride, coff;
    int xform;
    int gn_c0;
    int seg;
    int pad_;
};
struct PPParams {
    PPChunk ch[PP_MAXCH];
    int n9, n1;
    int cout;
    int B, H, W, lx, ly;
    int rot;
    float* out; const float* addvec; int addvec_bs; const float* residual; float res_scale; double* stats_out; float out_scale;
    const float* coef; int coef_stride; const float* scale;
    const void* wimg_h1[PP_MAXCH];
};
hipError_t launch_conv_pp(const PPParams& p, const ConvRoute& r, hipStream_t s);
hipError_t launch_conv_sp(const PPParams& p, const ConvRoute& r, hipStream_t s);
hipError_t launch_conv(const ConvParams& p, const ConvRoute& r, hipStream_t s);
hipError_t launch_conv16(const ConvParams& p, const ConvRoute& r, hipStream_t s);
size_t conv_flops(const ConvParams& p);
hipError_t launch_begin_conv(const EdgeConvParams& p, hipStream_t s);
hipError_t launch_end_conv(const EdgeConvParams& p, hipStream_t s);
hipError_t launch_temb(const TembParams& p, hipStream_t s);
hipError_t launch_softmax_rows(float* data, int64_t rows, int cols, hipStream_t s);

hipError_t launch_gn_fwd_coeffs(const double* st0, int C0, const double* st1, int C1, int cpg, int HW, float eps, float* mu, float* rs, int B,
                                hipStream_t s);
hipError_t launch_gn_bwd_pre(float* g, const float* x, const float* mu, const float* rs, const float* gamma, const float* beta, double* bsum,
                             int B, int HW, int C, int coff, int Ct, int silu, hipStream_t s);
hipError_t launch_gn_bwd_coeffs(const double* bsum, int Ct, int cpg, int HW, float* m1, float* m2, int B, hipStream_t s);
hipError_t launch_gn_bwd_post(const float* dy, const float* x, const float* mu, const float* rs, const float* m1, const float* m2,
                              const float* add, float* out, int B, int HW, int C, int coff, int Ct, int accumulate, hipStream_t s, float add_scale = 1.0f);
hipError_t launch_transpose(const float* in, float* out, int B, int R, int Cc, hipStream_t s);
hipError_t launch_softmax_bwd(const float* A, float* dA, int64_t rows, int cols, float scale, hipStream_t s);
hipError_t launch_sumpool2(const float* in, float* out, int B, int H, int W, int C, int accumulate, hipStream_t s);

hipError_t launch_deg_H(const DegView& d, const float* x, float* y, int B, int C, int H, int W, float* scratch, hipStream_t s);
hipError_t launch_deg_Hadj(const DegView& d, const float* y, float* x, int B, int C, int H, int W, float* scratch, hipStream_t s);
hipError_t launch_grad_step(const DegView& d, const float* x, const float* y, const float* coef, float* z,
                            int B, int C, int H, int W, float* scratch, int laplace, hipStream_t s);
hipError_t launch_psf_sr(const DegView& d, const float* in, float* out, int B, int C, int H, int W, int sign, int mode, const float* aux, const float* coef,
                         hipStream_t s);
hipError_t launch_psf2d(const DegView& d, const float* in, float* out, int B, int C, int H, int W, int sign, int mode, const float* aux, const float* coef,
                        hipStream_t s);
hipError_t launch_psf_power_spectrum(const DegView& d, int H, int W, float* pw2, hipStream_t s);
hipError_t launch_interpolate(const float* z, const float* t, const float* noise, uint64_t seed, uint64_t stream_id,
                              float* zt, int B, int n, hipStream_t s);
hipError_t launch_interp_iter(const float* z, const float* t, const float* noise, const unsigned long long* rng ,
                              const int* iter, int num_samples, int sample, float* zt, int B, int n, hipStream_t s);
hipError_t launch_denoise_accum(float* acc, const float* zt, const float* v, const float* t, int mode, float ns,
                                int B, int n, hipStream_t s);
hipError_t launch_fill_normal(float* out, int64_t n, uint64_t seed, uint64_t stream_id, uint64_t elem_offset, hipStream_t s);
hipError_t launch_fill_rademacher(float* out, int64_t n, uint64_t seed, uint64_t stream_id, uint64_t elem_offset, hipStream_t s);
hipError_t launch_psnr(const float* rec, const float* clean, float* out, int B, int n, hipStream_t s);
hipError_t launch_fill(float* out, int64_t n, float v, hipStream_t s);
hipError_t launch_upfirdn2d(const float* in, const float* kernel, float* out, int planes, int in_h, int in_w, int kh, int kw,
                            int up_x, int up_y, int down_x, int down_y, int pad_x0, int pad_x1, int pad_y0, int pad_y1, hipStream_t s);
hipError_t launch_fused_bias_act(const float* x, const float* bias, const float* ref, float* out, int64_t n, int step_b, int size_b,
                                 int act, int grad, float alpha, float scale, hipStream_t s);
hipError_t launch_ssim(const float* rec, const float* clean, double* out, int B, int C, int H, int W, hipStream_t s);
hipError_t launch_vjp_normalise(const float* vec, float* vec_scaled, int64_t n, unsigned int* amax_bits, float* scale, hipStream_t s);
hipError_t launch_scale_inplace(float* x, int64_t n, const float* scale, hipStream_t s);

hipError_t launch_ot_ode_vec(const DegView& d, const float* x, const float* vt, const float* y, const float* one_minus_t,
                             const float* rt2, float sigma2, float* vec, int B, int C, int H, int W, hipStream_t s);
hipError_t launch_ot_ode_vec_blur(const DegView& d, const float* x, const float* vt, const float* y, const float* one_minus_t,
                                  const float* rt2, float sigma2, float* vec, int B, int C, int H, int W, float* scratch, hipStream_t s,
                                  bool spectrum_ready = false);
float* sr_solve_lam(float* scratch, int B, int C, int H, int W, int sf);
hipError_t launch_sr_aliased_spectrum(const DegView& d, int H, int W, float* lam, float* tmp, hipStream_t s);
hipError_t launch_fft_prox_sr(const DegView& d, const float* in, const double* alpha_dev, const float* lam, float* out, int B, int C, int H, int W, float* scratch,
                              hipStream_t s);
hipError_t launch_ot_ode_update(float* x, const float* vt, const float* vec, const float* g, const float* one_minus_t, const float* coef,
                                float delta, int B, int n, hipStream_t s);

hipError_t launch_ot_ode_x1hat(const float* x, const float* vt, const float* one_minus_t, float* x1, int B, int n, hipStream_t s);
hipError_t launch_ot_ode_residual(const float* y, const float* hx, float* d, int B, int n, hipStream_t s);
size_t krylov_workspace_floats(int B, size_t n, int max_iter);
hipError_t launch_krylov_solve(const DegView& d, const float* rt2, float sigma2, const float* rhs, float* sol, int B, int C, int H, int W, int max_iter,
                               float tol, float atol, float* ws, size_t ws_floats, int* iters_out, hipStream_t s, int* iterations_run = nullptr);

struct RkTerms { const float* k[7]; float c[7]; int n; };
int reduction_parts(int64_t n4);
hipError_t launch_dflow_axpy(const float* z, const float* v, float* out, float c, int64_t n, hipStream_t s);
hipError_t launch_dflow_objective(const float* hx, const float* y, float* r2, const float* z, double* partial, float* loss, float* coef, float lmbda,
                                  int B, int64_t ny, int64_t n, hipStream_t s);
hipError_t launch_dflow_reg_grad(const float* g, const float* z, const float* coef, float lmbda, float* grad, int B, int64_t n, hipStream_t s);
hipError_t launch_dflow_scale(const float* jg, float* h, float delta, int64_t n, hipStream_t s);
hipError_t launch_dflow_adjoint(float* g, const float* h, const float* jh, float half_delta, int64_t n, hipStream_t s);
hipError_t launch_rk_combine(const float* y0, const RkTerms& t, float* out, int64_t n, hipStream_t s);
hipError_t launch_rk_norm(const float* a, const float* b, const float* y0, const float* y1, const RkTerms& err, float atol, float rtol, double* partial,
                          double* out, int64_t n, hipStream_t s);
hipError_t launch_rk_interp(const float* y0, const float* y1, const float* ymid, const float* k0, const float* k6, float sign, float dt, float x, float* out,
                            int64_t n, hipStream_t s);
hipError_t launch_image_dot(const float* a, const float* c, double* partial, double* out, int B, int64_t n, hipStream_t s);
struct RkAug { const double* k[7]; double step[7]; double err[7]; int n; };
hipError_t launch_rk_aug(const RkAug& c, const double* logp, double* logp_new, double atol, double rtol, const double* sum_x, double* sum_out, int B,
                         hipStream_t s);
hipError_t launch_bpd_finish(const float* z, const double* delta_logp, double* partial, float* bpd, double offset, int B, int64_t n, hipStream_t s);

struct RfStepCoef {
    float dt;
    float c0;
    float a1, a2;
    float s;
};
hipError_t launch_rf_euler_step(float* x, const float* pred, const float* noise, const RfStepCoef& c, uint64_t seed, uint64_t stream_id, uint64_t first,
                                int64_t n, hipStream_t s);

enum { PNPGS_DG = 0, PNPGS_PGD = 1, PNPGS_HQS_MASK = 2, PNPGS_HQS_BLUR = 3, PNPGS_HQS_SR = 4 };
constexpr int PNPGS_MAX_PARTS = 256;
int pnpgs_parts(int64_t n4);
hipError_t launch_pnpgs_seed(const float* x, const float* N, float* r, double* partial, int64_t n, hipStream_t s);
hipError_t launch_pnpgs_combine(int mode, const float* z, const float* N, const float* JN, const float* aux, const uint8_t* mask, const double* alpha_dev,
                                float* out, int B, int64_t n, int64_t hw, hipStream_t s);
hipError_t launch_pnpgs_sqdist(const float* a, const float* b, float* copy_to, double* partial, int64_t n, hipStream_t s);
hipError_t launch_pnpgs_sum(const double* partial, int nparts, double scale, double* out, hipStream_t s);
hipError_t launch_pnpgs_decide(const double* p_new, int np_new, const double* p_dx, int np_dx, double* e_prev, double* alpha_dev, const int* iter, double* log,
                               int max_iter, hipStream_t s);
hipError_t launch_blur_power_spectrum(const DegView& d, int H, int W, float* pw_h, float* pw_w, hipStream_t s);
hipError_t launch_fft_prox_blur(const float* in, const double* alpha_dev, const float* pw_h, const float* pw_w, float* out, int B, int C, int H, int W,
                                float* cplx, hipStream_t s, const float* pw2 = nullptr);

struct AdamCoef;
struct FlowPriorsCoef {
    float dt;
    float fd;
    float num_t;
    float lik;
    int first;
};
hipError_t launch_fp_seed(const float* hx, const float* y, const float* hxi, float* seed, float tn, float omt, float coef, int laplace, int64_t n, hipStream_t s);
hipError_t launch_fp_residual(const DegView& d, const float* x, const float* pred, const float* y, const float* hxi, float* w, float dt, float tn, float omt,
                              float coef, int laplace, int B, int C, int H, int W, hipStream_t s);
hipError_t launch_fp_axpy(const float* a, const float* b, float* out, float c, int64_t n, hipStream_t s);
hipError_t launch_fp_shift(const float* x, const float* eps, float* xp, float* xm, float h, int64_t n, hipStream_t s);
hipError_t launch_fp_grad_adam(const FlowPriorsCoef& c, const AdamCoef* adam, const float* w, const float* jw, const float* jp, const float* jm, const float* pred,
                               float* x, float* m, float* v, float* out_g, float* out_g_data, float* out_g_trace, float* out_g_extra, int64_t n, hipStream_t s);
hipError_t launch_adam_step(const AdamCoef& c, float* x, float* m, float* v, const float* g, int64_t n, hipStream_t s);

struct FirParams {
    const float* src;
    float* out_act; float* out_raw;
    const float* coef; int coef_stride;
    double* stats_raw;
    int B, Hs, Ws, H, W, C;
    int up, down, pad0, K;
    float k2d[64];
};
hipError_t launch_fir_nhwc(const FirParams& p, hipStream_t s);

struct NxTembParams {
    const float* t; float t_scale;
    const float* Wf;
    const float* w0; const float* b0;
    const float* w1; const float* b1;
    const float* wp; const float* bp;
    float* out; int B, nf, total_out;
};
hipError_t launch_nx_temb(const NxTembParams& p, hipStream_t s);

hipError_t launch_img_to_nhwc32(const float* img, float* out, int B, int Cimg, int H, int W, hipStream_t s, const float* div = nullptr );
hipError_t launch_nhwc32_to_img(const float* in, float* img, const float* t, float t_scale, int scale_by_sigma, int B, int Cimg, int H, int W,
                                hipStream_t s, float* sigma_out = nullptr );

}
```

pnpflow_amd/csrc/unet_misc.hip:

```cpp
#include "pf_common.h"

namespace pf {

__device__ __forceinline__ float silu_acc(float x) { return x / (1.0f + expf(-x)); }

template <int C>
__global__ __launch_bounds__(256) void begin_conv_kernel(const EdgeConvParams p) {
    __shared__ float s_t[256][C + 1];
    __shared__ float s_part[8][C][2];
    const int tid = threadIdx.x;
    const float* __restrict__ wgt = p.w;
    const float* __restrict__ bias = p.bias;
    const int HW = p.H * p.W;
    const int pix0 = blockIdx.x * 256;
    const int pix = pix0 + tid;
    const int b = blockIdx.y;
    const bool valid = pix < HW;
    float acc[C];
#pragma unroll
    for (int c = 0; c < C; ++c) acc[c] = valid ? bias[c] : 0.f;
    if (valid) {
        const int y = pix / p.W, x = pix % p.W;
        for (int ci = 0; ci < p.Cimg; ++ci) {
            const float* img = p.in + ((size_t)b * p.Cimg + ci) * HW;
// ... 206 lines not shown
            var = var > 0.0 ? var : 0.0;
            const float rstd = (float)(1.0 / sqrt(var + (double)p.gn_eps));
            sc = p.gamma[tid] * rstd;
            sh = p.beta[tid] - (float)mean * sc;
        }
        s_sc[tid] = sc; s_sh[tid] = sh;
    }
    __syncthreads();
    const int oy0 = ty * 16, ox0 = tx * 16;
    const float* __restrict__ w = p.w;
    for (int pix = tid; pix < PP; pix += 256) {
        const int gy = oy0 - 1 + pix / PW, gx = ox0 - 1 + pix % PW;
        float t[NT_];
#pragma unroll
        for (int k = 0; k < NT_; ++k) t[k] = 0.f;
        if (gy >= 0 && gy < p.H && gx >= 0 && gx < p.W) {
            const float4* src = reinterpret_cast<const float4*>(p.in + ((size_t)(b * p.H + gy) * p.W + gx) * C);
            float a[C];
#pragma unroll
            for (int q = 0; q < C / 4; ++q) {
                const float4 v = src[q];
                a[4 * q] = v.x; a[4 * q + 1] = v.y; a[4 * q + 2] = v.z; a[4 * q + 3] = v.w;
            }
            if (!raw) {
#pragma unroll
                for (int c = 0; c < C; ++c) { const float u = a[c] * s_sc[c] + s_sh[c]; a[c] = u * __builtin_amdgcn_rcpf(1.0f + __expf(-u)); }
            }
#pragma unroll
            for (int k = 0; k < NT_; ++k) {
                float acc = 0.f;
#pragma unroll
                for (int c = 0; c < C; ++c) acc = fmaf(a[c], w[k * C + c], acc);
                t[k] = acc;
            }
        }
#pragma unroll
        for (int k = 0; k < NT_; ++k) s_t[pix * TP + k] = t[k];
    }
    __syncthreads();
    const int ly = tid / 16, lx = tid % 16;
    const int oy = oy0 + ly, ox = ox0 + lx;
    float acc[CIMG];
#pragma unroll
    for (int co = 0; co < CIMG; ++co) acc[co] = p.bias[co];
#pragma unroll
    for (int tap = 0; tap < 9; ++tap) {
        const float* tp = s_t + ((ly + tap / 3) * PW + lx + tap % 3) * TP + tap * CIMG;
#pragma unroll
        for (int co = 0; co < CIMG; ++co) acc[co] += tp[co];
    }
    if (oy < p.H && ox < p.W) {
#pragma unroll
        for (int co = 0; co < CIMG; ++co) p.out[((size_t)(b * CIMG + co) * p.H + oy) * p.W + ox] = acc[co];
    }
}


typedef _Float16 ec_h8 __attribute__((ext_vector_type(8)));
typedef float ec_f16v __attribute__((ext_vector_type(16)));

template <int CIMG>
__global__ __launch_bounds__(256) void end_conv2_kernel(const EdgeConvParams p) {
    constexpr int C = 32, PW = 18, PP = PW * PW, NT_ = 9 * CIMG, TP = NT_ + 1, MTILES = (PP + 31) / 32;
    __shared__ float s_t[PP * TP];
    __shared__ float s_sc[C], s_sh[C];
    const int tiles_x = (p.W + 15) / 16, tiles_y = (p.H + 15) / 16;
    int bid = blockIdx.x;
    const int tx = bid % tiles_x; bid /= tiles_x;
    const int ty = bid % tiles_y;
    const int b = bid / tiles_y;
    const int tid = threadIdx.x, lane = tid & 63, wv = tid >> 6;
    if (tid < C) {
        const int g = tid / p.gn_cpg;
        double sm = 0.0, ss = 0.0;
        for (int j = g * p.gn_cpg; j < (g + 1) * p.gn_cpg; ++j) {
            const double* st = p.stats + ((size_t)b * C + j) * 2;
            sm += st[0]; ss += st[1];
        }
        const double N = (double)p.gn_cpg * p.H * p.W;
        const double mean = sm / N;
        double var = ss / N - mean * mean;
        var = var > 0.0 ? var : 0.0;
        const float rstd = (float)(1.0 / sqrt(var + (double)p.gn_eps));
        const float sc = p.gamma[tid] * rstd;
        s_sc[tid] = sc; s_sh[tid] = p.beta[tid] - (float)mean * sc;
    }
    const ec_h8* wimg = reinterpret_cast<const ec_h8*>(p.w16);
    const ec_h8 wh0 = wimg[0 * 64 + lane], wl0 = wimg[1 * 64 + lane], wh1 = wimg[2 * 64 + lane], wl1 = wimg[3 * 64 + lane];
    __syncthreads();
    const int pl = lane & 31, h = lane >> 5;
    float sc[16], sh[16];
#pragma unroll
    for (int j = 0; j < 16; ++j) { sc[j] = s_sc[16 * h + j]; sh[j] = s_sh[16 * h + j]; }
    const int oy0 = ty * 16, ox0 = tx * 16;
    for (int mt = wv; mt < MTILES; mt += 4) {
        const int hp = mt * 32 + pl;
        const int gy = oy0 - 1 + hp / PW, gx = ox0 - 1 + hp % PW;
        const bool valid = hp < PP && gy >= 0 && gy < p.H && gx >= 0 && gx < p.W;
        float a[16];
        if (valid) {
            const float4* src = reinterpret_cast<const float4*>(p.in + ((size_t)(b * p.H + gy) * p.W + gx) * C + 16 * h);
#pragma unroll
            for (int q4 = 0; q4 < 4; ++q4) { const float4 v = src[q4]; a[4 * q4] = v.x; a[4 * q4 + 1] = v.y; a[4 * q4 + 2] = v.z; a[4 * q4 + 3] = v.w; }
#pragma unroll
            for (int j = 0; j < 16; ++j) { const float u = a[j] * sc[j] + sh[j]; a[j] = u * __builtin_amdgcn_rcpf(1.0f + __expf(-u)) * 8.0f; }
        } else {
#pragma unroll
            for (int j = 0; j < 16; ++j) a[j] = 0.f;
        }
        ec_h8 ah0, al0, ah1, al1;
#pragma unroll
        for (int j = 0; j < 8; ++j) {
            ah0[j] = (_Float16)a[j]; al0[j] = (_Float16)(a[j] - (float)ah0[j]);
            ah1[j] = (_Float16)a[8 + j]; al1[j] = (_Float16)(a[8 + j] - (float)ah1[j]);
        }
        ec_f16v acc;
#pragma unroll
        for (int i = 0; i < 16; ++i) acc[i] = 0.f;
        acc = __builtin_amdgcn_mfma_f32_32x32x16_f16(al0, wh0, acc, 0, 0, 0);
        acc = __builtin_amdgcn_mfma_f32_32x32x16_f16(ah0, wl0, acc, 0, 0, 0);
        acc = __builtin_amdgcn_mfma_f32_32x32x16_f16(ah0, wh0, acc, 0, 0, 0);
        acc = __builtin_amdgcn_mfma_f32_32x32x16_f16(al1, wh1, acc, 0, 0, 0);
        acc = __builtin_amdgcn_mfma_f32_32x32x16_f16(ah1, wl1, acc, 0, 0, 0);
        acc = __builtin_amdgcn_mfma_f32_32x32x16_f16(ah1, wh1, acc, 0, 0, 0);
        if (pl < NT_) {
#pragma unroll
            for (int i = 0; i < 16; ++i) {
                const int row = mt * 32 + 8 * (i >> 2) + 4 * h + (i & 3);
                if (row < PP) s_t[row * TP + pl] = acc[i] * (1.0f / 2048.0f);
            }
        }
    }
    __syncthreads();
    const int ly = tid / 16, lx = tid % 16;
    const int oy = oy0 + ly, ox = ox0 + lx;
    float o[CIMG];
#pragma unroll
    for (int co = 0; co < CIMG; ++co) o[co] = p.bias[co];
#pragma unroll
    for (int tap = 0; tap < 9; ++tap) {
        const float* tp = s_t + ((ly + tap / 3) * PW + lx + tap % 3) * TP + tap * CIMG;
#pragma unroll
        for (int co = 0; co < CIMG; ++co) o[co] += tp[co];
    }
    if (oy < p.H && ox < p.W) {
#pragma unroll
        for (int co = 0; co < CIMG; ++co) p.out[((size_t)(b * CIMG + co) * p.H + oy) * p.W + ox] = o[co];
    }
}

hipError_t launch_end_conv(const EdgeConvParams& p, hipStream_t s) {
    if (p.C != 32 || (p.Cimg != 1 && p.Cimg != 3)) return hipErrorInvalidValue;
    dim3 grid(p.B * ((p.H + 15) / 16) * ((p.W + 15) / 16));
    if (p.w16 != nullptr && p.stats != nullptr) {
        if (p.Cimg == 3) hipLaunchKernelGGL(end_conv2_kernel<3>, grid, dim3(256), 0, s, p);
        else hipLaunchKernelGGL(end_conv2_kernel<1>, grid, dim3(256), 0, s, p);
        return hipGetLastError();
    }
    if (p.Cimg == 3) hipLaunchKernelGGL((end_conv_kernel<32, 3>), grid, dim3(256), 0, s, p);
    else hipLaunchKernelGGL((end_conv_kernel<32, 1>), grid, dim3(256), 0, s, p);
    return hipGetLastError();
}

__global__ __launch_bounds__(256) void temb_kernel(const TembParams p) {
    __shared__ float s_e[64];
    __shared__ float s_h[512];
    __shared__ float s_s[512];
    const int b = blockIdx.y, tid = threadIdx.x;
    const int ch = p.ch, tch = 4 * p.ch, half = ch / 2;
    if (tid < half) {
        const float f = expf((float)tid * -(logf(10000.0f) / (float)(half - 1)));
        const float a = p.t[b] * f;
        s_e[tid] = sinf(a);
        s_e[half + tid] = cosf(a);
    }
    __syncthreads();
    for (int j = tid; j < tch; j += 256) {
        float acc = p.b0[j];
        for (int k = 0; k < ch; ++k) acc = fmaf(p.w0[j * ch + k], s_e[k], acc);
        s_h[j] = silu_acc(acc);
    }
    __syncthreads();
    for (int j = tid; j < tch; j += 256) {
        float acc = p.b1[j];
        for (int k = 0; k < tch; ++k) acc = fmaf(p.w1[j * tch + k], s_h[k], acc);
        s_s[j] = silu_acc(acc);
    }
    __syncthreads();
    const int j = blockIdx.x * 256 + tid;
    if (j < p.total_out) {
        const float4* w = reinterpret_cast<const float4*>(p.wp + (size_t)j * tch);
        float acc = p.bp[j];
        for (int k = 0; k < tch / 4; ++k) {
            const float4 wv = w[k];
            acc = fmaf(wv.x, s_s[4 * k], acc); acc = fmaf(wv.y, s_s[4 * k + 1], acc);
            acc = fmaf(wv.z, s_s[4 * k + 2], acc); acc = fmaf(wv.w, s_s[4 * k + 3], acc);
        }
        p.out[(size_t)b * p.total_out + j] = acc;
    }
}

hipError_t launch_temb(const TembParams& p, hipStream_t s) {
    if (p.ch > 64 || 4 * p.ch > 512 || (p.ch & 1)) return hipErrorInvalidValue;
    dim3 grid((p.total_out + 255) / 256, p.B);
    hipLaunchKernelGGL(temb_kernel, grid, dim3(256), 0, s, p);
    return hipGetLastError();
}

__global__ __launch_bounds__(256) void softmax_rows_kernel(float* data, int64_t rows, int cols) {
    const int lane = threadIdx.x & 63;
    const int64_t row = (int64_t)blockIdx.x * 4 + (threadIdx.x >> 6);
    if (row >= rows) return;
    float* r = data + row * cols;
    float m = -INFINITY;
    for (int i = lane; i < cols; i += 64) m = fmaxf(m, r[i]);
#pragma unroll
    for (int o = 32; o > 0; o >>= 1) m = fmaxf(m, __shfl_xor(m, o));
    float s = 0.f;
    for (int i = lane; i < cols; i += 64) {
        const float e = expf(r[i] - m);
        r[i] = e;
        s += e;
    }
#pragma unroll
    for (int o = 32; o > 0; o >>= 1) s += __shfl_xor(s, o);
    const float inv = 1.0f / s;
    for (int i = lane; i < cols; i += 64) r[i] *= inv;
}

hipError_t launch_softmax_rows(float* data, int64_t rows, int cols, hipStream_t s) {
    hipLaunchKernelGGL(softmax_rows_kernel, dim3((unsigned)((rows + 3) / 4)), dim3(256), 0, s, data, rows, cols);
    return hipGetLastError();
}

__global__ __launch_bounds__(256) void gn_coef_kernel(const GnCoefParams p) {
    __shared__ double s_st[2 * 1024];
    __shared__ double s_red[16];
    __shared__ int s_bad;
    const int b = blockIdx.x, tid = threadIdx.x;
    if (tid == 0) s_bad = 0;
    bool bad = false;
    for (int c = tid; c < p.gn_C; c += 256) {
        double a = 0.0, q = 0.0;
        for (int si = 0; si < p.nseg; ++si)
            if (p.xform[si] != 0 && c >= p.gn_off[si] && c < p.gn_off[si] + p.C[si]) {
                const double* st = p.st[si] + ((size_t)b * p.C[si] + (c - p.gn_off[si])) * 2;
                a = st[0]; q = st[1];
            }
        bad |= !(isfinite(a) && isfinite(q));
        s_st[2 * c] = a; s_st[2 * c + 1] = q;
    }
    double raw_ss[3] = {0.0, 0.0, 0.0};
    for (int si = 0; si < p.nseg; ++si)
        if (p.xform[si] == 0 && p.st[si] != nullptr)
            for (int c = tid; c < p.C[si]; c += 256) {
                const double q = p.st[si][((size_t)b * p.C[si] + c) * 2 + 1];
                bad |= !isfinite(q);
                raw_ss[si] += q;
            }
    __syncthreads();
    double gn_ms = 0.0;
    const double inv_n = 1.0 / ((double)p.gn_cpg * (double)p.HW);
    for (int c = tid; c < p.gn_C; c += 256) {
        const int g0 = (c / p.gn_cpg) * p.gn_cpg;
        double sm = 0.0, ss = 0.0;
        for (int j = g0; j < g0 + p.gn_cpg; ++j) { sm += s_st[2 * j]; ss += s_st[2 * j + 1]; }
        const double mean = sm * inv_n;
        double var = ss * inv_n - mean * mean;
        var = var > 0.0 ? var : 0.0;
        const float rstd = (float)(1.0 / sqrt(var + (double)p.eps));
        const float ga = p.gamma[c], be = p.beta[c];
        const float sc = ga * rstd;
        p.coef[((size_t)b * 2 + 0) * p.coef_stride + c] = sc;
        p.coef[((size_t)b * 2 + 1) * p.coef_stride + c] = be - (float)mean * sc;
        if (p.mu_out != nullptr) { p.mu_out[(size_t)b * p.gn_C + c] = (float)mean; p.rs_out[(size_t)b * p.gn_C + c] = rstd; }
        gn_ms += (double)ga * ga + (double)be * be;
    }
    if (bad) atomicOr(&s_bad, 1);
    if (p.scale != nullptr) {
#pragma unroll
        for (int o = 32; o > 0; o >>= 1) {
            gn_ms += __shfl_xor(gn_ms, o);
#pragma unroll
            for (int k = 0; k < 3; ++k) raw_ss[k] += __shfl_xor(raw_ss[k], o);
        }
        if ((tid & 63) == 0) { s_red[(tid >> 6) * 4] = gn_ms; for (int k = 0; k < 3; ++k) s_red[(tid >> 6) * 4 + 1 + k] = raw_ss[k]; }
    }
    __syncthreads();
    if (tid == 0) {
        if (s_bad && p.flags != nullptr) { atomicOr(p.flags, 1u); atomicCAS(p.flags + 1, 0u, (unsigned)(p.id + 1)); }
        if (p.scale != nullptr) {
            auto pow2_for = [](double ms) {
                float s = 1.0f;
                const float rms = (float)sqrt(ms);
                if (isfinite(rms) && rms > 0.f && (rms < 0.25f || rms > 64.f)) {
                    int e; frexpf(rms, &e);
                    e = e < -40 ? -40 : (e > 40 ? 40 : e);
                    s = ldexpf(1.0f, -e);
                }
                return s;
            };
            const double gs = s_red[0] + s_red[4] + s_red[8] + s_red[12];
            const float s_gn = p.gn_C > 0 ? pow2_for(gs / (double)p.gn_C) : 1.0f;
            for (int si = 0; si < 3; ++si) {
                float sv = 1.0f;
                if (si < p.nseg) {
                    if (p.xform[si] != 0) sv = s_gn;
                    else if (p.st[si] != nullptr)
                        sv = pow2_for((s_red[1 + si] + s_red[5 + si] + s_red[9 + si] + s_red[13 + si]) / ((double)p.C[si] * (double)p.HW));
                }
                p.scale[8 * b + si] = sv; p.scale[8 * b + 4 + si] = 1.0f / sv;
            }
        }
    }
}

hipError_t launch_gn_coef(const GnCoefParams& p, int B, hipStream_t s) {
    if (p.gn_C > 1024 || (p.gn_C > 0 && (p.coef == nullptr || p.gn_cpg <= 0))) return hipErrorInvalidValue;
    hipLaunchKernelGGL(gn_coef_kernel, dim3(B), dim3(256), 0, s, p);
    return hipGetLastError();
}

}
```

pnpflow_amd/csrc/weight_pack.h:

```cpp
#pragma once
#include <cstddef>
#include <vector>

namespace wpack {

using half_t = _Float16;
constexpr int KC = 16;

struct Oihw {
    const float* w; int O, I, kk;
    float operator()(int o, int i, int tap) const { return w[((size_t)o * I + i) * kk + tap]; }
};

struct Split { half_t hi, lo; half_t part(int p) const { return p ? lo : hi; } };
inline Split split16(float w) { w *= 256.0f; const half_t hi = (half_t)w; return {hi, (half_t)(w - (float)hi)}; }

inline int col_channel(int n) { return 4 * (n & 7) + (n >> 3); }

inline std::vector<float> frag32(const Oihw& w, int lo, int hi) {
    const int C = hi - lo, nchunk = (C + KC - 1) / KC;
    std::vector<float> img((size_t)nchunk * w.kk * w.O * KC, 0.f);
    for (int c = 0; c < C; ++c)
        for (int tap = 0; tap < w.kk; ++tap)
            for (int n = 0; n < w.O; ++n)
                img[((((size_t)(c / KC) * w.kk + tap) * 2 + c % KC / 8) * w.O + n) * 8 + c % 8] = w(n, lo + c, tap);
    return img;
}

inline std::vector<half_t> slice16(const Oihw& w, int lo, int hi, int terms) {
    const int C = hi - lo, nchunk = (C + KC - 1) / KC, P = terms == 1 ? 1 : 2;
    std::vector<half_t> img((size_t)nchunk * w.kk * P * w.O * KC, (half_t)0.f);
    for (int c = 0; c < C; ++c)
        for (int tap = 0; tap < w.kk; ++tap)
            for (int n = 0; n < w.O; ++n) {
                const Split s = split16(w(n, lo + c, tap));
                for (int part = 0; part < P; ++part)
                    img[((((size_t)(c / KC) * w.kk + tap) * P + part) * w.O + n) * KC + c % KC] = s.part(part);
            }
    return img;
}

inline std::vector<half_t> chunk_pp(const Oihw& w, int lo) {
    std::vector<half_t> img((size_t)w.kk * 2 * 2 * 2 * 32 * 8, (half_t)0.f);
    size_t at = 0;
    for (int tap = 0; tap < w.kk; ++tap)
        for (int j = 0; j < 2; ++j)
            for (int part = 0; part < 2; ++part)
                for (int kh = 0; kh < 2; ++kh)
                    for (int n = 0; n < 32; ++n)
                        for (int i = 0; i < 8; ++i) img[at++] = split16(w(col_channel(n), lo + 16 * j + 8 * kh + i, tap)).part(part);
    return img;
}

inline std::vector<half_t> chunk_sp(const Oihw& w, int lo, int NT, int terms, int row0 = 0) {
    const int P = terms == 1 ? 1 : 2;
    std::vector<half_t> img((size_t)w.kk * P * NT * 512, (half_t)0.f);
    size_t at = 0;
    for (int tap = 0; tap < w.kk; ++tap)
        for (int part = 0; part < P; ++part)
            for (int nt = 0; nt < NT; ++nt)
                for (int kh = 0; kh < 2; ++kh)
                    for (int n = 0; n < 32; ++n)
                        for (int i = 0; i < 8; ++i) img[at++] = split16(w(row0 + 32 * nt + col_channel(n), lo + 8 * kh + i, tap)).part(part);
    return img;
}

inline std::vector<half_t> edge_frag(const Oihw& w, bool begin) {
    const int cimg = begin ? w.I : w.O;
    std::vector<half_t> img((size_t)2 * 2 * 64 * 8, (half_t)0.f);
    for (int ks = 0; ks < 2; ++ks) for (int hh = 0; hh < 2; ++hh) for (int n = 0; n < 32; ++n) for (int j = 0; j < 8; ++j) {
        const int k = begin ? 16 * ks + 8 * hh + j : n;
        if (k >= 9 * cimg) continue;
        const Split s = begin ? split16(w(n, k / 9, k % 9)) : split16(w(n % cimg, 16 * hh + 8 * ks + j, n / cimg));
        for (int part = 0; part < 2; ++part) img[((((size_t)ks * 2 + part) * 2 + hh) * 32 + n) * 8 + j] = s.part(part);
    }
    return img;
}

inline std::vector<float> adjoint(const Oihw& w, int lo, int hi) {
    const int C = hi - lo;
    std::vector<float> t((size_t)C * w.O * w.kk);
    for (int ci = 0; ci < C; ++ci) for (int co = 0; co < w.O; ++co) for (int tap = 0; tap < w.kk; ++tap)
        t[((size_t)ci * w.O + co) * w.kk + tap] = w(co, lo + ci, w.kk - 1 - tap);
    return t;
}

inline std::vector<float> phase_sums(const Oihw& w) {
    static const int R0[2][2] = {{0, 1}, {0, 2}}, R1[2][2] = {{1, 3}, {2, 3}};
    std::vector<float> t((size_t)4 * w.O * w.I * 4, 0.f);
    for (int dy = 0; dy < 2; ++dy) for (int dx = 0; dx < 2; ++dx)
        for (int o = 0; o < w.O; ++o) for (int i = 0; i < w.I; ++i)
            for (int ty = 0; ty < 2; ++ty) for (int tx = 0; tx < 2; ++tx) {
                double sum = 0.0;
                for (int ky = R0[dy][ty]; ky < R1[dy][ty]; ++ky)
                    for (int kx = R0[dx][tx]; kx < R1[dx][tx]; ++kx) sum += (double)w(o, i, ky * 3 + kx);
                t[(((size_t)(dy * 2 + dx) * w.O + o) * w.I + i) * 4 + ty * 2 + tx] = (float)sum;
            }
    return t;
}

}
```

Before: 3.248 images/s.

## Fold 1x1 shortcut conv into SP 3x3 conv kernel as side taps

Adds an SP_SIDE route in which a 3x3 conv with a concatenated 1x1 shortcut segment (Cout 64) runs in the persistent SP kernel. Each 16-channel 3x3 chunk carries two extra side-step MMA taps that read raw 1x1 inputs from global memory, split them to f16 hi/lo and multiply with packed weights. The weight images are built per chunk with 11 taps. GroupNorm coefficients switch to one common scale, so the shortcut and the main path share an operand scale. This is meant to remove the separate 1x1 conv launch and one output round trip, at the cost of more LDS, more VGPR pressure and heavier scheduling in the SP kernel.

After: 3.262 images/s (median of 6 runs). Within noise of the previous version (+0.4%).

```diff
diff --git a/pnpflow_amd/csrc/conv_route.h b/pnpflow_amd/csrc/conv_route.h
--- a/pnpflow_amd/csrc/conv_route.h
+++ b/pnpflow_amd/csrc/conv_route.h
@@ -25,10 +25,14 @@
 constexpr int sp_npix(int MT) { return (sp_rows(MT) + 2) * SP_PW; }
 constexpr int sp_patch(int MT) { return (sp_rows(MT) + 2) * SP_PITCH * 64; }
 constexpr int sp_tap(int NT, int TERMS = 3) { return (TERMS == 3 ? 2 : 1) * NT * 1024; }
-constexpr int sp_x(int NT, int TERMS = 3) { return (5 * sp_tap(NT, TERMS) + 4095) / 4096 * 4096; }
-constexpr int sp_y(int NT, int TERMS = 3) { return 4 * sp_tap(NT, TERMS); }
+constexpr int sp_xt(int SIDE = 0) { return SIDE ? 6 : 5; }
+constexpr int sp_yt(int SIDE = 0) { return SIDE ? 5 : 4; }
+constexpr int sp_nt(int SIDE = 0) { return sp_xt(SIDE) + sp_yt(SIDE); }
+constexpr int sp_pos(int SIDE, int tap) { return !SIDE ? tap : tap < 4 ? tap : tap == 4 ? 5 : tap < 8 ? tap + 1 : 10; }
+constexpr int sp_x(int NT, int TERMS = 3, int SIDE = 0) { return (sp_xt(SIDE) * sp_tap(NT, TERMS) + 4095) / 4096 * 4096; }
+constexpr int sp_y(int NT, int TERMS = 3, int SIDE = 0) { return sp_yt(SIDE) * sp_tap(NT, TERMS); }
 constexpr int SP_TAB = PP_MAXCH * 32;
-constexpr int sp_lds(int MT, int NT, int TERMS = 3) { return sp_x(NT, TERMS) + sp_y(NT, TERMS) + 2 * sp_patch(MT) + SP_TAB; }
+constexpr int sp_lds(int MT, int NT, int TERMS = 3, int SIDE = 0) { return sp_x(NT, TERMS, SIDE) + sp_y(NT, TERMS, SIDE) + 2 * sp_patch(MT) + SP_TAB; }
 
 constexpr int DMA_TH = 8, DMA_BN = 128;
 constexpr size_t dma_lds() {
@@ -53,10 +57,11 @@
     int sp = 1;
     int dma = 1;
     int upphase = 1;
+    int spside = 1;
 };
 inline RouteEnv mfma_only(RouteEnv env) { env.pp = env.sp = env.dma = 0; return env; }
 
-enum class ConvFamily { MFMA32, MFMA16, DMA, PP, SP };
+enum class ConvFamily { MFMA32, MFMA16, DMA, PP, SP, SP_SIDE };
 struct ConvRoute {
     ConvFamily family = ConvFamily::MFMA32;
     int terms = 0;
@@ -128,6 +133,29 @@
     if (nch < 2 || nch > PP_MAXCH || (nch & 1)) return false;
     if (!(p.gn_C > 0 && p.coef && p.scale)) return false;
     return chunk_sources(p, true);
+}
+
+inline bool sp_side_ok(const RouteShape& p, int stride, int up, int terms, const RouteEnv& env, int& n9, int& n1) {
+    if (env.spside == 0 || (env.sp != 1 && env.sp != 4) || terms != 3 || stride != 1 || up != 0 || p.gnb || p.residual) return false;
+    if (p.Cout != 64 || p.out_cstride != p.Cout || !p.addvec) return false;
+    constexpr int TH = sp_rows(2);
+    if (p.H % TH || p.W % 16 || p.Hs != p.H || p.Ws != p.W) return false;
+    if ((long long)(TH + 1) * p.W + SP_PW - 1 > 65535) return false;
+    if (ilog2_exact(p.H / TH) < 0 || ilog2_exact(p.W / 16) < 0) return false;
+    if (env.cu_grid < 8 || (long long)p.B * (p.H / TH) * (p.W / 16) < 4LL * env.cu_grid) return false;
+    int c9 = 0, c1 = 0;
+    for (int i = 0; i < p.nseg; ++i) {
+        const RouteSeg& s = p.seg[i];
+        if ((double)p.B * p.H * p.W * s.cstride >= 2147483648.0) return false;
+        if (s.w_mode != 0 || !s.has_w16 || !s.has_w16_src || s.src_O != p.Cout) return false;
+        if (s.taps == 9) { if (c1 > 0 || s.xform != 2 || s.C % 32 || s.src_kk != 9) return false; c9 += s.C; }
+        else if (s.taps == 1) { if (s.xform != 0 || s.C % 16 || s.src_kk != 1) return false; c1 += s.C; }
+        else return false;
+    }
+    if (c9 == 0 || c1 != 2 * c9) return false;
+    n9 = c9 / 16; n1 = c1 / 16;
+    if (n9 + n1 > PP_MAXCH) return false;
+    return p.gn_C > 0 && p.coef && p.scale;
 }
 
 inline bool dma_phase_shape_ok(const RouteShape& p, int terms, const RouteEnv& env) {
@@ -259,6 +287,13 @@
         r.grid_x = env.cu_grid; r.lds_bytes = (size_t)sp_lds(r.MT, r.NT, terms);
         return r;
     }
+    if (d::sp_side_ok(p, stride, up, terms, env, r.n9, r.n1)) {
+        r.family = ConvFamily::SP_SIDE; r.csv_code = 6;
+        r.MT = 2; r.NT = 2; r.nsplit = 1; r.res = false;
+        r.grid_x = env.cu_grid; r.lds_bytes = (size_t)sp_lds(2, 2, 3, 2);
+        return r;
+    }
+    r.n9 = r.n1 = 0;
     if (d::pp_ok(p, stride, up, terms, env, r.n9, r.n1)) {
         r.family = ConvFamily::PP; r.csv_code = 2;
         r.MT = PP_MT; r.res = p.residual; r.teams = pp_teams(r.n9, r.n1, terms);
diff --git a/pnpflow_amd/csrc/conv_sp.hip b/pnpflow_amd/csrc/conv_sp.hip
--- a/pnpflow_amd/csrc/conv_sp.hip
+++ b/pnpflow_amd/csrc/conv_sp.hip
@@ -23,21 +23,23 @@
 #define SP_STAMP(k) do { } while (0)
 #endif
 
-template <int MT, int NT, bool RES, int TERMS = 3, int NSPLIT = 1>
+template <int MT, int NT, bool RES, int TERMS = 3, int NSPLIT = 1, int SIDE = 0>
 __global__ __launch_bounds__(256, 1) void conv_sp_kernel(const PPParams p) {
     constexpr int TH = sp_rows(MT), NPIX = sp_npix(MT), A9 = sp_a9(MT), PATCH = sp_patch(MT);
-    constexpr int TAPB = sp_tap(NT, TERMS), XB = sp_x(NT, TERMS), COUT = 32 * NT, CTOT = COUT * NSPLIT, OB = CTOT * 4;
+    constexpr int TAPB = sp_tap(NT, TERMS), XB = sp_x(NT, TERMS, SIDE), YB = sp_y(NT, TERMS, SIDE), XT = sp_xt(SIDE), NTAPS = sp_nt(SIDE), COUT = 32 * NT, CTOT = COUT * NSPLIT, OB = CTOT * 4;
     constexpr int NFRAG = (TERMS == 3 ? 2 : 1) * (MT + NT), NMMA = TERMS * MT * NT;
     static_assert(TERMS == 3 || TERMS == 1, "split terms");
     static_assert(NSPLIT == 1 || NSPLIT == 2, "N-halves");
-    static_assert(sp_y(NT, TERMS) % 4096 == 0 && 9 * TAPB >= XB, "refill rounds of 4 KiB; slot X's over-fetch stays inside the chunk image");
+    static_assert(SIDE == 0 || (SIDE == 2 && !RES && TERMS == 3 && NSPLIT == 1), "side steps: two per chunk, the folded shortcut replaces the identity residual, default mode");
+    static_assert(YB % 4096 == 0 && NTAPS * TAPB >= XB, "refill rounds of 4 KiB; slot X's over-fetch stays inside the chunk image");
     constexpr int REQ1 = sp_stage_0(A9, 4), REQ2 = A9 - REQ1 + 3;
-    static_assert(sp_stage_0(A9, 9) == A9 && REQ1 + NT + 4 * MT * NT < 64, "staging distribution / vmcnt range");
+    constexpr int SREQ = SIDE ? 2 * MT : 0;
+    static_assert(sp_stage_0(A9, 9) == A9 && REQ1 + SREQ + NT + 4 * MT * NT < 64, "staging distribution / vmcnt range");
     extern __shared__ __attribute__((aligned(16))) char smem[];
     const int tid = threadIdx.x;
     const int lane = tid & 63, wq = __builtin_amdgcn_readfirstlane(tid >> 6);
     const int l31 = lane & 31, hi = lane >> 5;
-    constexpr unsigned PATCH0 = (unsigned)(XB + sp_y(NT, TERMS)), TAB = PATCH0 + 2u * (unsigned)PATCH;
+    constexpr unsigned PATCH0 = (unsigned)(XB + YB), TAB = PATCH0 + 2u * (unsigned)PATCH;
     const pp_float_cptr scale_c = (pp_float_cptr)(uintptr_t)p.scale;
     const int nch = p.n9;
 
@@ -188,12 +190,14 @@
         if (p.ch[c].seg != p.ch[c - 1].seg) { if (seg_c1 < 0) seg_c1 = c; else seg_c2 = c; }
     const int seg_id[4] = {p.ch[0].seg, p.ch[seg_c1 > 0 ? seg_c1 : 0].seg, p.ch[seg_c2 > 0 ? seg_c2 : 0].seg, p.ch[nch - 1].seg};
     float addv[NT]; float oscale = 0.f;
+    float sscale = 1.0f;
     auto tile_inputs = [&](const PPTile& tl) __attribute__((always_inline)) {
 #pragma unroll
         for (int nt = 0; nt < NT; ++nt) addv[nt] = p.addvec[(size_t)tl.b * p.addvec_bs + hoff + nt * 32 + ch_of_col];
         const float inv_last = scale_c[8 * tl.b + 4 + seg_id[3]];
         oscale = p.out_scale * (1.0f / 256.0f) * inv_last;
         asm volatile("" : "+v"(oscale));
+        if constexpr (SIDE != 0) { sscale = scale_c[8 * tl.b + seg_id[0]]; asm volatile("" : "+v"(sscale)); }
     };
     auto epilogue = [&](const PPTile& tl) __attribute__((always_inline)) {
         if (tl.b != run_b || run_n >= 32) { flush_stats(); run_b = tl.b; }
@@ -248,7 +252,7 @@
     f16x8 fa[2][MT][2], fb[2][NT][2];
     auto load_tap = [&](int set, int tap, unsigned pofs) __attribute__((always_inline)) {
         const int ky = tap / 3, kx = tap % 3;
-        const unsigned wb = (unsigned)(tap < 5 ? tap * TAPB : XB + (tap - 5) * TAPB) + b_lane;
+        const unsigned wb = (unsigned)(sp_pos(SIDE, tap) < XT ? sp_pos(SIDE, tap) * TAPB : XB + (sp_pos(SIDE, tap) - XT) * TAPB) + b_lane;
         if constexpr (TERMS == 3) {
 #pragma unroll
             for (int mt = 0; mt < MT; ++mt) fa[set][mt][1] = *reinterpret_cast<const f16x8*>(smem + a_addr[kx][1] + (unsigned)((mt * 2 + ky) * SP_PITCH * 64) + pofs);
@@ -264,7 +268,7 @@
     };
     auto load_frag = [&](int set, int tap, unsigned pofs, int idx) __attribute__((always_inline)) {
         const int ky = tap / 3, kx = tap % 3;
-        const unsigned wb = (unsigned)(tap < 5 ? tap * TAPB : XB + (tap - 5) * TAPB) + b_lane;
+        const unsigned wb = (unsigned)(sp_pos(SIDE, tap) < XT ? sp_pos(SIDE, tap) * TAPB : XB + (sp_pos(SIDE, tap) - XT) * TAPB) + b_lane;
         if constexpr (TERMS == 3) {
             if (idx < MT) fa[set][idx][1] = *reinterpret_cast<const f16x8*>(smem + a_addr[kx][1] + (unsigned)((idx * 2 + ky) * SP_PITCH * 64) + pofs);
             else if (idx < MT + NT) fb[set][idx - MT][0] = *reinterpret_cast<const f16x8*>(smem + wb + (unsigned)((idx - MT) * 1024));
@@ -312,7 +316,7 @@
         }
     };
     auto mma_tap_refill = [&](int set, const __attribute__((address_space(1))) char* src, int t0, int nrounds, int nset, int ntap, unsigned npofs) __attribute__((always_inline)) {
-        const unsigned dst0 = (unsigned)(t0 < 5 ? t0 * TAPB : XB + (t0 - 5) * TAPB) + (unsigned)(wq * nrounds * 1024);
+        const unsigned dst0 = (unsigned)(t0 < XT ? t0 * TAPB : XB + (t0 - XT) * TAPB) + (unsigned)(wq * nrounds * 1024);
         const __attribute__((address_space(1))) char* sb = src + t0 * TAPB + wq * nrounds * 1024;
         unsigned keep;
         asm volatile("s_mov_b32 %0, m0" : "=s"(keep));
@@ -336,6 +340,87 @@
             }
         }
         asm volatile("s_mov_b32 m0, %0" :: "s"(keep));
+    };
+
+    float4 rs[SIDE ? MT : 1][2];
+    unsigned soff[SIDE ? MT : 1];
+    if constexpr (SIDE != 0) {
+#pragma unroll
+        for (int mt = 0; mt < MT; ++mt) soff[mt] = (unsigned)((wq * 2 * MT + mt * 2 + prow) * p.W + pcol);
+    }
+    struct SDesc { gptr base; unsigned cs4; };
+    auto sdescribe = [&](const PPTile& tl, const Ent& e) __attribute__((always_inline)) -> SDesc {
+        const int pix = (tl.b * p.H + tl.oy0) * p.W + tl.ox0;
+        const int cstride = __builtin_amdgcn_readfirstlane((int)e.b.x), coff = __builtin_amdgcn_readfirstlane((int)e.b.y);
+        SDesc d;
+        d.base = sptr(e.a.x, e.a.y) + (long)(pix * cstride + coff) * 4;
+        d.cs4 = (unsigned)cstride * 4u;
+        return d;
+    };
+    auto side_issue = [&](const SDesc& d) __attribute__((always_inline)) {
+#pragma unroll
+        for (int mt = 0; mt < (SIDE ? MT : 0); ++mt) {
+            const gptr a = d.base + (__umul24(soff[mt], d.cs4) + (unsigned)hi * 32u);
+            const pp_f4v t0 = *reinterpret_cast<const __attribute__((address_space(1))) pp_f4v*>(a);
+            const pp_f4v t1 = *reinterpret_cast<const __attribute__((address_space(1))) pp_f4v*>(a + 16);
+            rs[mt][0] = make_float4(t0.x, t0.y, t0.z, t0.w); rs[mt][1] = make_float4(t1.x, t1.y, t1.z, t1.w);
+        }
+    };
+    auto side_convert = [&](int set) __attribute__((always_inline)) {
+#pragma unroll
+        for (int mt = 0; mt < (SIDE ? MT : 0); ++mt) {
+            float4 a = rs[mt][0], b = rs[mt][1];
+            a.x *= sscale; a.y *= sscale; a.z *= sscale; a.w *= sscale; b.x *= sscale; b.y *= sscale; b.z *= sscale; b.w *= sscale;
+            uint4 h, l;
+            split4_pp(a, h.x, h.y, l.x, l.y);
+            split4_pp(b, h.z, h.w, l.z, l.w);
+            fa[set][mt][0] = __builtin_bit_cast(f16x8, h);
+            fa[set][mt][1] = __builtin_bit_cast(f16x8, l);
+        }
+    };
+    auto load_side_b = [&](int set, int pos) __attribute__((always_inline)) {
+        const unsigned wb = (unsigned)(pos < XT ? pos * TAPB : XB + (pos - XT) * TAPB) + b_lane;
+#pragma unroll
+        for (int nt = 0; nt < NT; ++nt) fb[set][nt][0] = *reinterpret_cast<const f16x8*>(smem + wb + (unsigned)(nt * 1024));
+#pragma unroll
+        for (int nt = 0; nt < NT; ++nt) fb[set][nt][1] = *reinterpret_cast<const f16x8*>(smem + wb + (unsigned)(NT * 1024 + nt * 1024));
+    };
+    auto side_pattern = [&]() __attribute__((always_inline)) {
+#pragma unroll
+        for (int k = 0; k < 3 * MT * NT; ++k) {
+            __builtin_amdgcn_sched_group_barrier(0x008, 1, 0);
+            if (k < NFRAG) __builtin_amdgcn_sched_group_barrier(0x100, 1, 0);
+            __builtin_amdgcn_sched_group_barrier(0x002, 3, 0);
+            __builtin_amdgcn_sched_group_barrier(0x004, 2, 0);
+            if (k >= 2 && k < 2 + SREQ) __builtin_amdgcn_sched_group_barrier(0x020, 1, 0);
+        }
+    };
+    SDesc sdb{}, sda{};
+    auto side_tap_pattern = [&](int n) __attribute__((always_inline)) {
+#pragma unroll
+        for (int k = 0; k < n; ++k) {
+            __builtin_amdgcn_sched_group_barrier(0x008, 1, 0);
+            if (k < NFRAG) __builtin_amdgcn_sched_group_barrier(0x100, 1, 0);
+            __builtin_amdgcn_sched_group_barrier(0x002, 5, 0);
+            __builtin_amdgcn_sched_group_barrier(0x400, 1, 0);
+            __builtin_amdgcn_sched_group_barrier(0x004, 4, 0);
+            if (k >= n - 4) __builtin_amdgcn_sched_group_barrier(0x200, 1, 0);
+            if (k == n - 2) __builtin_amdgcn_sched_group_barrier(0x020, 1, 0);
+        }
+    };
+    auto mma_tap_convert = [&](int set, int cset) __attribute__((always_inline)) {
+#pragma unroll
+        for (int g = 0; g < 2 * MT; ++g) mma_group(set, g);
+        side_tap_pattern(2 * MT * NT);
+        __builtin_amdgcn_sched_barrier(0);
+        side_convert(cset);
+#pragma unroll
+        for (int g = 2 * MT; g < 3 * MT; ++g) mma_group(set, g);
+#pragma unroll
+        for (int k = 0; k < MT * NT; ++k) {
+            __builtin_amdgcn_sched_group_barrier(0x008, 1, 0);
+            __builtin_amdgcn_sched_group_barrier(0x002, 6, 0);
+        }
     };
 
     int stamp_n = 0; (void)stamp_n;
@@ -356,24 +441,34 @@
 #pragma unroll
         for (int tap = 0; tap < 4; ++tap) {
             __builtin_amdgcn_sched_barrier(0);
-            load_tap((tap + 1 + SI) & 1, tap + 1, PCUR);
+            if (SIDE != 0 && tap == 1) sdb = sdescribe(tile_of(it), fetch(nch + 2 * c + 1));
+            if (SIDE != 0 && tap == 3) load_side_b((4 + SI) & 1, 4);
+            else load_tap((tap + 1 + SI) & 1, tap + 1, PCUR);
 #pragma unroll
             for (int i = sp_stage_0(A9, tap); i < sp_stage_0(A9, tap) + sp_stage_n(A9, tap); ++i) { transform_one(C, i, PNXT); issue_one(N, sr, i); }
-            mma_tap((tap + SI) & 1);
-            tap_pattern();
+            if (SIDE != 0 && tap == 3) mma_tap_convert((tap + SI) & 1, (4 + SI) & 1);
+            else if constexpr (SIDE != 0) { mma_tap((tap + SI) & 1); side_tap_pattern(NMMA); }
+            else { mma_tap((tap + SI) & 1); tap_pattern(); }
             __builtin_amdgcn_sched_barrier(0);
             SP_STAMP(1 + tap);
         }
         __builtin_amdgcn_sched_barrier(0);
-        if (c == 0) asm volatile("s_waitcnt vmcnt(%0) lgkmcnt(0)" :: "n"(REQ1 + NT + 4 * MT * NT) : "memory");
-        else asm volatile("s_waitcnt vmcnt(%0) lgkmcnt(0)" :: "n"(REQ1) : "memory");
+        if constexpr (SIDE != 0) {
+            load_tap((5 + SI) & 1, 4, PCUR);
+            side_issue(sdb);
+            mma_tap((4 + SI) & 1);
+            side_pattern();
+            __builtin_amdgcn_sched_barrier(0);
+        }
+        if (c == 0) asm volatile("s_waitcnt vmcnt(%0) lgkmcnt(0)" :: "n"(REQ1 + SREQ + NT + 4 * MT * NT) : "memory");
+        else asm volatile("s_waitcnt vmcnt(%0) lgkmcnt(0)" :: "n"(REQ1 + SREQ) : "memory");
 #pragma unroll
         for (int i = REQ1; i < A9; ++i) asm volatile("" :: "v"(ra[i].x));
         SP_STAMP(13);
         __builtin_amdgcn_s_barrier();
         __builtin_amdgcn_sched_barrier(0);
         SP_STAMP(5);
-        mma_tap_refill((4 + SI) & 1, wnext, 0, XB / 4096, (5 + SI) & 1, 5, PCUR);
+        mma_tap_refill((sp_pos(SIDE, 4) + SI) & 1, wnext, 0, XB / 4096, (sp_pos(SIDE, 5) + SI) & 1, 5, PCUR);
         SP_STAMP(6);
 #pragma unroll
         for (int tap = 5; tap < 8; ++tap) {
@@ -383,36 +478,48 @@
             if (q >= nch) { q -= nch; wrap = 2; }
             const int c2 = c + 2 >= nch ? c + 2 - nch : c + 2;
             Ent eq, e2;
-            if (tap == 6) { eq = fetch(q); e2 = fetch(c2); }
-            load_tap((tap + 1 + SI) & 1, tap + 1, PCUR);
+            Ent ea;
+            const int cn = c + 1 >= nch ? 0 : c + 1;
+            if (tap == 6) { eq = fetch(q); e2 = fetch(c2); if (SIDE != 0) ea = fetch(nch + 2 * cn); }
+            if (SIDE != 0 && tap == 7) load_side_b((9 + SI) & 1, 9);
+            else load_tap((sp_pos(SIDE, tap + 1) + SI) & 1, tap + 1, PCUR);
 #pragma unroll
             for (int i = sp_stage_0(A9, tap); i < sp_stage_0(A9, tap) + sp_stage_n(A9, tap); ++i) { transform_one(C, i, PNXT); issue_one(N, sr, i); }
             if (tap == 6) {
                 dn = describe(tile_of(it + wrap), eq);
                 wimg_next = sptr(e2.a.z, e2.a.w);
+                if constexpr (SIDE != 0) sda = sdescribe(tile_of(it + (c + 1 >= nch ? 1 : 0)), ea);
             }
             if (tap == 7) sr = prep(C, dn);
-            mma_tap((tap + SI) & 1);
-            tap_pattern();
+            if (SIDE != 0 && tap == 7) mma_tap_convert((sp_pos(SIDE, tap) + SI) & 1, (9 + SI) & 1);
+            else if constexpr (SIDE != 0) { mma_tap((sp_pos(SIDE, tap) + SI) & 1); side_tap_pattern(NMMA); }
+            else { mma_tap((sp_pos(SIDE, tap) + SI) & 1); tap_pattern(); }
             __builtin_amdgcn_sched_barrier(0);
             SP_STAMP(2 + tap);
         }
         __builtin_amdgcn_sched_barrier(0);
-        asm volatile("s_waitcnt vmcnt(%0) lgkmcnt(0)" :: "n"(REQ2) : "memory");
+        if constexpr (SIDE != 0) {
+            load_tap((10 + SI) & 1, 8, PCUR);
+            side_issue(sda);
+            mma_tap((9 + SI) & 1);
+            side_pattern();
+            __builtin_amdgcn_sched_barrier(0);
+        }
+        asm volatile("s_waitcnt vmcnt(%0) lgkmcnt(0)" :: "n"(REQ2 + SREQ) : "memory");
 #pragma unroll
         for (int i = 0; i < REQ1; ++i) asm volatile("" :: "v"(ra[i].x));
         SP_STAMP(14);
         __builtin_amdgcn_s_barrier();
         __builtin_amdgcn_sched_barrier(0);
         SP_STAMP(10);
-        mma_tap_refill((8 + SI) & 1, wnext, 5, 4 * TAPB / 4096, (9 + SI) & 1, 0, PNXT);
+        mma_tap_refill((sp_pos(SIDE, 8) + SI) & 1, wnext, XT, YB / 4096, (NTAPS + SI) & 1, 0, PNXT);
         SP_STAMP(11);
         SP_STAMP(12);
         ++stamp_n;
     };
 
     if (ntl <= 0) return;
-    for (int c = 0; c < nch; ++c) {
+    for (int c = 0; c < nch + (SIDE ? p.n1 : 0); ++c) {
         if (tid == 0) {
             const unsigned long long sp_ = (unsigned long long)(uintptr_t)p.ch[c].src, wp_ = (unsigned long long)(uintptr_t)(half ? p.wimg_h1[c] : p.ch[c].wimg);
             *reinterpret_cast<uint4*>(smem + TAB + (unsigned)c * 32u) = make_uint4((unsigned)sp_, (unsigned)(sp_ >> 32), (unsigned)wp_, (unsigned)(wp_ >> 32));
@@ -427,7 +534,7 @@
         {
             const char* w0 = reinterpret_cast<const char*>(half ? p.wimg_h1[0] : p.ch[0].wimg);
 #pragma unroll
-            for (int j = 0; j < (TERMS == 3 ? 9 * TAPB : XB) / 4096; ++j) glds16_sp(dma_lane, w0 + j * 4096, (unsigned)(j * 4096) + (unsigned)(wq * 1024));
+            for (int j = 0; j < (TERMS == 3 ? NTAPS * TAPB : XB) / 4096; ++j) glds16_sp(dma_lane, w0 + j * 4096, (unsigned)(j * 4096) + (unsigned)(wq * 1024));
             if constexpr (TERMS != 3) {
 #pragma unroll
                 for (int j = 0; j < 4 * TAPB / 4096; ++j) glds16_sp(dma_lane, w0 + 5 * TAPB + j * 4096, (unsigned)(XB + j * 4096) + (unsigned)(wq * 1024));
@@ -439,6 +546,7 @@
 #pragma unroll
         for (int i = 0; i < A9; ++i) issue_one(cf1, s1, i);
         sr = prep(cf0, describe(tile_of(2 >= nch ? 1 : 0), fetch(2 >= nch ? 2 - nch : 2)));
+        if constexpr (SIDE != 0) side_issue(sdescribe(tile_of(0), fetch(nch)));
         asm volatile("s_waitcnt vmcnt(0) lgkmcnt(0)" ::: "memory");
         __builtin_amdgcn_s_barrier();
         __builtin_amdgcn_sched_barrier(0);
@@ -491,7 +599,20 @@
     return hipGetLastError();
 }
 
+static hipError_t launch_sp_side(const PPParams& p0, const ConvRoute& r, hipStream_t s) {
+    static unsigned long long attr_set = 0ull;
+    if (r.MT != 2 || r.NT != 2 || r.terms != 3 || r.nsplit != 1 || r.res || r.n9 != p0.n9 || r.n1 != p0.n1 || p0.n1 != 2 * p0.n9 || p0.n9 + p0.n1 > PP_MAXCH ||
+        p0.residual != nullptr || r.grid_x <= 0) return hipErrorInvalidValue;
+    { hipError_t e = set_max_dynamic_lds_once(reinterpret_cast<const void*>(conv_sp_kernel<2, 2, false, 3, 1, 2>), attr_set, ROUTE_LDS_MAX); if (e != hipSuccess) return e; }
+    PPParams p = p0;
+    p.lx = ilog2_exact(p.W / 16); p.ly = ilog2_exact(p.H / sp_rows(2));
+    p.rot = 5;
+    hipLaunchKernelGGL((conv_sp_kernel<2, 2, false, 3, 1, 2>), dim3(r.grid_x), dim3(256), r.lds_bytes, s, p);
+    return hipGetLastError();
+}
+
 hipError_t launch_conv_sp(const PPParams& p, const ConvRoute& r, hipStream_t s) {
+    if (r.family == ConvFamily::SP_SIDE) return launch_sp_side(p, r, s);
     if (r.family != ConvFamily::SP || r.n9 != p.n9 || p.n1 != 0 || r.res != (p.residual != nullptr)) return hipErrorInvalidValue;
     switch (r.MT * 1000 + r.NT * 100 + r.nsplit * 10 + r.terms) {
         case 2423: return launch_sp_t<2, 4, 3, 2>(p, r, s);
diff --git a/pnpflow_amd/csrc/engine.hip b/pnpflow_amd/csrc/engine.hip
--- a/pnpflow_amd/csrc/engine.hip
+++ b/pnpflow_amd/csrc/engine.hip
@@ -399,6 +399,7 @@
     static const RouteEnv switches = [] {
         auto rd = [](const char* name) { const char* v = getenv(name); return v ? atoi(v) : 1; };
         RouteEnv v; v.pp = rd("PNPFLOW_HIP_PP"); v.sp = rd("PNPFLOW_HIP_SP"); v.dma = rd("PNPFLOW_HIP_DMA"); v.upphase = rd("PNPFLOW_HIP_UPPHASE");
+        v.spside = rd("PNPFLOW_HIP_SPSIDE");
         return v;
     }();
     RouteEnv v = switches; v.cu_grid = persistent_grid();
@@ -476,6 +477,48 @@
     return true;
 }
 
+static bool attach_sp_side(Builder& bd, const ConvParams& p, const ConvRoute& r, PPParams& q) {
+    pf_engine* e = bd.e;
+    q = PPParams{};
+    q.cout = p.Cout;
+    struct Side { const ConvSeg* sg; int seg, cc; std::string name; int lo; };
+    std::vector<Side> side;
+    for (int i = 0; i < p.nseg; ++i) {
+        if (p.seg[i].taps != 1) continue;
+        const pf_engine::W16Src& src = e->w16_src.at(p.seg[i].w16);
+        for (int cc = 0; cc < p.seg[i].C / 16; ++cc) side.push_back({&p.seg[i], i, cc, src.name, src.lo + cc * 16});
+    }
+    int n = 0;
+    for (int i = 0; i < p.nseg; ++i) {
+        const ConvSeg& sg = p.seg[i];
+        if (sg.taps != 9) continue;
+        const pf_engine::W16Src& src = e->w16_src.at(sg.w16);
+        const wpack::Oihw w = oihw(e, src.name);
+        for (int cc = 0; cc < sg.C / 16; ++cc, ++n) {
+            if (2 * n + 1 >= (int)side.size()) return false;
+            PPChunk& k = q.ch[n];
+            k.src = sg.src; k.cstride = sg.cstride; k.coff = sg.coff + cc * 16; k.xform = sg.xform; k.gn_c0 = sg.gn_off + cc * 16; k.seg = i;
+            const Side &sa = side[2 * n], &sb = side[2 * n + 1];
+            const wpack::Oihw wa = oihw(e, sa.name), wb = oihw(e, sb.name);
+            const int lo = src.lo + cc * 16;
+            const std::string key = src.name + "#sps" + std::to_string(p.Cout) + "_" + std::to_string(lo) + "|" + sa.name + "_" + std::to_string(sa.lo) + "|" + sb.name + "_" + std::to_string(sb.lo);
+            k.wimg = weight_image(e, key, [&] { return wpack::chunk_sp_side(w, lo, wa, sa.lo, wb, sb.lo, r.NT); });
+            if (!k.wimg) return false;
+        }
+    }
+    q.n9 = n; q.n1 = (int)side.size();
+    if (q.n9 != r.n9 || q.n1 != r.n1 || q.n9 + q.n1 > PP_MAXCH) return false;
+    for (int j = 0; j < q.n1; ++j) {
+        PPChunk& k = q.ch[q.n9 + j];
+        const ConvSeg& sg = *side[j].sg;
+        k.src = sg.src; k.cstride = sg.cstride; k.coff = sg.coff + side[j].cc * 16; k.xform = 0; k.gn_c0 = 0; k.seg = side[j].seg; k.wimg = nullptr;
+    }
+    q.B = p.B; q.H = p.H; q.W = p.W;
+    q.out = p.out; q.addvec = p.addvec; q.addvec_bs = p.addvec_bs; q.residual = nullptr; q.res_scale = p.res_scale;
+    q.stats_out = p.stats_out; q.out_scale = p.out_scale; q.coef = p.coef; q.coef_stride = p.coef_stride; q.scale = p.scale;
+    return true;
+}
+
 static ConvFamily push_conv(Builder& bd, const ConvParams& p0, int stride = 1, int up = 0) {
     pf_engine* e = bd.e;
     ConvParams p = with_coef(bd, p0, bd.plan->ops);
@@ -485,6 +528,11 @@
     bool built = true;
     if (op.route.refused) { built = false; e->err = std::string("conv launch refused: ") + op.route.refused; }
     else if (f == ConvFamily::PP || f == ConvFamily::SP) built = attach_pp(bd, p, op.route, op.ppp);
+    else if (f == ConvFamily::SP_SIDE) {
+        built = attach_sp_side(bd, p, op.route, op.ppp);
+        if (built && (bd.plan->ops.empty() || bd.plan->ops.back().kind != OP_GN_COEF || bd.plan->ops.back().gp.scale != p.scale)) built = false;
+        if (built) bd.plan->ops.back().gp.common_scale = 1;
+    }
     else if (f == ConvFamily::DMA) built = attach_dma(bd, p, op.route, bd.plan->ops);
     if (!built) {
         if (bd.ok) { bd.ok = false; if (!op.route.refused) e->err = "conv launch: a weight image or operand buffer could not be allocated"; }
@@ -705,7 +753,7 @@
 static void fix_stats(Op& op, double* slab) {
     auto fx = [&](const double*& p) { if (p) p = (const double*)((char*)slab + ((uintptr_t)p - 1)); };
     auto fxm = [&](double*& p) { if (p) p = (double*)((char*)slab + ((uintptr_t)p - 1)); };
-    if (op.kind == OP_CONV) { for (int i = 0; i < op.cp.nseg; ++i) fx(op.cp.seg[i].stats); fxm(op.cp.stats_out); fxm(op.cp.gnb_sum); if (op.route.family == ConvFamily::PP || op.route.family == ConvFamily::SP) op.ppp.stats_out = op.cp.stats_out; }
+    if (op.kind == OP_CONV) { for (int i = 0; i < op.cp.nseg; ++i) fx(op.cp.seg[i].stats); fxm(op.cp.stats_out); fxm(op.cp.gnb_sum); if (op.route.family == ConvFamily::PP || op.route.family == ConvFamily::SP || op.route.family == ConvFamily::SP_SIDE) op.ppp.stats_out = op.cp.stats_out; }
     if (op.kind == OP_GN_COEF) for (int i = 0; i < op.gp.nseg; ++i) fx(op.gp.st[i]);
     if (op.kind == OP_STATS) { double* d = (double*)op.O; fxm(d); op.O = d; }
     if (op.kind == OP_NX_FIR) fxm(op.fp.stats_raw);
@@ -1247,7 +1295,7 @@
 
 static hipError_t dispatch_conv(const Op& op, hipStream_t s) {
     switch (op.route.family) {
-        case ConvFamily::SP: return launch_conv_sp(op.ppp, op.route, s);
+        case ConvFamily::SP: case ConvFamily::SP_SIDE: return launch_conv_sp(op.ppp, op.route, s);
         case ConvFamily::PP: return launch_conv_pp(op.ppp, op.route, s);
         case ConvFamily::DMA: return launch_conv_dma(op.cp, op.route, s);
         case ConvFamily::MFMA16: return launch_conv16(op.cp, op.route, s);
diff --git a/pnpflow_amd/csrc/pf_common.h b/pnpflow_amd/csrc/pf_common.h
--- a/pnpflow_amd/csrc/pf_common.h
+++ b/pnpflow_amd/csrc/pf_common.h
@@ -146,6 +146,7 @@
     unsigned int* flags;
     int id;
     float* mu_out; float* rs_out;
+    int common_scale;
 };
 hipError_t launch_gn_coef(const GnCoefParams& p, int B, hipStream_t s);
 
diff --git a/pnpflow_amd/csrc/unet_misc.hip b/pnpflow_amd/csrc/unet_misc.hip
--- a/pnpflow_amd/csrc/unet_misc.hip
+++ b/pnpflow_amd/csrc/unet_misc.hip
@@ -532,10 +532,18 @@
             };
             const double gs = s_red[0] + s_red[4] + s_red[8] + s_red[12];
             const float s_gn = p.gn_C > 0 ? pow2_for(gs / (double)p.gn_C) : 1.0f;
+            double ms_max = p.gn_C > 0 ? gs / (double)p.gn_C : -1.0;
+            for (int si = 0; si < p.nseg && si < 3; ++si)
+                if (p.xform[si] == 0 && p.st[si] != nullptr) {
+                    const double ms = (s_red[1 + si] + s_red[5 + si] + s_red[9 + si] + s_red[13 + si]) / ((double)p.C[si] * (double)p.HW);
+                    ms_max = ms > ms_max ? ms : ms_max;
+                }
+            const float s_common = ms_max >= 0.0 ? pow2_for(ms_max) : 1.0f;
             for (int si = 0; si < 3; ++si) {
                 float sv = 1.0f;
                 if (si < p.nseg) {
-                    if (p.xform[si] != 0) sv = s_gn;
+                    if (p.common_scale != 0) sv = s_common;
+                    else if (p.xform[si] != 0) sv = s_gn;
                     else if (p.st[si] != nullptr)
                         sv = pow2_for((s_red[1 + si] + s_red[5 + si] + s_red[9 + si] + s_red[13 + si]) / ((double)p.C[si] * (double)p.HW));
                 }
diff --git a/pnpflow_amd/csrc/weight_pack.h b/pnpflow_amd/csrc/weight_pack.h
--- a/pnpflow_amd/csrc/weight_pack.h
+++ b/pnpflow_amd/csrc/weight_pack.h
@@ -65,6 +65,21 @@
     return img;
 }
 
+inline std::vector<half_t> chunk_sp_side(const Oihw& w9, int lo, const Oihw& w1a, int lo_a, const Oihw& w1b, int lo_b, int NT) {
+    std::vector<half_t> img((size_t)11 * 2 * NT * 512, (half_t)0.f);
+    size_t at = 0;
+    for (int q = 0; q < 11; ++q) {
+        const Oihw& w = q == 4 ? w1a : q == 9 ? w1b : w9;
+        const int l0 = q == 4 ? lo_a : q == 9 ? lo_b : lo, tap = q == 4 || q == 9 ? 0 : q < 4 ? q : q < 9 ? q - 1 : 8;
+        for (int part = 0; part < 2; ++part)
+            for (int nt = 0; nt < NT; ++nt)
+                for (int kh = 0; kh < 2; ++kh)
+                    for (int n = 0; n < 32; ++n)
+                        for (int i = 0; i < 8; ++i) img[at++] = split16(w(32 * nt + col_channel(n), l0 + 8 * kh + i, tap)).part(part);
+    }
+    return img;
+}
+
 inline std::vector<half_t> edge_frag(const Oihw& w, bool begin) {
     const int cimg = begin ? w.I : w.O;
     std::vector<half_t> img((size_t)2 * 2 * 64 * 8, (half_t)0.f);
```
